# naman1618/Distributed-Inference-with-PyTorch-and-LiteLLM

Hardware: AMD Instinct MI355X
Metric: fine-tune tokens/sec (whole node) Llama-3.1-70B DDP at 1/2/4/8 MI355X (higher is better)
Workload: dtype bf16; 1 GPU; model=Llama-3.1-70B, global_batch=2, seq_len=2048, parallelism=dp1, finetune=lora r=16 alpha=32.0 on q,k,v,o,gate,up,down; frozen bf16 base, micro_batch=2, grad_accum=1, activation_checkpointing=False, optimizer=fused AdamW (HIP), grad clip 1.0, grad_reduce_dtype=bf16

## Files before the change

csrc/bindings.cpp:

```cpp
#include <torch/library.h>
#include <ATen/ATen.h>
#include <ATen/hip/impl/HIPStreamMasqueradingAsCUDA.h>
#include <ATen/hip/impl/HIPGuardImplMasqueradingAsCUDA.h>
#include <hip/hip_runtime.h>
#include "bindings.h"
#include <algorithm>
#include <cstring>
#include <limits>
#include <mutex>
#include <vector>

namespace {

inline hipStream_t cur_stream() { return c10::hip::getCurrentHIPStreamMasqueradingAsCUDA().stream(); }
using DevGuard = c10::hip::HIPGuardMasqueradingAsCUDA;

#define MX_CHECK(cond, ...) TORCH_CHECK(cond, "mxllm: ", __VA_ARGS__)
#define MX_OK(call)                                                                              \
  do {                                                                                           \
    int _rc = (call);                                                                            \
    TORCH_CHECK(_rc == 0, "mxllm kernel launch failed (" #call ") rc=", _rc, " ",                 \
                hipGetErrorString((hipError_t)(_rc > 0 ? _rc : 1)));                             \
  } while (0)

// ... 100 lines not shown
  return {dx, need_dw ? dw : at::Tensor()};
}

void copy2d_batched(const at::Tensor& desc, int64_t total_blocks) {
  MX_CHECK(desc.is_cuda() && desc.scalar_type() == at::kLong && desc.dim() == 2 && desc.size(1) == 9 &&
               desc.is_contiguous(), "desc must be int64 [n, 9] on the GPU");
  DevGuard g(desc.device());
  MX_OK(mx_copy2d_batched(desc.data_ptr<int64_t>(), (int)desc.size(0), total_blocks, cur_stream()));
}

at::Tensor transpose2d(const at::Tensor& in, const c10::optional<at::Tensor>& scale) {
  MX_CHECK(in.is_cuda() && in.dim() == 2 && in.element_size() == 2, "in must be a 2-D 16-bit GPU tensor");
  MX_CHECK(in.stride(1) == 1 && in.stride(0) >= in.size(1), "in must be a row-major (row-strided) view");
  const float* sc = nullptr;
  if (scale.has_value()) {
    MX_CHECK(in.scalar_type() == at::kBFloat16 && scale->scalar_type() == at::kFloat && scale->numel() == 1 &&
                 scale->device() == in.device(), "transpose2d scale: f32 scalar on the device, bf16 input");
    sc = scale->data_ptr<float>();
  }
  DevGuard g(in.device());
  const int64_t R = in.size(0), C = in.size(1);
  auto out = at::empty({C, R}, in.options());
  MX_OK(mx_transpose16(in.data_ptr(), out.data_ptr(), R, C, in.stride(0), R, sc, cur_stream()));
  return out;
}


inline const uint16_t* g8p(const mx::G8Mat& m) { return static_cast<const uint16_t*>(m.p); }
inline uint16_t* g8pm(const mx::G8Mat& m) { return static_cast<uint16_t*>(const_cast<void*>(m.p)); }

const float* f32_scalar(const char* what, const c10::optional<at::Tensor>& t, const at::Device& dev) {
  if (!t.has_value()) return nullptr;
  MX_CHECK(t->scalar_type() == at::kFloat && t->numel() == 1 && t->device() == dev, what,
           ": f32 scalar on the device");
  return t->data_ptr<float>();
}

bool g8_fill(const char* op, mx::G8Launch& L, const at::Tensor& a, bool a_kc, const at::Tensor& b, bool b_kc,
             const at::Tensor* out, bool f32_ok) {
  MX_CHECK(a.is_cuda() && b.is_cuda() && (!out || out->is_cuda()), op, ": GPU tensors");
  MX_CHECK(a.scalar_type() == at::kBFloat16 && b.scalar_type() == at::kBFloat16, op, ": bf16 operands");
  MX_CHECK(!out || out->scalar_type() == at::kBFloat16 || (f32_ok && out->scalar_type() == at::kFloat), op,
           f32_ok ? ": fp32 / bf16 output" : ": bf16 output");
  MX_CHECK(a.dim() == 2 && b.dim() == 2 && (!out || out->dim() == 2), op, ": 2-D operands");
  const int64_t M = a_kc ? a.size(0) : a.size(1), K = a_kc ? a.size(1) : a.size(0);
  const int64_t N = b_kc ? b.size(0) : b.size(1), Kb = b_kc ? b.size(1) : b.size(0);
  MX_CHECK(K == Kb && (!out || (out->size(0) == M && out->size(1) == N)), op, ": shape mismatch");
  if (a.stride(1) != 1 || b.stride(1) != 1 || (out && out->stride(1) != 1)) return false;
  if (M > INT32_MAX || N > INT32_MAX || K > INT32_MAX) return false;
  L.A = {a.data_ptr(), a.stride(0), a_kc ? 1 : 0};
  L.B = {b.data_ptr(), b.stride(0), b_kc ? 1 : 0};
  if (out) L.C = {out->data_ptr(), out->stride(0), 1};
  L.out_f32 = out && out->scalar_type() == at::kFloat ? 1 : 0;
  L.M = (int)M, L.N = (int)N, L.K = (int)K;
  return true;
}

bool g8_fill_rope(const char* op, mx::G8Launch& L, const at::Tensor& x, const at::Tensor& w, const at::Tensor& cos,
                  const at::Tensor& sin, int64_t B, int64_t S, int64_t Hq, int64_t Hkv, at::Tensor& q, at::Tensor& k,
                  at::Tensor& v) {
  MX_CHECK(x.dim() == 2 && w.dim() == 2 && x.size(0) == B * S, op, ": shapes");
  MX_CHECK(w.size(0) == (Hq + 2 * Hkv) * 128, op, ": head dim 128");
  MX_CHECK(cos.scalar_type() == at::kFloat && sin.scalar_type() == at::kFloat && cos.is_contiguous() &&
               sin.is_contiguous() && cos.size(-1) == 64 && cos.size(0) >= S && sin.sizes() == cos.sizes(),
           op, ": f32 [>= S, 64] tables");
  for (const at::Tensor* t : {&q, &k, &v})
    MX_CHECK(t->is_cuda() && t->scalar_type() == at::kBFloat16 && t->is_contiguous(), op, ": bf16 outputs");
  MX_CHECK(q.numel() == B * Hq * S * 128 && k.numel() == B * Hkv * S * 128 && v.numel() == k.numel(), op,
           ": output sizes");
  if (!g8_fill(op, L, x, true, w, true, nullptr, false)) return false;
  L.epi = mx::G8_EPI_ROPE;
  L.ep.q = bfm(q), L.ep.k = bfm(k), L.ep.v = bfm(v);
  L.ep.cosb = cos.data_ptr<float>(), L.ep.sinb = sin.data_ptr<float>();
  L.ep.S = (int)S, L.ep.Hq = (int)Hq, L.ep.Hkv = (int)Hkv;
  return true;
}

bool g8_launched(const char* op, int rc) {
  if (rc == -1) return false;
  TORCH_CHECK(rc == 0, "mxllm kernel launch failed (", op, ") rc=", rc, " ", hipGetErrorString((hipError_t)(rc > 0 ? rc : 1)));
  return true;
}

bool gemm8(const at::Tensor& a, bool a_kc, const at::Tensor& b, bool b_kc, at::Tensor& out, double beta,
           const c10::optional<at::Tensor>& alpha_t, double alpha_f, int64_t ph) {
  mx::G8Launch L{};
  if (!g8_fill("gemm8", L, a, a_kc, b, b_kc, &out, true)) return false;
  const float* sc = f32_scalar("gemm8 alpha_t", alpha_t, a.device());
  DevGuard g(a.device());
  return g8_launched("mx_gemm8", mx_gemm8(g8p(L.A), L.A.ld, L.A.kc, g8p(L.B), L.B.ld, L.B.kc, out.data_ptr(), L.C.ld,
                                          L.out_f32, L.M, L.N, L.K, (float)beta, sc, (float)alpha_f, (int)ph,
                                          cur_stream()));
}

bool gemm8_sq(const at::Tensor& a, bool a_kc, const at::Tensor& b, bool b_kc, at::Tensor& out, at::Tensor& sq,
              const c10::optional<at::Tensor>& alpha_t, double alpha_f) {
  MX_CHECK(sq.is_cuda() && sq.scalar_type() == at::kFloat, "gemm8_sq: f32 GPU partials");
  mx::G8Launch L{};
  if (!g8_fill("gemm8_sq", L, a, a_kc, b, b_kc, &out, false) || !sq.is_contiguous()) return false;
  if (L.M % 256 || L.N % 256) return false;
  MX_CHECK(sq.numel() >= (int64_t)(L.M / 256) * (L.N / 256), "gemm8_sq: partials buffer too small");
  const float* sc = f32_scalar("gemm8_sq alpha_t", alpha_t, a.device());
  DevGuard g(a.device());
  return g8_launched("mx_gemm8_sq", mx_gemm8_sq(g8p(L.A), L.A.ld, L.A.kc, g8p(L.B), L.B.ld, L.B.kc, g8pm(L.C), L.C.ld,
                                                L.M, L.N, L.K, sc, (float)alpha_f, sq.data_ptr<float>(),
                                                cur_stream()));
}

bool gemm8_tail(const at::Tensor& a, bool a_kc, const at::Tensor& b, bool b_kc, at::Tensor& out, int64_t at,
                bool rows, int64_t ph, const c10::optional<at::Tensor>& sq) {
  mx::G8Launch L{};
  if (!g8_fill("gemm8_tail", L, a, a_kc, b, b_kc, &out, false)) return false;
  const int64_t lim = rows ? L.M : L.N;
  if (at <= 0 || at >= lim) return false;
  float* sqp = nullptr;
  if (sq.has_value()) {
    MX_CHECK(sq->scalar_type() == at::kFloat && sq->is_contiguous() && sq->device() == a.device(),
             "gemm8_tail sq: contiguous f32 on the device");
    if (L.M % 256 || L.N % 256) return false;
    MX_CHECK(sq->numel() >= (int64_t)(L.M / 256) * (L.N / 256), "gemm8_tail sq: partials buffer too small");
    sqp = sq->data_ptr<float>();
  }
  DevGuard g(a.device());
  auto ws = at::empty({2 * (lim - at) * (rows ? L.N : L.M)}, a.options().dtype(at::kFloat));
  return g8_launched("mx_gemm8_tail",
                     mx_gemm8_tail(g8p(L.A), L.A.ld, L.A.kc, g8p(L.B), L.B.ld, L.B.kc, g8pm(L.C), L.C.ld, L.M, L.N, L.K,
                                   rows ? 1 : 0, (int)at, ws.data_ptr<float>(), (int)ph, cur_stream(), sqp));
}

bool gemm8_rope(const at::Tensor& x, const at::Tensor& w, const at::Tensor& cos, const at::Tensor& sin, int64_t B,
                int64_t S, int64_t Hq, int64_t Hkv, at::Tensor& q, at::Tensor& k, at::Tensor& v) {
  mx::G8Launch L{};
  if (!g8_fill_rope("gemm8_rope", L, x, w, cos, sin, B, S, Hq, Hkv, q, k, v)) return false;
  DevGuard g(x.device());
  return g8_launched("mx_gemm8_epi", mx_gemm8_epi(g8p(L.A), L.A.ld, g8p(L.B), L.B.ld, nullptr, 0, L.M, L.N, L.K,
                                                  mx::G8_EPI_ROPE, L.ep, cur_stream()));
}

bool gemm8_rope_tail(const at::Tensor& x, const at::Tensor& w, const at::Tensor& cos, const at::Tensor& sin, int64_t B,
                     int64_t S, int64_t Hq, int64_t Hkv, at::Tensor& q, at::Tensor& k, at::Tensor& v, int64_t at) {
  mx::G8Launch L{};
  if (!g8_fill_rope("gemm8_rope_tail", L, x, w, cos, sin, B, S, Hq, Hkv, q, k, v) || at <= 0 || at >= L.N) return false;
  DevGuard g(x.device());
  auto ws = at::empty({2 * (int64_t)L.M * (L.N - at)}, x.options().dtype(at::kFloat));
  return g8_launched("mx_gemm8_rope_tail", mx_gemm8_rope_tail(g8p(L.A), L.A.ld, g8p(L.B), L.B.ld, L.M, L.N, L.K, (int)at,
                                                              ws.data_ptr<float>(), L.ep, cur_stream()));
}

bool gemm8_swiglu(const at::Tensor& x, const at::Tensor& w, at::Tensor& gu, at::Tensor& m) {
  mx::G8Launch L{};
  const bool ok = g8_fill("gemm8_swiglu", L, x, true, w, true, &gu, false);
  MX_CHECK(m.scalar_type() == at::kBFloat16 && m.dim() == 2 && m.size(0) == x.size(0) && 2 * m.size(1) == w.size(0),
           "gemm8_swiglu: m [T, F] bf16");
  if (!ok || m.stride(1) != 1) return false;
  DevGuard g(x.device());
  L.ep.m = bfm(m);
  L.ep.ldm = m.stride(0);
  return g8_launched("mx_gemm8_epi", mx_gemm8_epi(g8p(L.A), L.A.ld, g8p(L.B), L.B.ld, g8pm(L.C), L.C.ld, L.M, L.N, L.K,
                                                  mx::G8_EPI_SWIGLU, L.ep, cur_stream()));
}

bool gemm8_swiglu_bwd(const at::Tensor& dy, const at::Tensor& w, const at::Tensor& gu, at::Tensor& dgu,
                      const c10::optional<at::Tensor>& m) {
  mx::G8Launch L{};
  const bool ok = g8_fill("gemm8_swiglu_bwd", L, dy, true, w, false, nullptr, false);
  MX_CHECK(gu.is_cuda() && gu.scalar_type() == at::kBFloat16 && dgu.scalar_type() == at::kBFloat16,
           "gemm8_swiglu_bwd: bf16 GPU tensors");
  MX_CHECK(gu.dim() == 2 && dgu.dim() == 2 && gu.size(0) == dy.size(0) && gu.size(1) == 2 * w.size(1) &&
               dgu.sizes() == gu.sizes(),
           "gemm8_swiglu_bwd: shapes");
  if (m) {
    MX_CHECK(m->scalar_type() == at::kBFloat16 && m->dim() == 2 && m->size(0) == dy.size(0) &&
                 m->size(1) == w.size(1),
             "gemm8_swiglu_bwd: m [T, F] bf16");
    if (m->stride(1) != 1) return false;
    L.ep.m = reinterpret_cast<uint16_t*>(m->data_ptr());
    L.ep.ldm = m->stride(0);
  }
  if (!ok || gu.stride(1) != 1 || dgu.stride(1) != 1) return false;
  DevGuard g(dy.device());
  L.ep.gu = bf(gu);
  L.ep.ldg = gu.stride(0);
  return g8_launched("mx_gemm8_epi", mx_gemm8_epi(g8p(L.A), L.A.ld, g8p(L.B), L.B.ld, bfm(dgu), dgu.stride(0), L.M, L.N,
                                                  L.K, mx::G8_EPI_SWIGLU_BWD, L.ep, cur_stream()));
}

at::Tensor gemm8_stamps() {
  auto out = at::empty({1024, 2, 80}, at::TensorOptions().dtype(at::kLong));
  MX_OK(mx_gemm8_stamps(reinterpret_cast<unsigned long long*>(out.data_ptr<int64_t>())));
  return out;
}

int64_t cu_masked_stream(int64_t device, std::vector<int64_t> mask) {
  MX_CHECK(!mask.empty(), "cu_masked_stream: empty mask");
  DevGuard g(c10::Device(c10::DeviceType::CUDA, (c10::DeviceIndex)device));
  std::vector<uint32_t> w(mask.size());
  for (size_t i = 0; i < mask.size(); ++i) w[i] = (uint32_t)(mask[i] & 0xffffffffLL);
  hipStream_t s = nullptr;
  hipError_t e = hipExtStreamCreateWithCUMask(&s, (uint32_t)(w.size() * 32), w.data());
  MX_CHECK(e == hipSuccess, "hipExtStreamCreateWithCUMask: ", hipGetErrorString(e));
  return (int64_t)reinterpret_cast<intptr_t>(s);
}

void prefetch(const at::Tensor& t, int64_t wgs) {
  MX_CHECK(t.is_cuda() && t.is_contiguous(), "prefetch: contiguous GPU tensor");
  DevGuard g(t.device());
  MX_OK(mx_prefetch(t.data_ptr(), t.numel() * t.element_size(), (int)wgs, cur_stream()));
}

at::Tensor segmented_mean(const at::Tensor& codes, const at::Tensor& offsets) {
  MX_CHECK(codes.is_cuda() && codes.scalar_type() == at::kInt, "codes must be int32 GPU");
  MX_CHECK(offsets.is_cuda() && offsets.scalar_type() == at::kLong, "offsets must be int64 GPU");
  DevGuard g(codes.device());
  const int64_t n = offsets.numel() - 1;
  auto out = at::empty({std::max<int64_t>(n, 0)}, codes.options().dtype(at::kFloat));
  if (n > 0)
    MX_OK(mx_segmented_mean_i32(codes.data_ptr<int32_t>(), offsets.data_ptr<int64_t>(),
                                out.data_ptr<float>(), (int)n, cur_stream()));
  return out;
}

at::Tensor sqnorm(const at::Tensor& x) {
  MX_CHECK(x.is_cuda() && x.is_contiguous(), "x must be a contiguous GPU tensor");
  MX_CHECK(x.scalar_type() == at::kFloat || x.scalar_type() == at::kBFloat16, "x must be float32 or bfloat16");
  DevGuard g(x.device());
  auto opts = x.options().dtype(at::kFloat);
  auto out = at::empty({1}, opts);
  auto work = at::empty({2048}, opts);
  MX_OK(mx_sqnorm(x.data_ptr(), x.scalar_type() == at::kBFloat16 ? 1 : 0, x.numel(), out.data_ptr<float>(),
                  work.data_ptr<float>(), cur_stream()));
  return out;
}

at::Tensor swiglu_fwd(const at::Tensor& gu, int64_t out_pad) {
  check_bf16(gu, "gu");
  DevGuard g(gu.device());
  const int64_t F2 = gu.size(-1);
  MX_CHECK(F2 % 16 == 0, "2F must be a multiple of 16");
  MX_CHECK(out_pad >= 0 && out_pad % 8 == 0, "out_pad must be a non-negative multiple of 8");
  const int64_t T = gu.numel() / F2;
  at::Tensor m;
  if (out_pad > 0) {
    m = empty_rows(T, F2 / 2, out_pad, gu.options());
  } else {
    auto sizes = gu.sizes().vec();
    sizes.back() = F2 / 2;
    m = at::empty(sizes, gu.options());
  }
  if (T > 0) MX_OK(mx_swiglu_fwd(bf(gu), bfm(m), T, (int)(F2 / 2), F2 / 2 + out_pad, cur_stream()));
  return m;
}

at::Tensor swiglu_bwd(const at::Tensor& dm, const at::Tensor& gu, int64_t out_pad) {
  check_bf16(dm, "dm");
  check_bf16(gu, "gu");
  DevGuard g(gu.device());
  const int64_t F2 = gu.size(-1);
  const int64_t T = gu.numel() / F2;
  MX_CHECK(dm.numel() == T * (F2 / 2), "dm shape mismatch");
  MX_CHECK(out_pad >= 0 && out_pad % 8 == 0, "out_pad must be a non-negative multiple of 8");
  at::Tensor dgu = out_pad > 0 ? empty_rows(T, F2, out_pad, gu.options()) : at::empty_like(gu);
  if (T > 0) MX_OK(mx_swiglu_bwd(bf(dm), bf(gu), bfm(dgu), T, (int)(F2 / 2), F2 + out_pad, cur_stream()));
  return dgu;
}

std::vector<at::Tensor> swiglu_bwd_m(const at::Tensor& dm, const at::Tensor& gu) {
  check_bf16(dm, "dm");
  check_bf16(gu, "gu");
  DevGuard g(gu.device());
  const int64_t F2 = gu.size(-1);
  const int64_t T = gu.numel() / F2;
  MX_CHECK(dm.numel() == T * (F2 / 2), "dm shape mismatch");
  MX_CHECK(dm.is_contiguous() && gu.is_contiguous(), "swiglu_bwd_m: dense dm / gu");
  at::Tensor dgu = at::empty_like(gu);
  at::Tensor m = at::empty({T, F2 / 2}, gu.options());
  if (T > 0) MX_OK(mx_swiglu_bwd(bf(dm), bf(gu), bfm(dgu), T, (int)(F2 / 2), F2, cur_stream(), bfm(m)));
  return {dgu, m};
}

at::Tensor swiglu_lora(const c10::optional<at::Tensor>& dm, const at::Tensor& gu, int64_t pad, const at::Tensor& v,
                       int64_t nrb, double alpha) {
  check_bf16(gu, "gu");
  const int64_t ldv = check_rows_bf16(v, "v");
  DevGuard g(gu.device());
  const bool bwd = dm.has_value();
  MX_CHECK(gu.dim() == 2 && gu.size(1) > 0 && gu.size(1) % 256 == 0,
           "swiglu_lora: gu [T, 2F] with F % 128 == 0 (gate | up halves of equal width)");
  const int64_t F2 = gu.size(1), F = F2 / 2, T = gu.size(0);
  MX_CHECK(T % 16 == 0, "swiglu_lora: [T, 2F] with T % 16 == 0");
  MX_CHECK(nrb >= 1 && nrb <= 4 && pad >= 16 * nrb && pad % 8 == 0, "swiglu_lora: 16 nrb <= pad");
  MX_CHECK(v.size(0) >= 16 * nrb && v.size(1) == (bwd ? F2 : F), "swiglu_lora: v shape");
  if (bwd) {
    check_bf16(*dm, "dm");
    MX_CHECK(dm->numel() == T * F, "swiglu_lora: dm shape");
  }
  const int64_t W = bwd ? F2 : F;
  at::Tensor out = at::empty({T, W + pad}, gu.options());
  const int64_t nws = mx_swiglu_lora_ws((int)T, (int)F, (int)nrb);
  auto ws = at::empty({nws > 0 ? nws : 1}, gu.options().dtype(at::kFloat));
  if (T > 0)
    MX_OK(mx_swiglu_lora(bwd ? 1 : 0, bf(gu), bwd ? bf(*dm) : nullptr, bfm(out), W + pad, bf(v), ldv, (int)nrb,
                         (int)pad, (float)alpha, ws.data_ptr<float>(), (int)T, (int)F, cur_stream()));
  return out.narrow(1, 0, W);
}

void adamw_step(const c10::optional<at::Tensor>& master, at::Tensor grad, at::Tensor m, at::Tensor v,
                const c10::optional<at::Tensor>& lowp, const c10::optional<at::Tensor>& lo, double lr, double b1,
                double b2, double eps, double wd, double bc1, double bc2, const c10::optional<at::Tensor>& scale_t,
                double scale_f, bool zero_grad) {
  MX_CHECK(master.has_value() != lo.has_value(), "give either the fp32 master or the split low half");
  check_f32(m, "m");
  check_f32(v, "v");
  MX_CHECK(grad.is_cuda() && grad.is_contiguous(), "grad must be contiguous GPU");
  MX_CHECK(grad.scalar_type() == at::kFloat || grad.scalar_type() == at::kBFloat16, "grad f32/bf16");
  const int64_t n = m.numel();
  MX_CHECK(grad.numel() == n && v.numel() == n, "adamw size mismatch");
  float* mp = nullptr;
  if (master.has_value()) {
    check_f32(*master, "master");
    MX_CHECK(master->numel() == n, "master size");
    mp = master->data_ptr<float>();
  }
  DevGuard g(m.device());
  uint16_t* lp = nullptr;
  if (lowp.has_value()) {
    check_bf16(*lowp, "lowp");
    MX_CHECK(lowp->numel() == n, "lowp size");
    lp = reinterpret_cast<uint16_t*>(lowp->data_ptr());
  }
  int16_t* lop = nullptr;
  if (lo.has_value()) {
    MX_CHECK(lo->is_cuda() && lo->is_contiguous() && lo->scalar_type() == at::kShort && lo->numel() == n,
             "lo must be a contiguous int16 GPU tensor of the master's size");
    MX_CHECK(lp != nullptr, "split master needs lowp (the high half)");
    lop = lo->data_ptr<int16_t>();
  }
  const float* st = nullptr;
  if (scale_t.has_value()) {
    check_f32(*scale_t, "scale_t");
    st = scale_t->data_ptr<float>();
  }
  MX_OK(mx_adamw(mp, grad.data_ptr(), grad.scalar_type() == at::kBFloat16 ? 1 : 0, m.data_ptr<float>(),
                 v.data_ptr<float>(), lp, lop, n, (float)lr, (float)b1, (float)b2, (float)eps, (float)wd, (float)bc1,
                 (float)bc2, st, (float)scale_f, zero_grad ? 1 : 0, cur_stream()));
}

void split_master(const at::Tensor& x, at::Tensor hi, at::Tensor lo) {
  check_f32(x, "x");
  check_bf16(hi, "hi");
  MX_CHECK(lo.is_cuda() && lo.is_contiguous() && lo.scalar_type() == at::kShort, "lo int16 contiguous GPU");
  MX_CHECK(hi.numel() == x.numel() && lo.numel() == x.numel(), "split_master size mismatch");
  DevGuard g(x.device());
  MX_OK(mx_split_master(x.data_ptr<float>(), reinterpret_cast<uint16_t*>(hi.data_ptr()), lo.data_ptr<int16_t>(),
                        x.numel(), cur_stream()));
}

void join_master(const at::Tensor& hi, const at::Tensor& lo, at::Tensor out) {
  check_bf16(hi, "hi");
  check_f32(out, "out");
  MX_CHECK(lo.is_cuda() && lo.is_contiguous() && lo.scalar_type() == at::kShort, "lo int16 contiguous GPU");
  MX_CHECK(hi.numel() == out.numel() && lo.numel() == out.numel(), "join_master size mismatch");
  DevGuard g(out.device());
  MX_OK(mx_join_master(reinterpret_cast<const uint16_t*>(hi.data_ptr()), lo.data_ptr<int16_t>(),
                       out.data_ptr<float>(), out.numel(), cur_stream()));
}

at::Tensor embedding_fwd(const at::Tensor& ids, const at::Tensor& w) {
  check_bf16(w, "weight");
  MX_CHECK(ids.is_cuda() && ids.scalar_type() == at::kLong, "ids must be int64 GPU");
  DevGuard g(w.device());
  auto idc = ids.contiguous();
  const int64_t T = idc.numel(), H = w.size(1), V = w.size(0);
  auto out = at::empty({T, H}, w.options());
  MX_OK(mx_embedding_fwd(idc.data_ptr<int64_t>(), bf(w), bfm(out), T, (int)H, V, cur_stream()));
  return out;
}

at::Tensor embedding_bwd(const at::Tensor& dy, const at::Tensor& ids, int64_t V) {
  check_bf16(dy, "dy");
  DevGuard g(dy.device());
  auto idc = ids.contiguous();
  const int64_t H = dy.size(-1), T = idc.numel();
  auto dw = at::zeros({V, H}, dy.options().dtype(at::kFloat));
  MX_OK(mx_embedding_bwd(idc.data_ptr<int64_t>(), bf(dy), dw.data_ptr<float>(), T, (int)H, V, cur_stream()));
  return dw;
}

void embedding_bwd_sorted(const at::Tensor& dy, const at::Tensor& sid, const at::Tensor& perm, at::Tensor out) {
  check_bf16(dy, "dy");
  MX_CHECK(sid.scalar_type() == at::kLong && perm.scalar_type() == at::kLong && sid.is_contiguous() &&
               perm.is_contiguous() && sid.numel() == perm.numel(), "sid / perm: int64, same length");
  MX_CHECK(out.is_contiguous() && (out.scalar_type() == at::kFloat || out.scalar_type() == at::kBFloat16) &&
               out.dim() == 2 && out.size(1) == dy.size(-1) && dy.is_contiguous() &&
               dy.numel() == sid.numel() * dy.size(-1) && out.device() == dy.device(),
           "embedding_bwd_sorted: out [V, H] f32/bf16 contiguous, dy [T, H] contiguous");
  DevGuard g(dy.device());
  const int64_t T = sid.numel(), nch = (T + 63) / 64;
  auto ws = at::empty({std::max<int64_t>(1, 2 * nch * out.size(1))}, dy.options().dtype(at::kFloat));
  MX_OK(mx_embedding_bwd_sorted(bf(dy), sid.data_ptr<int64_t>(), perm.data_ptr<int64_t>(), T, (int)out.size(1),
                                out.size(0), out.data_ptr(), out.scalar_type() == at::kFloat ? 1 : 0,
                                ws.data_ptr<float>(), cur_stream()));
}

std::tuple<at::Tensor, at::Tensor> ce_fwd_bwd(at::Tensor logits, const at::Tensor& labels, int64_t ignore) {
  check_bf16(logits, "logits");
  MX_CHECK(labels.is_cuda() && labels.scalar_type() == at::kLong, "labels must be int64 GPU");
  DevGuard g(logits.device());
  const int64_t V = logits.size(-1), T = logits.numel() / V;
  MX_CHECK(labels.numel() == T, "labels size mismatch");
  auto lab = labels.contiguous();
  auto losses = at::empty({T}, logits.options().dtype(at::kFloat));
  auto ws = at::empty({2}, logits.options().dtype(at::kFloat));
  auto loss = at::empty({}, logits.options().dtype(at::kFloat));
  MX_OK(mx_ce_fwd_bwd(bfm(logits), lab.data_ptr<int64_t>(), losses.data_ptr<float>(), ws.data_ptr<float>(),
                      loss.data_ptr<float>(), T, (int)V, ignore, cur_stream()));
  return {loss, losses};
}

at::Tensor ce_inv_count(const at::Tensor& labels, int64_t ignore, int64_t V) {
  MX_CHECK(labels.is_cuda() && labels.scalar_type() == at::kLong, "labels must be int64 GPU");
  DevGuard g(labels.device());
  auto lab = labels.contiguous();
  auto inv = at::empty({1}, labels.options().dtype(at::kFloat));
  MX_OK(mx_ce_inv_count(lab.data_ptr<int64_t>(), lab.numel(), (int)V, ignore, inv.data_ptr<float>(), cur_stream()));
  return inv;
}

at::Tensor ce_chunk(at::Tensor logits, const at::Tensor& labels, int64_t ignore, const at::Tensor& inv_n) {
  check_bf16(logits, "logits");
  MX_CHECK(logits.is_contiguous(), "ce_chunk: contiguous logits");
  MX_CHECK(labels.is_cuda() && labels.scalar_type() == at::kLong, "labels must be int64 GPU");
  MX_CHECK(inv_n.scalar_type() == at::kFloat && inv_n.numel() == 1 && inv_n.device() == logits.device(),
           "ce_chunk: inv_n f32 device scalar");
  DevGuard g(logits.device());
  const int64_t V = logits.size(-1), T = logits.numel() / V;
  MX_CHECK(labels.numel() == T, "labels size mismatch");
  auto lab = labels.contiguous();
  auto losses = at::empty({T}, logits.options().dtype(at::kFloat));
  MX_OK(mx_ce_chunk(bfm(logits), lab.data_ptr<int64_t>(), losses.data_ptr<float>(), inv_n.data_ptr<float>(), T,
                    (int)V, ignore, cur_stream()));
  return losses;
}

at::Tensor ce_chunk_f32(const at::Tensor& logits, at::Tensor dl, const at::Tensor& labels, int64_t ignore,
                        const at::Tensor& inv_n) {
  check_f32(logits, "logits");
  check_bf16(dl, "dl");
  MX_CHECK(logits.is_contiguous() && dl.is_contiguous() && dl.sizes() == logits.sizes(), "ce_chunk_f32: shapes");
  MX_CHECK(labels.is_cuda() && labels.scalar_type() == at::kLong, "labels must be int64 GPU");
  MX_CHECK(inv_n.scalar_type() == at::kFloat && inv_n.numel() == 1 && inv_n.device() == logits.device(),
           "ce_chunk_f32: inv_n f32 device scalar");
  DevGuard g(logits.device());
  const int64_t V = logits.size(-1), T = logits.numel() / V;
  MX_CHECK(labels.numel() == T, "labels size mismatch");
  auto lab = labels.contiguous();
  auto losses = at::empty({T}, logits.options());
  MX_OK(mx_ce_chunk_f32(logits.data_ptr<float>(), bfm(dl), lab.data_ptr<int64_t>(), losses.data_ptr<float>(),
                        inv_n.data_ptr<float>(), T, (int)V, ignore, cur_stream()));
  return losses;
}

std::tuple<at::Tensor, at::Tensor, at::Tensor> rope_split(const at::Tensor& qkv, const at::Tensor& cos,
                                                          const at::Tensor& sin, int64_t B, int64_t S, int64_t Hq,
                                                          int64_t Hkv, int64_t D,
                                                          const c10::optional<at::Tensor>& positions) {
  check_bf16(qkv, "qkv");
  check_f32(cos, "cos");
  check_f32(sin, "sin");
  MX_CHECK(qkv.numel() == B * S * (Hq + 2 * Hkv) * D, "qkv shape mismatch");
  MX_CHECK(cos.size(-1) == D / 2, "rope table width");
  DevGuard g(qkv.device());
  const int32_t* pos = nullptr;
  if (positions.has_value()) {
    MX_CHECK(positions->scalar_type() == at::kInt && positions->numel() == B * S, "positions int32 [B*S]");
    pos = positions->data_ptr<int32_t>();
  } else {
    MX_CHECK(cos.size(0) >= S, "rope table too short");
  }
  auto q = at::empty({B, Hq, S, D}, qkv.options());
  auto k = at::empty({B, Hkv, S, D}, qkv.options());
  auto v = at::empty({B, Hkv, S, D}, qkv.options());
  MX_OK(mx_rope_split(bf(qkv), cos.data_ptr<float>(), sin.data_ptr<float>(), pos, bfm(q), bfm(k), bfm(v), (int)B,
                      (int)S, (int)Hq, (int)Hkv, (int)D, cur_stream()));
  return {q, k, v};
}

at::Tensor rope_merge_bwd(const at::Tensor& dq, const at::Tensor& dkp, const at::Tensor& dvp, const at::Tensor& cos,
                          const at::Tensor& sin, int64_t B, int64_t S, int64_t Hq, int64_t Hkv, int64_t D,
                          int64_t out_pad) {
  check_f32(dq, "dq");
  check_f32(dkp, "dkp");
  check_f32(dvp, "dvp");
  DevGuard g(dq.device());
  const int64_t kvin = dkp.size(1);
  MX_CHECK(dkp.dim() == 4 && dkp.size(0) == B && dkp.size(2) == S && dkp.size(3) == D, "dk partial shape");
  MX_CHECK(out_pad >= 0 && out_pad % 8 == 0, "out_pad must be a non-negative multiple of 8");
  const int64_t NHD = (Hq + 2 * Hkv) * D;
  auto dqkv = empty_rows(B * S, NHD, out_pad, dq.options().dtype(at::kBFloat16));
  MX_OK(mx_rope_merge_bwd(dq.data_ptr<float>(), dkp.data_ptr<float>(), dvp.data_ptr<float>(), cos.data_ptr<float>(),
                          sin.data_ptr<float>(), bfm(dqkv), (int)B, (int)S, (int)Hq, (int)Hkv, (int)kvin, (int)D,
                          NHD + out_pad, cur_stream(), 0));
  return dqkv;
}

typedef c10::optional<at::Tensor> OptTensor;
static void attn_operand(const char* op, const char* name, const at::Tensor& t, at::Device dev, at::ScalarType dt) {
  MX_CHECK(t.is_cuda() && t.device() == dev && t.scalar_type() == dt && t.is_contiguous(), op, ": ", name,
           " must be a contiguous ", c10::toString(dt), " GPU tensor on q's device");
}
static void attn_launched(const char* op, int rc, const mx::AbLaunch& L) {
  MX_CHECK(rc != -1, op, ": the kernels do not take this call (mx::af_takes / mx::ab_takes, kernels/attn_args.h): B ",
           L.B, ", Hq ", L.Hq, ", Hkv ", L.Hkv, ", S ", L.S, ", Sk ", L.Sk, ", D ", L.D, ", causal ", L.causal,
           ", dq_mode ", L.dq_mode, ", row strides o ", L.ldo, ", dqkv ", L.ldq);
  TORCH_CHECK(rc == 0, "mxllm kernel launch failed (", op, ") rc=", rc, " ", hipGetErrorString((hipError_t)rc));
}
static mx::AbLaunch attn_fill(const char* op, const at::Tensor& q, const at::Tensor& k, const at::Tensor& v,
                              bool causal, int64_t dq_mode = 3, const at::Tensor* o = nullptr,
                              const at::Tensor* dout = nullptr, const at::Tensor* lse = nullptr,
                              const at::Tensor* cos = nullptr, const at::Tensor* sin = nullptr,
                              const OptTensor& dq_out = c10::nullopt, const OptTensor& dk_out = c10::nullopt,
                              const OptTensor& dv_out = c10::nullopt) {
  MX_CHECK(q.dim() == 4 && k.dim() == 4 && v.dim() == 4, op, ": q [B,Hq,S,D], k/v [B,Hkv,Sk,D]");
  const at::Device dev = q.device();
  for (auto [n, t] : {std::pair{"q", &q}, {"k", &k}, {"v", &v}}) attn_operand(op, n, *t, dev, at::kBFloat16);
  mx::AbLaunch L{};
  L.B = q.size(0), L.Hq = q.size(1), L.S = q.size(2), L.D = q.size(3), L.Hkv = k.size(1), L.Sk = k.size(2);
  MX_CHECK(k.size(0) == L.B && k.size(3) == L.D && v.sizes() == k.sizes(), op, ": k ", k.sizes(), " and v ", v.sizes(),
           " must be [B,Hkv,Sk,D] for q ", q.sizes());
  L.q = q.data_ptr(), L.k = k.data_ptr(), L.v = v.data_ptr(), L.q_bf16 = L.kv_bf16 = 1;
  L.causal = causal ? 1 : 0, L.dq_mode = (int)dq_mode, L.ldo = L.Hq * L.D, L.hpw = 1;
  if (!dout) return L;
  MX_CHECK(dq_mode >= 1 && dq_mode <= 3, op, ": dq_mode must be 1, 2 or 3");
  attn_operand(op, "dout", *dout, dev, at::kBFloat16);
  attn_operand(op, "lse", *lse, dev, at::kFloat);
  MX_CHECK(dout->numel() == q.numel() && o->numel() == dout->numel(), op, ": dout/o shape");
  MX_CHECK(lse->numel() == L.B * L.Hq * L.S, op, ": lse must be [B,Hq,S], got ", lse->sizes());
  if (o->is_contiguous()) {
    attn_operand(op, "o", *o, dev, at::kBFloat16);
  } else {
    MX_CHECK(o->is_cuda() && o->device() == dev && o->scalar_type() == at::kBFloat16 && o->dim() == 3 &&
                 o->stride(2) == 1 && o->size(2) == L.Hq * L.D && o->stride(0) == L.S * o->stride(1) &&
                 o->stride(1) % 8 == 0, op, ": o must be [B, S, Hq*D] with unit inner stride");
    L.ldo = o->stride(1);
  }
  L.o = o->data_ptr(), L.dout = dout->data_ptr(), L.lse = lse->data_ptr();
  L.o_bf16 = L.dout_bf16 = L.lse_f32 = L.out_f32 = 1;
  if (cos) {
    MX_CHECK(mx::ab_takes_rope(dq_mode, L.D, L.S, L.Sk), op, ": D = 128 self-attention in the split mode");
    for (auto [n, t] : {std::pair{"cos", cos}, {"sin", sin}}) attn_operand(op, n, *t, dev, at::kFloat);
    MX_CHECK(L.D >= 2 && cos->numel() >= L.S * (L.D / 2) && sin->numel() >= L.S * (L.D / 2), op,
             ": cos / sin: [>= S, D/2] contiguous f32");
    L.cos = cos->data_ptr(), L.sin = sin->data_ptr();
    L.cos_rows = std::min(cos->numel(), sin->numel()) / (L.D / 2);
  }
  const int64_t P = mx_attn_bwd_partial_heads(L);
  if (dq_out.has_value() || dk_out.has_value() || dv_out.has_value()) {
    MX_CHECK(dq_out.has_value() && dk_out.has_value() && dv_out.has_value() && dq_mode == 3, op,
             ": preallocated outputs need all three and the split mode");
    for (auto [n, t] : {std::pair{"dq_out", &*dq_out}, {"dk_out", &*dk_out}, {"dv_out", &*dv_out}})
      attn_operand(op, n, *t, dev, at::kFloat);
    MX_CHECK(dq_out->numel() == q.numel() && dk_out->numel() == L.B * P * L.Sk * L.D &&
                 dv_out->numel() == L.B * P * L.Sk * L.D, op, ": output sizes");
  }
  attn_launched(op, mx::ab_shape_takes(L) ? 0 : -1, L);
  return L;
}

std::tuple<at::Tensor, at::Tensor> attn_fwd(const at::Tensor& q, const at::Tensor& k, const at::Tensor& v,
                                            bool causal, double scale, int64_t out_pad) {
  mx::AbLaunch S = attn_fill("attn_fwd", q, k, v, causal);
  MX_CHECK(out_pad >= 0 && out_pad % 8 == 0, "out_pad must be a non-negative multiple of 8");
  S.ldo += out_pad;
  DevGuard g(q.device());
  auto o = at::empty({S.B, S.S, S.ldo}, q.options()).narrow(2, 0, S.Hq * S.D);
  auto lse = at::empty({S.B, S.Hq, S.S}, q.options().dtype(at::kFloat));
  mx::AfLaunch L{S.q, S.k, S.v, o.data_ptr(), lse.data_ptr(), 1, 1, 1, 1, S.B, S.Hq, S.Hkv, S.S, S.Sk, S.D, S.ldo};
  L.causal = S.causal;
  attn_launched("attn_fwd", mx_attn_fwd(L, (float)scale, cur_stream()), S);
  return {o, lse};
}

static std::tuple<at::Tensor, at::Tensor, at::Tensor> attn_bwd_impl(
    const char* op, const at::Tensor& dout, const at::Tensor& q, const at::Tensor& k, const at::Tensor& v,
    const at::Tensor& o, const at::Tensor& lse, bool causal, double scale, int64_t dq_mode, const OptTensor& dq_out,
    const OptTensor& dk_out, const OptTensor& dv_out, at::Tensor* dqkv = nullptr, int64_t dqkv_pad = 0,
    const at::Tensor* cos = nullptr, const at::Tensor* sin = nullptr) {
  mx::AbLaunch L = attn_fill(op, q, k, v, causal, dq_mode, &o, &dout, &lse, cos, sin, dq_out, dk_out, dv_out);
  DevGuard g(q.device());
  const auto f32 = q.options().dtype(at::kFloat);
  const bool outs = dq_out.has_value();
  const int64_t P = L.Hq / L.hpw, S_pad = mx::ab_s_pad(L.S);
  auto dkp = outs ? *dk_out : at::empty({L.B, P, L.Sk, L.D}, f32);
  auto dvp = outs ? *dv_out : at::empty({L.B, P, L.Sk, L.D}, f32);
  auto delta = at::empty({L.B, L.Hq, L.S}, f32);
  auto work = at::empty({mx::ab_work_bytes(L)}, q.options().dtype(at::kByte));
  auto dq = outs ? *dq_out
                 : (dq_mode == 1 ? at::zeros({L.B, L.Hq, S_pad, L.D}, f32)
                                 : at::empty({dqkv ? 0 : L.B, L.Hq, L.S, L.D}, f32));
  L.delta = delta.data_ptr(), L.dq = dq.data_ptr(), L.dkp = dkp.data_ptr(), L.dvp = dvp.data_ptr();
  if (dq_mode != 1) L.work = work.data_ptr();
  if (dqkv) *dqkv = empty_rows(L.B * L.S, (L.Hq + 2 * L.Hkv) * L.D, dqkv_pad, q.options());
  if (dqkv) L.dqkv = dqkv->data_ptr(), L.ldq = dqkv->stride(0), L.dqkv_bf16 = 1;
  attn_launched(op, mx_attn_bwd(L, (float)scale, cur_stream()), L);
  if (dq_mode == 1 && S_pad != L.S) dq = dq.narrow(2, 0, L.S).contiguous();
  return {dq, dkp, dvp};
}
// ... 433 lines not shown
at::Tensor spec_accept(const at::Tensor& drawn, const at::Tensor& tokens, const at::Tensor& nq) {
  MX_CHECK(drawn.is_cuda() && drawn.is_contiguous() && drawn.dim() == 2 && drawn.scalar_type() == at::kLong &&
               drawn.size(1) >= 1,
           "spec_accept: drawn must be a contiguous int64 [B, n] GPU tensor");
  MX_CHECK(tokens.device() == drawn.device() && tokens.is_contiguous() && tokens.scalar_type() == at::kLong &&
               tokens.sizes() == drawn.sizes(),
           "spec_accept: tokens must be a contiguous int64 [B, n] tensor on drawn's device");
  const int64_t B = drawn.size(0), n = drawn.size(1);
  MX_CHECK(B <= 0x7fffffff / (n + 1), "spec_accept: B * (n + 1) must fit 31 bits");
  MX_CHECK(nq.defined(), "spec_accept: nq");
  const int32_t* np = check_rows_i32(nq, drawn.device(), B, "spec_accept", "nq");
  DevGuard g(drawn.device());
  auto out = at::empty({B, n + 1}, drawn.options().dtype(at::kInt));
  MX_OK(mx_spec_accept(drawn.data_ptr<int64_t>(), tokens.data_ptr<int64_t>(), np, out.data_ptr<int32_t>(), (int)B,
                       (int)n, cur_stream()));
  return out;
}

at::Tensor logits_adjust_rows(const at::Tensor& logits, const c10::optional<at::Tensor>& state,
                              const at::Tensor& slots, const at::Tensor& presence, const at::Tensor& frequency,
                              const at::Tensor& repetition, const c10::optional<at::Tensor>& bias) {
  MX_CHECK(logits.is_cuda() && logits.is_contiguous() && logits.dim() == 2, "logits [B, V] contiguous GPU");
  MX_CHECK(logits.scalar_type() == at::kBFloat16 || logits.scalar_type() == at::kFloat, "logits bf16/f32");
  const int64_t B = logits.size(0), V = logits.size(1);
  auto chk = [&](const at::Tensor& t, at::ScalarType st, const char* name) {
    MX_CHECK(t.is_cuda() && t.is_contiguous() && t.scalar_type() == st && t.numel() == B, name);
  };
  chk(slots, at::kInt, "slots i32 [B]");
  chk(presence, at::kFloat, "presence f32 [B]");
  chk(frequency, at::kFloat, "frequency f32 [B]");
  chk(repetition, at::kFloat, "repetition f32 [B]");
  int64_t n_slots = -1;
  auto table = [&](const c10::optional<at::Tensor>& t, at::ScalarType st, const char* name) {
    if (!t.has_value()) return;
    MX_CHECK(t->is_cuda() && t->is_contiguous() && t->scalar_type() == st && t->dim() == 2 && t->size(1) == V &&
                 (n_slots < 0 || t->size(0) == n_slots), name);
    n_slots = t->size(0);
  };
  table(state, at::kInt, "state i32 [n_slots, V]");
  table(bias, at::kFloat, "bias f32 [n_slots, V]");
  DevGuard g(logits.device());
  auto out = at::empty({B, V}, logits.options().dtype(at::kFloat));
  MX_OK(mx_logits_adjust_rows(logits.data_ptr(), logits.scalar_type() == at::kBFloat16 ? 1 : 0,
                              out.data_ptr<float>(), (int)B, (int)V,
                              state.has_value() ? state->data_ptr<int32_t>() : nullptr, slots.data_ptr<int32_t>(),
                              (int)std::max<int64_t>(n_slots, 0), presence.data_ptr<float>(),
                              frequency.data_ptr<float>(), repetition.data_ptr<float>(),
                              bias.has_value() ? bias->data_ptr<float>() : nullptr, cur_stream()));
  return out;
}

void token_state_update(at::Tensor state, const at::Tensor& slots, const at::Tensor& ids) {
  MX_CHECK(state.is_cuda() && state.is_contiguous() && state.scalar_type() == at::kInt && state.dim() == 2,
           "state i32 [n_slots, V] contiguous GPU");
  const int64_t B = slots.numel();
  MX_CHECK(slots.is_cuda() && slots.is_contiguous() && slots.scalar_type() == at::kInt, "slots i32 [B]");
  MX_CHECK(ids.is_cuda() && ids.is_contiguous() && ids.scalar_type() == at::kLong && ids.numel() == B, "ids i64 [B]");
  DevGuard g(state.device());
  MX_OK(mx_token_state_update(state.data_ptr<int32_t>(), slots.data_ptr<int32_t>(), ids.data_ptr<int64_t>(), (int)B,
                              (int)state.size(1), (int)state.size(0), cur_stream()));
}

std::tuple<at::Tensor, at::Tensor, at::Tensor> logprob_rows(const at::Tensor& logits, const at::Tensor& ids,
                                                            const at::Tensor& n_top) {
  MX_CHECK(logits.is_cuda() && logits.is_contiguous() && logits.dim() == 2, "logits [B, V] contiguous GPU");
  MX_CHECK(logits.scalar_type() == at::kBFloat16 || logits.scalar_type() == at::kFloat, "logits bf16/f32");
  const int64_t B = logits.size(0);
  MX_CHECK(ids.is_cuda() && ids.is_contiguous() && ids.scalar_type() == at::kLong && ids.numel() == B, "ids i64 [B]");
  MX_CHECK(n_top.is_cuda() && n_top.is_contiguous() && n_top.scalar_type() == at::kInt && n_top.numel() == B,
           "n_top i32 [B]");
  DevGuard g(logits.device());
  auto chosen = at::empty({B}, logits.options().dtype(at::kFloat));
  auto top_ids = at::empty({B, 20}, logits.options().dtype(at::kInt));
  auto top_lp = at::empty({B, 20}, logits.options().dtype(at::kFloat));
  MX_CHECK(B <= 65535 && logits.size(1) <= 2048 * 400, "logprob_rows: at most 65535 rows of at most 819200 logits");
  auto ws = at::empty({std::max<int64_t>(1, (mx_logprob_ws_bytes((int)B, (int)logits.size(1)) + 7) / 8)},
                      logits.options().dtype(at::kLong));
  MX_OK(mx_logprob_rows(logits.data_ptr(), logits.scalar_type() == at::kBFloat16 ? 1 : 0, ids.data_ptr<int64_t>(),
                        n_top.data_ptr<int32_t>(), chosen.data_ptr<float>(), top_ids.data_ptr<int32_t>(),
                        top_lp.data_ptr<float>(), (int)B, (int)logits.size(1), ws.data_ptr(), cur_stream()));
  return {chosen, top_ids, top_lp};
}

}


static void sk_rows(const char* op, const char* name, const at::Tensor& t, const at::Device& dev) {
  MX_CHECK(t.is_cuda() && t.device() == dev && t.scalar_type() == at::kBFloat16 && t.dim() == 2 && t.stride(1) == 1, op,
           ": ", name, " must be bf16 [rows, cols] GPU rows with a unit inner stride, on one device with the others");
}
static bool sk_ints(int64_t M, int64_t N, int64_t K) {
  const int64_t lim = std::numeric_limits<int>::max();
  return M <= lim && N <= lim && K <= lim;
}
static mx::SkLaunch sk_fill(const char* op, mx::SkEntry entry, const at::Tensor* x, const at::Tensor& w,
                            const at::Device& dev, int64_t M, int64_t K) {
  if (x) sk_rows(op, "x", *x, dev);
  sk_rows(op, "w", w, dev);
  MX_CHECK(w.size(1) == K && (!x || M >= 1) && sk_ints(M, w.size(0), K), op, ": ", M, " rows of ", K, " against w ",
           w.sizes());
  mx::SkLaunch L{};
  L.entry = entry, L.W = {w.data_ptr(), w.stride(0)}, L.M = (int)M, L.N = (int)w.size(0), L.K = (int)K;
  if (x) L.X = {x->data_ptr(), x->stride(0)};
  return L;
}
static mx::SkLaunch sk_fill(const char* op, mx::SkEntry entry, const at::Tensor& x, const at::Tensor& w) {
  MX_CHECK(x.dim() == 2, op, ": x must be [M, K]");
  return sk_fill(op, entry, &x, w, x.device(), x.size(0), x.size(1));
}
static at::Tensor sk_norm(const char* op, mx::SkLaunch& L, const at::Tensor& h, const c10::optional<at::Tensor>& delta,
                          const at::Tensor& gamma, double eps) {
  MX_CHECK(gamma.device() == h.device() && gamma.scalar_type() == at::kBFloat16 && gamma.is_contiguous() &&
               gamma.numel() == L.K, op, ": gamma must be contiguous bf16 [K] on h's device");
  L.na.gamma = bf(gamma);
  L.na.eps = (float)eps;
  if (!delta.has_value() || !delta->defined()) return h;
  sk_rows(op, "delta", *delta, h.device());
  MX_CHECK(delta->size(0) == L.M && delta->size(1) == L.K, op, ": delta must have h's shape");
  at::Tensor h_out = at::empty({L.M, L.K}, h.options());
  L.na.delta = bf(*delta), L.na.ldd = delta->stride(0), L.na.h_out = bfm(h_out);
  return h_out;
}
static void sk_rope(const char* op, mx::SkLaunch& L, const at::Tensor& h, const at::Tensor& cosb, const at::Tensor& sinb,
                    const at::Tensor& pos, const c10::optional<at::Tensor>& slots, at::Tensor& k_cache,
                    at::Tensor& v_cache, int64_t Hq, int64_t Hkv, const c10::optional<at::Tensor>& block_table) {
  MX_CHECK(Hq > 0 && Hkv > 0 && sk_ints(Hq, Hkv, 0), op, ": Hq, Hkv");
  check_kv_pools(k_cache, v_cache, at::kBFloat16, 128, h.device(), Hkv, op);
  for (const at::Tensor* t : {&cosb, &sinb})
    MX_CHECK(t->device() == h.device() && t->scalar_type() == at::kFloat && t->is_contiguous() && t->dim() == 2 &&
                 t->size(1) == 64, op, ": cos / sin must be contiguous float32 [positions, 64] on h's device");
  MX_CHECK(pos.defined(), op, ": pos");
  const int32_t* pp = check_rows_i32(pos, h.device(), L.M, op, "pos");
  const int32_t* sl = check_rows_i32(slots, h.device(), L.M, op, "slots");
  const KvPages pg = kv_pages(block_table, k_cache);
  L.rp = {cosb.data_ptr<float>(), sinb.data_ptr<float>(), pp, sl, nullptr, bfm(k_cache), bfm(v_cache), (int)Hq,
          (int)Hkv, (int)k_cache.size(2), pg.bt, pg.maxb};
}
static void sk_launched(const char* op, int rc, const mx::SkLaunch& L) {
  MX_CHECK(rc != -1, op, ": the kernel does not take this call (mx::sk_takes, csrc/kernels/skinny_args.h): M ", L.M,
           ", N ", L.N, ", K ", L.K, ", row strides x ", L.X.ld, ", w ", L.W.ld, ", y ", L.Y.ld, ", delta ", L.na.ldd);
  TORCH_CHECK(rc == 0, "mxllm kernel launch failed (", op, ") rc=", rc, " ", hipGetErrorString((hipError_t)rc));
}
static at::Tensor sk_run(const char* op, mx::SkLaunch& L, const at::Tensor& t, int64_t cols) {
  auto y = at::empty({L.M, cols}, t.options());
  L.Y = {y.data_ptr(), cols};
  sk_launched(op, mx_skinny(L, cur_stream()), L);
  return y;
}

at::Tensor skinny_linear(const at::Tensor& x, const at::Tensor& w) {
  mx::SkLaunch L = sk_fill("skinny_linear", mx::SK_PLAIN, x, w);
  DevGuard g(x.device());
  return sk_run("skinny_linear", L, x, L.N);
}

at::Tensor skinny_linear_swiglu(const at::Tensor& x, const at::Tensor& w) {
  mx::SkLaunch L = sk_fill("skinny_linear_swiglu", mx::SK_SWIGLU, x, w);
  DevGuard g(x.device());
  return sk_run("skinny_linear_swiglu", L, x, L.N / 2);
}

std::tuple<at::Tensor, at::Tensor> skinny_norm_linear(const at::Tensor& h, const c10::optional<at::Tensor>& delta,
                                                      const at::Tensor& gamma, double eps, const at::Tensor& w,
                                                      bool swiglu) {
  mx::SkLaunch L = sk_fill("skinny_norm_linear", mx::SK_NORM, h, w);
  L.swiglu = swiglu ? 1 : 0;
  DevGuard g(h.device());
  at::Tensor h_out = sk_norm("skinny_norm_linear", L, h, delta, gamma, eps);
  return {sk_run("skinny_norm_linear", L, h, swiglu ? L.N / 2 : L.N), h_out};
}

std::tuple<at::Tensor, at::Tensor> skinny_qkv_rope(const at::Tensor& h, const c10::optional<at::Tensor>& delta,
                                                   const c10::optional<at::Tensor>& gamma, double eps,
                                                   const at::Tensor& w, const at::Tensor& cosb, const at::Tensor& sinb,
                                                   const at::Tensor& pos, const c10::optional<at::Tensor>& slots,
                                                   at::Tensor& k_cache, at::Tensor& v_cache, int64_t Hq, int64_t Hkv,
                                                   const c10::optional<at::Tensor>& block_table) {
  mx::SkLaunch L = sk_fill("skinny_qkv_rope", mx::SK_ROPE, h, w);
  sk_rope("skinny_qkv_rope", L, h, cosb, sinb, pos, slots, k_cache, v_cache, Hq, Hkv, block_table);
  L.norm = gamma.has_value() && gamma->defined();
  DevGuard g(h.device());
  at::Tensor h_out = L.norm ? sk_norm("skinny_qkv_rope", L, h, delta, *gamma, eps) : h;
  auto q = at::empty({L.M, Hq, 128}, h.options());
  L.rp.q = bfm(q);
  sk_launched("skinny_qkv_rope", mx_skinny(L, cur_stream()), L);
  return {q, h_out};
}

at::Tensor skinny_merge_linear(const at::Tensor& ml, const at::Tensor& po, const at::Tensor& w) {
  MX_CHECK(ml.is_cuda() && ml.scalar_type() == at::kFloat && ml.is_contiguous() && ml.dim() == 4 && ml.size(3) == 2,
           "skinny_merge_linear: part_ml f32 [M, Hq, nsplit, 2]");
  MX_CHECK(po.device() == ml.device() && po.scalar_type() == at::kFloat && po.is_contiguous() && po.dim() == 4 &&
               po.size(0) == ml.size(0) && po.size(1) == ml.size(1) && po.size(2) == ml.size(2) && po.size(3) == 128,
           "skinny_merge_linear: part_o f32 [M, Hq, nsplit, 128]");
  mx::SkLaunch L = sk_fill("skinny_merge_linear", mx::SK_MERGE, nullptr, w, ml.device(), ml.size(0), ml.size(1) * 128);
  MX_CHECK(sk_ints(ml.size(2), 0, 0), "skinny_merge_linear: nsplit");
  L.mg = {ml.data_ptr<float>(), po.data_ptr<float>(), (int)ml.size(2)};
  DevGuard g(w.device());
  return sk_run("skinny_merge_linear", L, w, L.N);
}

at::Tensor w8_linear(const at::Tensor& x, const at::Tensor& q, const at::Tensor& scale) {
  sk_rows("w8_linear", "x", x, x.device());
  MX_CHECK(q.is_cuda() && q.scalar_type() == at::kByte && q.dim() == 2 && q.is_contiguous(), "q: uint8 [N, K]");
  check_f32(scale, "scale");
  const int64_t M = x.size(0), K = x.size(1), N = q.size(0);
  MX_CHECK(q.size(1) == K && scale.numel() == N, "w8_linear shapes");
  DevGuard g(x.device());
  auto y = at::empty({M, N}, x.options());
  mx::SkLaunch L{};
  L.entry = mx::SK_W8, L.X = {x.data_ptr(), x.stride(0)}, L.W = {q.data_ptr(), K}, L.Y = {y.data_ptr(), N};
  L.M = (int)M, L.N = (int)N, L.K = (int)K, L.scale = scale.data_ptr<float>();
  if (M == 0 || (sk_ints(M, N, K) && mx::sk_takes(L))) {
    sk_launched("w8_linear", mx_w8a16_gemm(bf(x), x.stride(0), q.data_ptr<uint8_t>(), L.scale, bfm(y), N, L.M, L.N,
                                           L.K, cur_stream()), L);
    return y;
  }
  auto w = at::empty({N, K}, x.options());
  MX_OK(mx_w8_dequant(q.data_ptr<uint8_t>(), scale.data_ptr<float>(), bfm(w), N, (int)K, cur_stream()));
  return at::mm(x, w.t());
}

std::tuple<at::Tensor, at::Tensor> quant_rows_e4m3(const at::Tensor& x) {
  MX_CHECK(x.is_cuda() && x.scalar_type() == at::kBFloat16 && x.dim() == 2 && x.stride(1) == 1, "x: bf16 [M, K] rows");
  DevGuard g(x.device());
  const int64_t M = x.size(0), K = x.size(1);
  auto q = at::empty({M, K}, x.options().dtype(at::kByte));
  auto s = at::empty({M, 1}, x.options().dtype(at::kFloat));
  MX_OK(mx_quant_rows_e4m3(bf(x), x.stride(0), q.data_ptr<uint8_t>(), s.data_ptr<float>(), M, (int)K,
                           cur_stream()));
  return {q, s};
}

at::Tensor w8_dequant(const at::Tensor& q, const at::Tensor& scale) {
  MX_CHECK(q.is_cuda() && q.scalar_type() == at::kByte && q.dim() == 2 && q.is_contiguous(), "q: uint8 [N, K]");
  check_f32(scale, "scale");
  DevGuard g(q.device());
  auto w = at::empty({q.size(0), q.size(1)}, q.options().dtype(at::kBFloat16));
  MX_OK(mx_w8_dequant(q.data_ptr<uint8_t>(), scale.data_ptr<float>(), bfm(w), q.size(0), (int)q.size(1),
                      cur_stream()));
  return w;
}

static void w4_weights(const char* op, const at::Tensor& codes, const at::Tensor& scales, const at::Device& dev) {
  MX_CHECK(codes.is_cuda() && codes.device() == dev && codes.scalar_type() == at::kByte && codes.dim() == 2 &&
               codes.is_contiguous(), op, ": codes must be contiguous uint8 [N, K/2] on the GPU");
  MX_CHECK(scales.device() == dev && scales.scalar_type() == at::kByte && scales.dim() == 2 && scales.is_contiguous() &&
               scales.size(0) == codes.size(0) && codes.size(1) % 16 == 0 && scales.size(1) == codes.size(1) / 16,
           op, ": scales must be contiguous uint8 [N, K/32] beside codes [N, K/2], K % 32 == 0");
}

at::Tensor w4_dequant(const at::Tensor& codes, const at::Tensor& scales) {
  w4_weights("w4_dequant", codes, scales, codes.device());
  DevGuard g(codes.device());
  const int64_t N = codes.size(0), K = 2 * codes.size(1);
  auto w = at::empty({N, K}, codes.options().dtype(at::kBFloat16));
  MX_OK(mx_w4_dequant(codes.data_ptr<uint8_t>(), scales.data_ptr<uint8_t>(), bfm(w), N, K, cur_stream()));
  return w;
}

at::Tensor w4_linear(const at::Tensor& x, const at::Tensor& codes, const at::Tensor& scales, int64_t stream_m) {
  sk_rows("w4_linear", "x", x, x.device());
  w4_weights("w4_linear", codes, scales, x.device());
  const int64_t M = x.size(0), K = x.size(1), N = codes.size(0);
  MX_CHECK(2 * codes.size(1) == K, "w4_linear: x has ", K, " columns, the codes ", 2 * codes.size(1));
  DevGuard g(x.device());
  auto y = at::empty({M, N}, x.options());
  if (M == 0 || N == 0) return y;
  const int64_t ldx = M <= 1 ? K : x.stride(0);
  mx::W4Launch L{};
  L.x = x.data_ptr(), L.ldx = ldx, L.codes = codes.data_ptr(), L.scales = scales.data_ptr();
  L.y = y.data_ptr(), L.ldy = N;
  L.M = std::min<int64_t>(M, mx::W4_MAX_M), L.N = N, L.K = K;
  if (M <= std::max<int64_t>(stream_m, mx::W4_MAX_M) && mx::w4_takes(L)) {
    for (int64_t m0 = 0; m0 < M; m0 += mx::W4_MAX_M) {
      L.x = bf(x) + m0 * ldx, L.y = bfm(y) + m0 * N, L.M = std::min<int64_t>(M - m0, mx::W4_MAX_M);
      const int rc = mx_w4a16_gemm(L, cur_stream());
      MX_CHECK(rc != -1, "w4_linear: the kernel does not take this call (mx::w4_takes, csrc/kernels/w4_args.h): M ", L.M,
               ", N ", N, ", K ", K, ", row stride x ", ldx);
      TORCH_CHECK(rc == 0, "mxllm kernel launch failed (w4_linear) rc=", rc, " ", hipGetErrorString((hipError_t)rc));
    }
    return y;
  }
  auto w = at::empty({N, K}, x.options());
  MX_OK(mx_w4_dequant(codes.data_ptr<uint8_t>(), scales.data_ptr<uint8_t>(), bfm(w), N, K, cur_stream()));
  return at::mm(x, w.t());
}

void lora_xwt(const at::Tensor& x, const at::Tensor& v, at::Tensor& out, double alpha, int64_t rows) {
  const int64_t ldx = check_rows_bf16(x, "x"), ldv = check_rows_bf16(v, "v"), ldo = check_rows_bf16(out, "out");
  const int64_t M = x.size(0), K = x.size(1), Vr = v.size(0);
  MX_CHECK(v.size(1) == K && out.size(0) == M && out.size(1) >= Vr, "lora_xwt shapes");
  MX_CHECK(rows >= 0 && rows <= Vr, "lora_xwt: rows <= rows(v)");
  MX_CHECK(M % 16 == 0 && K % 64 == 0 && Vr % 64 == 0 && ldo % 4 == 0,
           "lora_xwt: M % 16, K % 64, rows(v) % 64");
  DevGuard g(x.device());
  const int64_t nws = mx_lora_xwt_ws((int)M, (int)K, (int)rows);
  auto ws = at::empty({nws > 0 ? nws : 1}, x.options().dtype(at::kFloat));
  MX_OK(mx_lora_xwt(bf(x), ldx, bf(v), ldv, (int)Vr, bfm(out), ldo, ws.data_ptr<float>(), (int)M, (int)K, (float)alpha,
                    (int)rows, cur_stream()));
}

void lora_grads(const at::Tensor& x, const at::Tensor& dy, const at::Tensor& g, const at::Tensor& st, at::Tensor& ga,
                at::Tensor& gb, at::IntArrayRef splits, int64_t r, bool accumulate) {
  const int64_t ldx = check_rows_bf16(x, "x"), ldd = check_rows_bf16(dy, "dy");
  const int64_t ldg = check_rows_bf16(g, "g"), lds = check_rows_bf16(st, "st");
  check_bf16(ga, "ga");
  check_bf16(gb, "gb");
  const int64_t T = x.size(0), K = x.size(1), N = dy.size(1), n = (int64_t)splits.size(), R = n * r;
  MX_CHECK(dy.size(0) == T && g.size(0) == T && st.size(0) == T, "lora_grads: token counts differ");
  MX_CHECK(ga.size(0) == R && ga.size(1) == K && gb.size(0) == N && gb.size(1) == R, "lora_grads: grad shapes");
  MX_CHECK(T % 64 == 0 && K % 64 == 0 && r % 16 == 0 && r <= 64, "lora_grads: T, K multiples of 64, r of 16");
  std::vector<int64_t> desc;
  auto add = [&](const uint16_t* X, int64_t lx, const uint16_t* G, int64_t lg, int64_t gw, uint16_t* out, int64_t os_n,
                 int64_t os_j, int64_t Nx, int64_t jb0, int64_t JB) {
    MX_CHECK(16 * (jb0 + JB) <= gw, "lora_grads: operand tail too narrow");
    MX_CHECK(Nx % 64 == 0, "lora_grads: split sizes must be multiples of 64");
    if (JB > 1 && 16 * jb0 + 64 > gw) {
      for (int64_t j = 0; j < JB; ++j)
        desc.insert(desc.end(), {(int64_t)X, (int64_t)G, (int64_t)(out + 16 * j * os_j), lx, lg, os_n, os_j, Nx,
                                 jb0 + j, (int64_t)1});
      return;
    }
    desc.insert(desc.end(), {(int64_t)X, (int64_t)G, (int64_t)out, lx, lg, os_n, os_j, Nx, jb0, JB});
  };
  for (int64_t j0 = 0; j0 < R; j0 += 64) {
    const int64_t jb = std::min<int64_t>(4, (R - j0) / 16);
    add(bf(x), ldx, bf(g), ldg, g.size(1), bfm(ga) + j0 * K, 1, K, K, j0 / 16, jb);
  }
  int64_t off = 0;
  for (int64_t i = 0; i < n; ++i) {
    const int64_t ni = splits[i];
    add(bf(dy) + off, ldd, bf(st), lds, st.size(1), bfm(gb) + off * R + i * r, R, 1, ni, i * r / 16, r / 16);
    off += ni;
  }
  MX_CHECK(off == N, "lora_grads: splits do not sum to dy's width");
  const int np = (int)(desc.size() / 10);
  MX_CHECK(np <= 8, "lora_grads: too many problems");
  int64_t ntiles = 0;
  for (int i = 0; i < np; ++i) ntiles += desc[i * 10 + 7] / 64;
  DevGuard gd(x.device());
  const int64_t nws = mx_lora_xtg_ws((int)ntiles, (int)T);
  auto ws = at::empty({nws > 0 ? nws : 1}, x.options().dtype(at::kFloat));
  MX_OK(mx_lora_xtg(desc.data(), np, (int)T, 1.0f, accumulate ? 1 : 0, ws.data_ptr<float>(), cur_stream()));
}

struct LoraServeCall {
  int64_t M, W, ld, n_adapters, KS, R;
  const int32_t* ids;
};
static LoraServeCall check_lora_serve(const char* op, const at::Tensor& rows, const char* rows_name,
                                      const at::Tensor& ids, const at::Tensor& tab, int64_t tab_w_dim,
                                      const at::Tensor& partials, int64_t K) {
  MX_CHECK(rows.is_cuda() && rows.scalar_type() == at::kBFloat16 && rows.dim() == 2 && rows.size(0) >= 1, op, ": ",
           rows_name, " must be a bfloat16 [M, ", tab_w_dim == 2 ? "K" : "N", "] GPU tensor with M >= 1");
  MX_CHECK(rows.stride(1) == 1 && rows.stride(0) >= rows.size(1) && rows.stride(0) % 8 == 0 &&
               reinterpret_cast<uintptr_t>(rows.data_ptr()) % 16 == 0,
           op, ": ", rows_name, " must be a 16-byte aligned row-major view with a row stride that is a multiple of 8");
  LoraServeCall c{rows.size(0), rows.size(1), rows.stride(0), 0, 0, 0, nullptr};
  MX_CHECK(c.W >= 8 && c.W % 8 == 0, op, ": ", rows_name, " has ", c.W, " columns, not a positive multiple of 8");
  MX_CHECK(c.M < (int64_t(1) << 31) && c.ld < (int64_t(1) << 31), op, ": ", rows_name, " is too large");
  c.ids = check_rows_i32(ids, rows.device(), c.M, op, "ids");
  MX_CHECK(c.ids != nullptr, op, ": ids");
  MX_CHECK(tab.device() == rows.device() && tab.scalar_type() == at::kBFloat16 && tab.is_contiguous() &&
               tab.dim() == 3 && tab.size(0) >= 1 && tab.size(tab_w_dim) == c.W,
           op, ": the table must be a contiguous bfloat16 ", tab_w_dim == 2 ? "[n_adapters, R, K]" : "[n_adapters, N, r_max]",
           " tensor on ", rows_name, "'s device whose ", tab_w_dim == 2 ? "K" : "N", " is ", c.W);
  c.n_adapters = tab.size(0);
  c.KS = mx_lora_serve_ksplits((int)(tab_w_dim == 2 ? c.W : K));
  MX_CHECK(partials.device() == rows.device() && partials.scalar_type() == at::kFloat && partials.is_contiguous() &&
               partials.dim() == 3 && partials.size(0) == c.KS && partials.size(1) == c.M,
           op, ": partials must be a contiguous float32 [", c.KS, ", ", c.M, ", R] tensor on ", rows_name, "'s device");
  c.R = partials.size(2);
  return c;
}

void lora_gather_shrink(const at::Tensor& x, const at::Tensor& ids, const at::Tensor& a_tab, at::Tensor partials) {
  const LoraServeCall c = check_lora_serve("lora_gather_shrink", x, "x", ids, a_tab, 2, partials, 0);
  MX_CHECK(a_tab.size(1) == c.R && c.R % 8 == 0 && c.R >= 8 && c.R <= 192, "lora_gather_shrink: A_tab holds ",
           a_tab.size(1), " rows per adapter and partials ", c.R, "; both must be n_splits * r_max <= 192");
  DevGuard g(x.device());
  MX_OK(mx_lora_gather_shrink(bf(x), c.ld, c.ids, bf(a_tab), partials.data_ptr<float>(), (int)c.M, (int)c.W, (int)c.R,
                              (int)c.n_adapters, cur_stream()));
}

void lora_gather_expand_add_(at::Tensor y, const at::Tensor& partials, const at::Tensor& ids, const at::Tensor& b_tab,
                             const at::Tensor& s_tab, at::IntArrayRef splits, int64_t K) {
  const char* op = "lora_gather_expand_add_";
  MX_CHECK(K >= 8 && K % 8 == 0 && K < (int64_t(1) << 31), op, ": K must be a positive multiple of 8");
  const LoraServeCall c = check_lora_serve(op, y, "y", ids, b_tab, 1, partials, K);
  const int64_t r_max = b_tab.size(2), ns = (int64_t)splits.size();
  MX_CHECK(r_max == 8 || r_max == 16 || r_max == 32 || r_max == 64, op, ": r_max must be 8, 16, 32 or 64, got ", r_max);
  MX_CHECK(ns >= 1 && ns <= 3, op, ": 1 to 3 splits, got ", ns);
  int sp[3] = {0, 0, 0};
  int64_t sum = 0;
  for (int64_t i = 0; i < ns; ++i) {
    MX_CHECK(splits[i] >= 8 && splits[i] % 8 == 0, op, ": every split must be a positive multiple of 8, got ", splits[i]);
    sp[i] = (int)splits[i];
    sum += splits[i];
  }
  MX_CHECK(sum == c.W, op, ": the splits sum to ", sum, ", y has ", c.W, " columns");
  MX_CHECK(c.R == ns * r_max, op, ": partials hold ", c.R, " columns, expected n_splits * r_max = ", ns * r_max);
  MX_CHECK(s_tab.device() == y.device() && s_tab.scalar_type() == at::kFloat && s_tab.is_contiguous() &&
               s_tab.dim() == 1 && s_tab.size(0) == c.n_adapters,
           op, ": s_tab must be a contiguous float32 [n_adapters] tensor on y's device");
  DevGuard g(y.device());
  MX_OK(mx_lora_gather_expand_add(bfm(y), c.ld, partials.data_ptr<float>(), c.ids, bf(b_tab), s_tab.data_ptr<float>(),
                                  (int)c.M, (int)c.W, (int)c.KS, (int)r_max, sp, (int)ns, (int)c.n_adapters,
                                  cur_stream()));
}

TORCH_LIBRARY(mxllm, m) {
  m.def("rmsnorm_fwd(Tensor x, Tensor? res, Tensor w, float eps, int out_pad=0) -> (Tensor, Tensor, Tensor)");
  m.def("rmsnorm_bwd(Tensor dy, Tensor x, Tensor w, Tensor rstd, Tensor? dres, bool need_dw, int out_pad=0) -> (Tensor, Tensor)");
  m.def("segmented_mean(Tensor codes, Tensor offsets) -> Tensor");
  m.def("copy2d_batched(Tensor desc, int total_blocks) -> ()");
  m.def("transpose2d(Tensor x, Tensor? scale=None) -> Tensor");
  m.def("gemm8(Tensor a, bool a_kc, Tensor b, bool b_kc, Tensor(a!) out, float beta, Tensor? alpha_t=None, float alpha=1.0, int ph=8) -> bool");
  m.def("prefetch(Tensor t, int wgs) -> ()");
  m.def("cu_masked_stream(int device, int[] mask) -> int", &cu_masked_stream);
  m.def("gemm8_stamps() -> Tensor", &gemm8_stamps);
  m.def("gemm8_tail(Tensor a, bool a_kc, Tensor b, bool b_kc, Tensor(a!) out, int at, bool rows=False, int ph=4, Tensor(b!)? sq=None) -> bool");
  m.def("gemm8_rope(Tensor x, Tensor w, Tensor cos, Tensor sin, int B, int S, int Hq, int Hkv, Tensor(a!) q, Tensor(b!) k, Tensor(c!) v) -> bool");
  m.def("gemm8_rope_tail(Tensor x, Tensor w, Tensor cos, Tensor sin, int B, int S, int Hq, int Hkv, Tensor(a!) q, Tensor(b!) k, Tensor(c!) v, int at) -> bool");
  m.def("gemm8_swiglu(Tensor x, Tensor w, Tensor(a!) gu, Tensor(b!) m) -> bool");
  m.def("gemm8_sq(Tensor a, bool a_kc, Tensor b, bool b_kc, Tensor(a!) out, Tensor(b!) sq, Tensor? alpha_t=None, float alpha=1.0) -> bool");
  m.def("gemm8_swiglu_bwd(Tensor dy, Tensor w, Tensor gu, Tensor(a!) dgu, Tensor(b!)? m=None) -> bool");
  m.def("sqnorm(Tensor x) -> Tensor");
  m.def("swiglu_fwd(Tensor gu, int out_pad=0) -> Tensor");
  m.def("swiglu_bwd(Tensor dm, Tensor gu, int out_pad=0) -> Tensor");
  m.def("swiglu_bwd_m(Tensor dm, Tensor gu) -> Tensor[]");
  m.def("adamw_step(Tensor(a!)? master, Tensor(e!) grad, Tensor(b!) m, Tensor(c!) v, Tensor(d!)? lowp, Tensor(f!)? lo, float lr, float b1, float b2, float eps, float wd, float bc1, float bc2, Tensor? scale_t, float scale_f, bool zero_grad=False) -> ()");
  m.def("split_master(Tensor x, Tensor(a!) hi, Tensor(b!) lo) -> ()");
  m.def("join_master(Tensor hi, Tensor lo, Tensor(a!) out) -> ()");
  m.def("embedding_fwd(Tensor ids, Tensor w) -> Tensor");
  m.def("embedding_bwd(Tensor dy, Tensor ids, int V) -> Tensor");
  m.def("embedding_bwd_sorted(Tensor dy, Tensor sid, Tensor perm, Tensor(a!) out) -> ()");
  m.def("ce_fwd_bwd(Tensor(a!) logits, Tensor labels, int ignore_index) -> (Tensor, Tensor)");
  m.def("ce_inv_count(Tensor labels, int ignore_index, int vocab) -> Tensor");
  m.def("ce_chunk(Tensor(a!) logits, Tensor labels, int ignore_index, Tensor inv_n) -> Tensor");
  m.def("ce_chunk_f32(Tensor logits, Tensor(a!) dl, Tensor labels, int ignore_index, Tensor inv_n) -> Tensor");
  m.def("rope_split(Tensor qkv, Tensor cos, Tensor sin, int B, int S, int Hq, int Hkv, int D, Tensor? positions=None) -> (Tensor, Tensor, Tensor)");
  m.def("rope_merge_bwd(Tensor dq, Tensor dkp, Tensor dvp, Tensor cos, Tensor sin, int B, int S, int Hq, int Hkv, int D, int out_pad=0) -> Tensor");
  m.def("attn_fwd(Tensor q, Tensor k, Tensor v, bool causal, float scale, int out_pad=0) -> (Tensor, Tensor)");
  m.def("rope_append(Tensor qkv, Tensor cos, Tensor sin, Tensor pos, Tensor? slots, Tensor(a!) k_cache, Tensor(b!) v_cache, int Hq, int Hkv, int D, Tensor? block_table=None) -> Tensor");
  m.def("decode_attn(Tensor q, Tensor k_cache, Tensor v_cache, Tensor lens, Tensor? slots, int max_len, float scale, int len_off=0, Tensor? block_table=None, Tensor? counters=None) -> Tensor");
  m.def("decode_attn_partials(Tensor q, Tensor k_cache, Tensor v_cache, Tensor lens, Tensor? slots, int max_len, float scale, int len_off=0, Tensor? block_table=None) -> (Tensor, Tensor)");
  m.def("prefill_attn_paged(Tensor q, Tensor k_cache, Tensor v_cache, Tensor block_table, Tensor segs, float scale, Tensor? out=None) -> Tensor");
  m.def("kv8_quant_rows(Tensor x) -> (Tensor, Tensor)");
  m.def("rope_append_kv8(Tensor qkv, Tensor cos, Tensor sin, Tensor pos, Tensor? slots, Tensor(a!) k_codes, Tensor(b!) k_scale, Tensor(c!) v_codes, Tensor(d!) v_scale, int Hq, int Hkv, Tensor? block_table=None) -> Tensor");
  m.def("decode_attn_kv8(Tensor q, Tensor k_codes, Tensor k_scale, Tensor v_codes, Tensor v_scale, Tensor lens, Tensor? slots, int max_len, float scale, int len_off=0, Tensor? block_table=None) -> Tensor");
  m.def("verify_attn(Tensor q, Tensor k_cache, Tensor v_cache, Tensor lens, Tensor nq, Tensor? slots, int n, int max_len, float scale, Tensor? block_table=None, Tensor? out=None) -> Tensor");
  m.def("verify_attn_kv8(Tensor q, Tensor k_codes, Tensor k_scale, Tensor v_codes, Tensor v_scale, Tensor lens, Tensor nq, Tensor? slots, int n, int max_len, float scale, Tensor? block_table=None, Tensor? out=None) -> Tensor");
  m.def("spec_accept(Tensor drawn, Tensor tokens, Tensor nq) -> Tensor");
  m.def("skinny_merge_linear(Tensor ml, Tensor po, Tensor w) -> Tensor");
  m.def("sample(Tensor logits, float temperature, int seed, int step) -> Tensor");
  m.def("sample_rows(Tensor logits, Tensor temps, Tensor top_p, Tensor top_k, Tensor seeds, Tensor steps) -> Tensor");
  m.def("sample_temp_rows(Tensor logits, Tensor temps, Tensor seeds, Tensor steps) -> Tensor");
  m.def("logits_adjust_rows(Tensor logits, Tensor? state, Tensor slots, Tensor presence, Tensor frequency, "
        "Tensor repetition, Tensor? bias) -> Tensor");
  m.def("token_state_update(Tensor(a!) state, Tensor slots, Tensor ids) -> ()");
  m.def("logprob_rows(Tensor logits, Tensor ids, Tensor n_top) -> (Tensor, Tensor, Tensor)");
  m.def("w8_linear(Tensor x, Tensor q, Tensor scale) -> Tensor");
  m.def("skinny_linear(Tensor x, Tensor w) -> Tensor");
  m.def("skinny_linear_swiglu(Tensor x, Tensor w) -> Tensor");
  m.def("skinny_qkv_rope(Tensor h, Tensor? delta, Tensor? gamma, float eps, Tensor w, Tensor cos, Tensor sin, Tensor pos, Tensor? slots, Tensor(a!) k_cache, Tensor(b!) v_cache, int Hq, int Hkv, Tensor? block_table=None) -> (Tensor, Tensor)");
  m.def("skinny_norm_linear(Tensor h, Tensor? delta, Tensor gamma, float eps, Tensor w, bool swiglu) -> (Tensor, Tensor)");
  m.def("w8_dequant(Tensor q, Tensor scale) -> Tensor");
  m.def("w4_linear(Tensor x, Tensor codes, Tensor scales, int stream_m) -> Tensor");
  m.def("w4_dequant(Tensor codes, Tensor scales) -> Tensor");
  m.def("quant_rows_e4m3(Tensor x) -> (Tensor, Tensor)");
  m.def("lora_xwt(Tensor x, Tensor v, Tensor(a!) out, float alpha, int rows=0) -> ()");
  m.def("swiglu_lora(Tensor? dm, Tensor gu, int pad, Tensor v, int nrb, float alpha) -> Tensor");
  m.def("lora_grads(Tensor x, Tensor dy, Tensor g, Tensor st, Tensor(a!) ga, Tensor(b!) gb, int[] splits, int r, bool accumulate) -> ()");
  m.def("lora_gather_shrink(Tensor x, Tensor ids, Tensor a_tab, Tensor(a!) partials) -> ()");
  m.def("lora_gather_expand_add_(Tensor(a!) y, Tensor partials, Tensor ids, Tensor b_tab, Tensor s_tab, int[] splits, int K) -> ()");
  m.def("attn_bwd(Tensor dout, Tensor q, Tensor k, Tensor v, Tensor o, Tensor lse, bool causal, float scale, int dq_mode=3, Tensor? dq_out=None, Tensor? dk_out=None, Tensor? dv_out=None) -> (Tensor, Tensor, Tensor)");
  m.def("attn_bwd_rope(Tensor dout, Tensor q, Tensor k, Tensor v, Tensor o, Tensor lse, bool causal, float scale, Tensor cos, Tensor sin, int out_pad=0) -> Tensor");
}

TORCH_LIBRARY_IMPL(mxllm, CUDA, m) {
  m.impl("rmsnorm_fwd", &rmsnorm_fwd);
  m.impl("rmsnorm_bwd", &rmsnorm_bwd);
  m.impl("segmented_mean", &segmented_mean);
  m.impl("copy2d_batched", &copy2d_batched);
  m.impl("transpose2d", &transpose2d);
  m.impl("gemm8", &gemm8);
  m.impl("gemm8_tail", &gemm8_tail);
  m.impl("gemm8_rope", &gemm8_rope);
  m.impl("gemm8_rope_tail", &gemm8_rope_tail);
  m.impl("gemm8_swiglu", &gemm8_swiglu);
  m.impl("gemm8_sq", &gemm8_sq);
  m.impl("gemm8_swiglu_bwd", &gemm8_swiglu_bwd);
  m.impl("ce_inv_count", &ce_inv_count);
  m.impl("ce_chunk", &ce_chunk);
  m.impl("ce_chunk_f32", &ce_chunk_f32);
  m.impl("prefetch", &prefetch);
  m.impl("sqnorm", &sqnorm);
  m.impl("swiglu_fwd", &swiglu_fwd);
  m.impl("swiglu_bwd", &swiglu_bwd);
  m.impl("swiglu_bwd_m", &swiglu_bwd_m);
  m.impl("adamw_step", &adamw_step);
  m.impl("split_master", &split_master);
  m.impl("join_master", &join_master);
  m.impl("embedding_fwd", &embedding_fwd);
  m.impl("embedding_bwd", &embedding_bwd);
  m.impl("embedding_bwd_sorted", &embedding_bwd_sorted);
  m.impl("ce_fwd_bwd", &ce_fwd_bwd);
  m.impl("rope_split", &rope_split);
  m.impl("rope_merge_bwd", &rope_merge_bwd);
  m.impl("attn_fwd", &attn_fwd);
  m.impl("attn_bwd", &attn_bwd);
  m.impl("attn_bwd_rope", &attn_bwd_rope);
  m.impl("rope_append", &rope_append);
  m.impl("decode_attn_partials", &decode_attn_partials);
  m.impl("skinny_merge_linear", &skinny_merge_linear);
  m.impl("decode_attn", &decode_attn);
  m.impl("prefill_attn_paged", &prefill_attn_paged);
  m.impl("kv8_quant_rows", &kv8_quant_rows);
  m.impl("rope_append_kv8", &rope_append_kv8);
  m.impl("decode_attn_kv8", &decode_attn_kv8);
  m.impl("spec_accept", &spec_accept);
  m.impl("verify_attn", &verify_attn);
  m.impl("verify_attn_kv8", &verify_attn_kv8);
  m.impl("sample", &sample);
  m.impl("sample_rows", &sample_rows);
  m.impl("sample_temp_rows", &sample_temp_rows);
  m.impl("logits_adjust_rows", &logits_adjust_rows);
  m.impl("token_state_update", &token_state_update);
  m.impl("logprob_rows", &logprob_rows);
  m.impl("w8_linear", &w8_linear);
  m.impl("skinny_linear", &skinny_linear);
  m.impl("skinny_linear_swiglu", &skinny_linear_swiglu);
  m.impl("skinny_qkv_rope", &skinny_qkv_rope);
  m.impl("skinny_norm_linear", &skinny_norm_linear);
  m.impl("w8_dequant", &w8_dequant);
  m.impl("w4_linear", &w4_linear);
  m.impl("w4_dequant", &w4_dequant);
  m.impl("quant_rows_e4m3", &quant_rows_e4m3);
  m.impl("lora_xwt", &lora_xwt);
  m.impl("swiglu_lora", &swiglu_lora);
  m.impl("lora_grads", &lora_grads);
  m.impl("lora_gather_shrink", &lora_gather_shrink);
  m.impl("lora_gather_expand_add_", &lora_gather_expand_add_);
}
```

csrc/bindings.h:

```cpp
#pragma once
#include <hip/hip_runtime.h>
#include <stddef.h>
#include <stdint.h>

#include "kernels/attn_args.h"
#include "kernels/gemm8_args.h"
#include "kernels/prefill_paged_args.h"
#include "kernels/skinny_args.h"
#include "kernels/verify_args.h"
#include "kernels/w4_args.h"

extern "C" {
int mx_attn_bwd_partial_heads(mx::AbLaunch& L);
int mx_attn_bwd(const mx::AbLaunch& L, float scale, hipStream_t stream);

int mx_attn_fwd(const mx::AfLaunch& L, float scale, hipStream_t stream);

int mx_ce_fwd_bwd(uint16_t* logits, const int64_t* labels, float* losses, float* inv_n, float* loss_out, int64_t T,
                  int V, int64_t ignore, hipStream_t stream);
int mx_ce_inv_count(const int64_t* labels, int64_t T, int V, int64_t ignore, float* inv_n, hipStream_t stream);
int mx_ce_chunk(uint16_t* logits, const int64_t* labels, float* losses, const float* inv_n, int64_t T, int V,
                int64_t ignore, hipStream_t stream);
int mx_ce_chunk_f32(const float* logits, uint16_t* dl, const int64_t* labels, float* losses, const float* inv_n,
                    int64_t T, int V, int64_t ignore, hipStream_t stream);

int mx_rope_append(const uint16_t* qkv, const float* cosb, const float* sinb, const int32_t* pos, const int32_t* slots,
                   uint16_t* q, uint16_t* kc, uint16_t* vc, int B, int Hq, int Hkv, int D, int max_seq,
                   const int32_t* bt, int maxb, hipStream_t stream);
int mx_decode_attn(const uint16_t* q, const uint16_t* kc, const uint16_t* vc, const int32_t* lens, int len_off,
                   const int32_t* slots, float* part_ml, float* part_o, uint16_t* out, int B, int Hq, int Hkv, int D,
                   int max_seq, int nsplit, float scale, const int32_t* bt, int maxb, unsigned int* cnt,
                   hipStream_t stream);
int mx_kv8_quant_rows(const uint16_t* x, int64_t ldx, uint8_t* q, float* s, int64_t R, hipStream_t stream);
int mx_rope_append_kv8(const uint16_t* qkv, const float* cosb, const float* sinb, const int32_t* pos,
                       const int32_t* slots, uint16_t* q, uint8_t* kq, float* ks, uint8_t* vq, float* vs, int B, int Hq,
                       int Hkv, int max_seq, const int32_t* bt, int maxb, hipStream_t stream);
int mx_decode_attn_kv8(const uint16_t* q, const uint8_t* kq, const float* ks, const uint8_t* vq, const float* vs,
                       const int32_t* lens, int len_off, const int32_t* slots, float* part_ml, float* part_o,
                       uint16_t* out, int B, int Hq, int Hkv, int max_seq, int nsplit, float scale, const int32_t* bt,
                       int maxb, hipStream_t stream);
int mx_verify_attn(const mx::VfLaunch& L, float scale, hipStream_t stream);
int64_t mx_sample_ws_floats(int B);
int mx_sample(const void* logits, int is_bf16, int64_t* out, int B, int V, float temperature, uint32_t seed,
              uint32_t step, float* ws, hipStream_t stream);
int mx_sample_temp_rows(const void* logits, int is_bf16, int64_t* out, int B, int V, const float* temps,
                        const int64_t* seeds, const int32_t* steps, float* ws, hipStream_t stream);

int mx_swiglu_fwd(const uint16_t* gu, uint16_t* m, int64_t T, int F, int64_t ldm, hipStream_t stream);
int mx_swiglu_bwd(const uint16_t* dm, const uint16_t* gu, uint16_t* dgu, int64_t T, int F, int64_t ldg,
                  hipStream_t stream, uint16_t* m = nullptr);
int mx_adamw(float* p, void* g, int grad_bf16, float* m, float* v, uint16_t* lowp, int16_t* lo, int64_t n,
             float lr, float b1, float b2, float eps, float wd, float bc1, float bc2, const float* scale_t,
             float scale_f, int zero_grad, hipStream_t stream);
int mx_split_master(const float* x, uint16_t* hi, int16_t* lo, int64_t n, hipStream_t stream);
int mx_join_master(const uint16_t* hi, const int16_t* lo, float* x, int64_t n, hipStream_t stream);
int mx_embedding_fwd(const int64_t* ids, const uint16_t* w, uint16_t* out, int64_t T, int H, int64_t V,
                     hipStream_t stream);
int mx_embedding_bwd_sorted(const uint16_t* dy, const int64_t* sid, const int64_t* perm, int64_t T, int H,
                            int64_t V, void* out, int out_f32, float* ws, hipStream_t stream);
int mx_embedding_bwd(const int64_t* ids, const uint16_t* dy, float* dw, int64_t T, int H, int64_t V,
                     hipStream_t stream);

int mx_w8a16_gemm(const uint16_t* x, int64_t ldx, const uint8_t* q, const float* scale, uint16_t* y, int64_t ldy,
                  int M, int N, int K, hipStream_t stream);
int mx_quant_rows_e4m3(const uint16_t* x, int64_t ldx, uint8_t* q, float* s, int64_t M, int K, hipStream_t stream);
int mx_w8_dequant(const uint8_t* q, const float* scale, uint16_t* w, int64_t N, int K, hipStream_t stream);

int mx_w4a16_gemm(const mx::W4Launch& L, hipStream_t stream);
int mx_w4_dequant(const uint8_t* codes, const uint8_t* scales, uint16_t* w, int64_t N, int64_t K, hipStream_t stream);

int mx_gemm8(const uint16_t* A, int64_t lda, int a_kc, const uint16_t* B, int64_t ldb, int b_kc, void* C,
             int64_t ldc, int out_f32, int M, int N, int K, float beta, const float* alpha_t, float alpha_f,
             int ph, hipStream_t stream);
int mx_gemm8_epi(const uint16_t* A, int64_t lda, const uint16_t* B, int64_t ldb, uint16_t* C, int64_t ldc, int M,
                 int N, int K, mx::G8EpiMode mode, mx::G8Epi ep, hipStream_t stream);
int mx_gemm8_sq(const uint16_t* A, int64_t lda, int a_kc, const uint16_t* B, int64_t ldb, int b_kc, uint16_t* C,
                int64_t ldc, int M, int N, int K, const float* alpha_t, float alpha_f, float* sq, hipStream_t stream);
int mx_gemm8_tail(const uint16_t* A, int64_t lda, int a_kc, const uint16_t* B, int64_t ldb, int b_kc, uint16_t* C,
                  int64_t ldc, int M, int N, int K, int rows, int at, float* ws, int ph, hipStream_t stream,
                  float* sq = nullptr);
int mx_gemm8_rope_tail(const uint16_t* A, int64_t lda, const uint16_t* B, int64_t ldb, int M, int N, int K, int at,
                       float* ws, mx::G8Epi ep, hipStream_t stream);
int mx_gemm8_stamps(unsigned long long* host);

int mx_logits_adjust_rows(const void* logits, int is_bf16, float* out, int B, int V, const int32_t* state,
                          const int32_t* slots, int n_slots, const float* presence, const float* frequency,
                          const float* repetition, const float* bias, hipStream_t stream);
int mx_token_state_update(int32_t* state, const int32_t* slots, const int64_t* ids, int B, int V, int n_slots,
                          hipStream_t stream);
int64_t mx_logprob_ws_bytes(int B, int V);
int mx_logprob_rows(const void* logits, int is_bf16, const int64_t* ids, const int32_t* n_top, float* chosen_lp,
                    int32_t* top_ids, float* top_lp, int B, int V, void* ws, hipStream_t stream);

int64_t mx_swiglu_lora_ws(int T, int F, int nrb);
int mx_swiglu_lora(int bwd, const uint16_t* gu, const uint16_t* dm, uint16_t* out, int64_t ldo, const uint16_t* V,
                   int64_t ldv, int nrb, int pad, float alpha, float* ws, int T, int F, hipStream_t stream);
int64_t mx_lora_xwt_ws(int M, int K, int rows);
int64_t mx_lora_xtg_ws(int ntiles, int T);
int mx_lora_xwt(const uint16_t* X, int64_t ldx, const uint16_t* V, int64_t ldv, int Vrows, uint16_t* out, int64_t ldo,
                float* ws, int M, int K, float alpha, int rows, hipStream_t stream);
int mx_lora_xtg(const int64_t* desc, int np, int T, float alpha, int accumulate, float* ws, hipStream_t stream);

int mx_lora_serve_ksplits(int K);
int mx_lora_gather_shrink(const uint16_t* x, int64_t ldx, const int32_t* ids, const uint16_t* a_tab, float* part,
                          int M, int K, int R, int n_adapters, hipStream_t stream);
int mx_lora_gather_expand_add(uint16_t* y, int64_t ldy, const float* part, const int32_t* ids, const uint16_t* b_tab,
                              const float* s_tab, int M, int N, int KS, int r_max, const int* splits, int n_splits,
                              int n_adapters, hipStream_t stream);

int mx_copy2d_batched(const int64_t* desc, int n, int64_t total_blocks, hipStream_t stream);
int mx_segmented_mean_i32(const int32_t* codes, const int64_t* offs, float* out, int nseg,
                          hipStream_t stream);
int mx_sqnorm(const void* x, int bf16, int64_t n, float* out, float* work, hipStream_t stream);
int mx_transpose16(const void* in, void* out, int64_t R, int64_t C, int64_t ld_in, int64_t ld_out,
                   const float* scale, hipStream_t stream);
int mx_prefetch(const void* p, int64_t bytes, int wgs, hipStream_t stream);

size_t mx_peer_staging_bytes(int world, int wgs, int slot_bytes);
size_t mx_peer_staging_bytes2(int world, int wgs, int slot_bytes, int64_t light_cap);
int mx_peer_collective_light(int mode, int dtype, int wire, char* const* lbases, const void* in, void* out,
                             int64_t n, int64_t m, int rank, int world, int wgs, int64_t light_cap,
                             uint32_t* epoch, int* err, long long timeout_ticks, hipStream_t stream);
int mx_peer_collective(int mode, int dtype, char* const* bases, const void* in, void* out, int64_t n,
                       int64_t m, int rank, int world, int wgs, int slot_bytes, uint32_t* epochs, int* err,
                       long long timeout_ticks, hipStream_t stream);

int mx_prefill_attn_paged(const mx::PpLaunch& L, float scale, hipStream_t stream);

int mx_rmsnorm_fwd(const uint16_t* x, const uint16_t* res, const uint16_t* w, uint16_t* y,
                   uint16_t* h_out, float* rstd, int T, int H, int ldy, float eps, hipStream_t stream);
int mx_rmsnorm_bwd(const uint16_t* dy, const uint16_t* x, const uint16_t* w, const float* rstd,
                   const uint16_t* dres, uint16_t* dx, float* dwp, int T, int H, int ldr, int ldx, int rpb,
                   hipStream_t stream);
int mx_colsum_f32(const float* p, float* out, int nblk, int H, hipStream_t stream);

int mx_rope_split(const uint16_t* qkv, const float* cosb, const float* sinb, const int32_t* positions, uint16_t* q,
                  uint16_t* k, uint16_t* v, int B, int S, int Hq, int Hkv, int D, hipStream_t stream);
int mx_rope_merge_bwd(const float* dq, const float* dkp, const float* dvp, const float* cosb, const float* sinb,
                      uint16_t* dqkv, int B, int S, int Hq, int Hkv, int kv_heads_in, int D, int64_t ldq,
                      hipStream_t stream, int head0);

int mx_sample_rows(const void* logits, int is_bf16, int64_t* out, int B, int V, const float* temps,
                   const float* top_ps, const int32_t* top_ks, const int64_t* seeds, const int32_t* steps,
                   hipStream_t stream);

int mx_spec_accept(const int64_t* drawn, const int64_t* tokens, const int32_t* nq, int32_t* out, int B, int n,
                   hipStream_t stream);

int mx_skinny(const mx::SkLaunch& L, hipStream_t stream);

int mx_xgmi_allreduce(uint32_t* const* flags, float* const* data, const float* in, float* out, int n,
                      int rank, int world, uint32_t epoch, int max_elems, int op, int* err,
                      long long timeout_ticks, hipStream_t stream);
int mx_xgmi_allreduce_bf16(uint32_t* const* flags, uint16_t* const* data, const uint16_t* in,
                           uint16_t* out, int n, int rank, int world, int max_elems, uint32_t* epochs,
                           int* err, long long timeout_ticks, hipStream_t stream);
}
```

csrc/kernels/lora.hip:

```cpp
#include "bindings.h"
#include "common.h"
#include <stdlib.h>
#include <string.h>

namespace mx {

namespace {

typedef __bf16 lbf16x8_t __attribute__((ext_vector_type(8)));
typedef __attribute__((address_space(1))) const void* lgptr_t;
typedef __attribute__((address_space(3))) void* llptr_t;

__device__ __forceinline__ f32x4 lmfma(const u16x8& a, const u16x8& b, const f32x4& c) {
  return __builtin_amdgcn_mfma_f32_16x16x32_bf16(__builtin_bit_cast(lbf16x8_t, a), __builtin_bit_cast(lbf16x8_t, b),
                                                 c, 0, 0, 0);
}

constexpr int kRS = 68;
constexpr int kMaxTiles = 16384;

__device__ unsigned int g_xwt_cnt[kMaxTiles];
__device__ unsigned int g_xtg_cnt[kMaxTiles];

__device__ __forceinline__ bool arrive_last(unsigned int* cnt, int S, int* s_flag) {
// ... 453 lines not shown
      for (int ks = 0; ks < 2; ++ks) {
        const u16x8 bf = u16x8{gr[ks][0][0], gr[ks][0][1], gr[ks][0][2], gr[ks][0][3],
                               gr[ks][1][0], gr[ks][1][1], gr[ks][1][2], gr[ks][1][3]};
#pragma unroll
        for (int i = 0; i < 4; ++i) {
          const u16x8 af = u16x8{xr[ks][0][i][0], xr[ks][0][i][1], xr[ks][0][i][2], xr[ks][0][i][3],
                                 xr[ks][1][i][0], xr[ks][1][i][1], xr[ks][1][i][2], xr[ks][1][i][3]};
          acc[i][0] = lmfma(af, bf, acc[i][0]);
        }
      }
    };
    if (b0 < b1) issue3(b0, 0);
    if (b0 + 1 < b1) issue3(b0 + 1, 1);
    if (b0 + 2 < b1) issue3(b0 + 2, 2);
    for (int b = b0; b < b1; b += 3) {
      block3(std::integral_constant<int, 0>{}, b);
      if (b + 1 < b1) block3(std::integral_constant<int, 1>{}, b + 1);
      if (b + 2 < b1) block3(std::integral_constant<int, 2>{}, b + 2);
    }
  }
  float* rw = reinterpret_cast<float*>(wreg);
#pragma unroll
  for (int i = 0; i < 4; ++i)
#pragma unroll
    for (int j = 0; j < 4; ++j) {
      if (j >= JB) continue;
#pragma unroll
      for (int e = 0; e < 4; ++e) rw[(16 * i + 4 * g + e) * kRS + 16 * j + c] = acc[i][j][e];
    }
  if (a.wt) {
    asm volatile("s_waitcnt lgkmcnt(0)" ::: "memory");
    __builtin_amdgcn_wave_barrier();
    const int J = 16 * JB, nel = 64 * J;
    const bool jfast = P.os_j == 1;
    for (int e = lane; e < nel; e += 64) {
      const int n = jfast ? e / J : (e & 63), j = jfast ? e % J : (e >> 6);
      uint16_t* o = P.out + (int64_t)(n0 + n) * P.os_n + (int64_t)j * P.os_j;
      const float r = a.alpha * rw[n * kRS + j] + (a.accumulate ? bf2f(*o) : 0.f);
      *o = f2bf(r);
    }
    return;
  }
  __syncthreads();
  const int J = 16 * JB, nel = 64 * J;
  const bool jfast = P.os_j == 1;
  float v[16];
#pragma unroll
  for (int q = 0; q < 16; ++q) {
    const int e = tid + 256 * q;
    v[q] = 0.f;
    if (e < nel) {
      const int n = jfast ? e / J : (e & 63), j = jfast ? e % J : (e >> 6);
      float s = 0.f;
#pragma unroll
      for (int ww = 0; ww < 4; ++ww) s += reinterpret_cast<const float*>(smem + ww * WREG)[n * kRS + j];
      v[q] = s;
    }
  }
  if (a.S > 1) {
    float* wp = ws + ((int64_t)split * a.ntiles + tile) * 4096;
    if (!a.fused_red) {
#pragma unroll
      for (int q = 0; q < 16; ++q)
        if (tid + 256 * q < nel) wp[tid + 256 * q] = v[q];
      return;
    }
#pragma unroll
    for (int q = 0; q < 16; ++q)
      if (tid + 256 * q < nel) __hip_atomic_store(wp + tid + 256 * q, v[q], __ATOMIC_RELAXED, __HIP_MEMORY_SCOPE_AGENT);
    if (!arrive_last_sc1(&g_xtg_cnt[tile], a.S, &s_last)) return;
#pragma unroll
    for (int q = 0; q < 16; ++q) {
      const int e = tid + 256 * q;
      if (e < nel) {
        float s = __hip_atomic_load(ws + (int64_t)tile * 4096 + e, __ATOMIC_RELAXED, __HIP_MEMORY_SCOPE_AGENT);
        for (int sp = 1; sp < a.S; ++sp)
          s += __hip_atomic_load(ws + ((int64_t)sp * a.ntiles + tile) * 4096 + e, __ATOMIC_RELAXED,
                                 __HIP_MEMORY_SCOPE_AGENT);
        v[q] = s;
      }
    }
  }
#pragma unroll
  for (int q = 0; q < 16; ++q) {
    const int e = tid + 256 * q;
    if (e < nel) {
      const int n = jfast ? e / J : (e & 63), j = jfast ? e % J : (e >> 6);
      uint16_t* o = P.out + (int64_t)(n0 + n) * P.os_n + (int64_t)j * P.os_j;
      const float r = a.alpha * v[q] + (a.accumulate ? bf2f(*o) : 0.f);
      *o = f2bf(r);
    }
  }
}

__global__ void __launch_bounds__(256) lora_xtg_reduce_kernel(const XtgArgs a, const float* __restrict__ ws) {
  const int tile = blockIdx.x, tid = threadIdx.x;
  XtgProb P = a.p[0];
#pragma unroll
  for (int i = 1; i < kMaxProb; ++i)
    if (i < a.np && tile >= a.p[i].tile0) P = a.p[i];
  const int n0 = (tile - P.tile0) * 64, J = 16 * P.JB, nel = 64 * J;
  const bool jfast = P.os_j == 1;
  for (int e = tid; e < nel; e += 256) {
    float s = ws[(int64_t)tile * 4096 + e];
    for (int sp = 1; sp < a.S; ++sp) s += ws[((int64_t)sp * a.ntiles + tile) * 4096 + e];
    const int n = jfast ? e / J : (e & 63), j = jfast ? e % J : (e >> 6);
    uint16_t* o = P.out + (int64_t)(n0 + n) * P.os_n + (int64_t)j * P.os_j;
    *o = f2bf(a.alpha * s + (a.accumulate ? bf2f(*o) : 0.f));
  }
}

constexpr int kSlRow = 136;

__device__ __forceinline__ float sl_sigmoid(float x) { return __builtin_amdgcn_rcpf(1.f + __expf(-x)); }

template <bool BWD, int NRB, int RBW>
__global__ void __launch_bounds__(256) swiglu_lora_kernel(const uint16_t* __restrict__ gu,
                                                          const uint16_t* __restrict__ dm, uint16_t* __restrict__ out,
                                                          int64_t ldo, const uint16_t* __restrict__ V, int64_t ldv,
                                                          float* __restrict__ ws, int F, int CS) {
  constexpr int NP = BWD ? 2 : 1;
  constexpr int NC = 16 * NRB;
  __shared__ __attribute__((aligned(16))) uint16_t img[2][NP][RBW][16 * kSlRow];
  __shared__ __attribute__((aligned(16))) float red[4][16][NC + 4];
  const int rg = blockIdx.x, split = blockIdx.y, tid = threadIdx.x;
  const int lane = tid & 63, w = tid >> 6, r = lane & 15, gq = lane >> 4;
  const int row = tid >> 4, ch = tid & 15;
  const int tiles = F >> 7;
  const int t0 = (int)((int64_t)split * tiles / CS), t1 = (int)((int64_t)(split + 1) * tiles / CS);
  const int64_t tok = (int64_t)rg * 16 * RBW + row;
  const uint16_t* grow = gu + tok * (2 * (int64_t)F) + 8 * ch;
  const uint16_t* drow = dm + tok * (int64_t)F + 8 * ch;
  uint16_t* orow = out + tok * ldo + 8 * ch;
  const int64_t gstep = 16 * (2 * (int64_t)F), dstep = 16 * (int64_t)F, ostep = 16 * ldo;
  const uint16_t* vrow = V + (int64_t)r * ldv + 32 * w + 8 * gq;
  const int wofs = row * kSlRow + 8 * ch, rofs = r * kSlRow + 32 * w + 8 * gq;

  f32x4 acc[RBW][NRB];
#pragma unroll
  for (int i = 0; i < RBW; ++i)
#pragma unroll
    for (int b = 0; b < NRB; ++b) acc[i][b] = f32x4{0.f, 0.f, 0.f, 0.f};

  u16x8 g[RBW], u[RBW], d[RBW], vf[NP][NRB];
  auto vload = [&](int t) {
#pragma unroll
    for (int p = 0; p < NP; ++p)
#pragma unroll
      for (int b = 0; b < NRB; ++b)
        vf[p][b] = *reinterpret_cast<const u16x8*>(vrow + (int64_t)(16 * b) * ldv + p * F + (t << 7));
  };
  auto load = [&](int t, u16x8(&g_)[RBW], u16x8(&u_)[RBW], u16x8(&d_)[RBW]) {
    const int c = t << 7;
#pragma unroll
    for (int i = 0; i < RBW; ++i) {
      g_[i] = *reinterpret_cast<const u16x8*>(grow + i * gstep + c);
      u_[i] = *reinterpret_cast<const u16x8*>(grow + i * gstep + F + c);
      if (BWD) d_[i] = *reinterpret_cast<const u16x8*>(drow + i * dstep + c);
    }
  };
  if (t0 < t1) {
    load(t0, g, u, d);
    vload(t0);
  }
  for (int t = t0; t < t1; ++t) {
    const int c = t << 7, buf = (t - t0) & 1;
    u16x8 gn[RBW], un[RBW], dn[RBW];
    load(t + 1 < t1 ? t + 1 : t, gn, un, dn);
#pragma unroll
    for (int i = 0; i < RBW; ++i) {
      u16x8 o0, o1;
      if (!BWD) {
#pragma unroll
        for (int j = 0; j < 8; ++j) {
          const float gf = bf2f(g[i][j]);
          o0[j] = f2bf(gf * sl_sigmoid(gf) * bf2f(u[i][j]));
        }
        *reinterpret_cast<u16x8*>(orow + i * ostep + c) = o0;
        *reinterpret_cast<u16x8*>(&img[buf][0][i][wofs]) = o0;
      } else {
#pragma unroll
        for (int j = 0; j < 8; ++j) {
          const float gf = bf2f(g[i][j]), uf = bf2f(u[i][j]), df = bf2f(d[i][j]);
          float dg, du;
          swiglu_grad(df, gf, uf, dg, du);
          o0[j] = f2bf(dg);
          o1[j] = f2bf(du);
        }
        *reinterpret_cast<u16x8*>(orow + i * ostep + c) = o0;
        *reinterpret_cast<u16x8*>(orow + i * ostep + F + c) = o1;
        *reinterpret_cast<u16x8*>(&img[buf][0][i][wofs]) = o0;
        *reinterpret_cast<u16x8*>(&img[buf][NP - 1][i][wofs]) = o1;
      }
    }
    __syncthreads();
#pragma unroll
    for (int i = 0; i < RBW; ++i)
#pragma unroll
      for (int p = 0; p < NP; ++p) {
        const u16x8 a = *reinterpret_cast<const u16x8*>(&img[buf][p][i][rofs]);
#pragma unroll
        for (int b = 0; b < NRB; ++b) acc[i][b] = lmfma(a, vf[p][b], acc[i][b]);
      }
    vload(t + 1 < t1 ? t + 1 : t);
#pragma unroll
    for (int i = 0; i < RBW; ++i) {
      g[i] = gn[i], u[i] = un[i];
      if (BWD) d[i] = dn[i];
    }
  }
#pragma unroll
  for (int i = 0; i < RBW; ++i) {
    __syncthreads();
#pragma unroll
    for (int b = 0; b < NRB; ++b)
#pragma unroll
      for (int e = 0; e < 4; ++e) red[w][4 * gq + e][16 * b + r] = acc[i][b][e];
    __syncthreads();
    float* wp = ws + ((int64_t)split * (gridDim.x * RBW) + rg * RBW + i) * (16 * NC);
    for (int k = tid; k < 16 * NC; k += 256) {
      const int rr = k / NC, cc = k % NC;
      wp[k] = ((red[0][rr][cc] + red[1][rr][cc]) + red[2][rr][cc]) + red[3][rr][cc];
    }
  }
}

__global__ void __launch_bounds__(256) swiglu_lora_reduce_kernel(const float* __restrict__ ws, int CS, int NC, int pad,
                                                                 uint16_t* __restrict__ tail, int64_t ldo, float alpha) {
  const int rb = blockIdx.x, nrb = gridDim.x;
  for (int i = threadIdx.x; i < 16 * pad; i += 256) {
    const int rr = i / pad, cc = i % pad;
    float v = 0.f;
    if (cc < NC)
      for (int sp = 0; sp < CS; ++sp) v += ws[(((int64_t)sp * nrb + rb) * 16 + rr) * NC + cc];
    tail[((int64_t)rb * 16 + rr) * ldo + cc] = f2bf(alpha * v);
  }
}

template <int NRB, int RBW>
__global__ void __launch_bounds__(256) lora_xwt_tile_kernel(const uint16_t* __restrict__ X, int64_t ldx,
                                                            const uint16_t* __restrict__ V, int64_t ldv,
                                                            float* __restrict__ ws, int K, int CS) {
  constexpr int NC = 16 * NRB;
  __shared__ __attribute__((aligned(16))) uint16_t img[2][RBW][16 * kSlRow];
  __shared__ __attribute__((aligned(16))) float red[4][16][NC + 4];
  const int rg = blockIdx.x, split = blockIdx.y, tid = threadIdx.x;
  const int lane = tid & 63, w = tid >> 6, r = lane & 15, gq = lane >> 4;
  const int row = tid >> 4, ch = tid & 15;
  const int tiles = K >> 7;
  const int t0 = (int)((int64_t)split * tiles / CS), t1 = (int)((int64_t)(split + 1) * tiles / CS);
  const uint16_t* xrow = X + ((int64_t)rg * 16 * RBW + row) * ldx + 8 * ch;
  const int64_t xstep = 16 * ldx;
  const uint16_t* vrow = V + (int64_t)r * ldv + 32 * w + 8 * gq;
  const int wofs = row * kSlRow + 8 * ch, rofs = r * kSlRow + 32 * w + 8 * gq;

  f32x4 acc[RBW][NRB];
#pragma unroll
  for (int i = 0; i < RBW; ++i)
#pragma unroll
    for (int b = 0; b < NRB; ++b) acc[i][b] = f32x4{0.f, 0.f, 0.f, 0.f};
  u16x8 x[RBW], vf[NRB];
  auto xload = [&](int t, u16x8(&dst)[RBW]) {
#pragma unroll
    for (int i = 0; i < RBW; ++i) dst[i] = *reinterpret_cast<const u16x8*>(xrow + i * xstep + (t << 7));
  };
  auto vload = [&](int t) {
#pragma unroll
    for (int b = 0; b < NRB; ++b) vf[b] = *reinterpret_cast<const u16x8*>(vrow + (int64_t)(16 * b) * ldv + (t << 7));
  };
  if (t0 < t1) {
    xload(t0, x);
    vload(t0);
  }
  for (int t = t0; t < t1; ++t) {
    const int buf = (t - t0) & 1;
    u16x8 xn[RBW];
    xload(t + 1 < t1 ? t + 1 : t, xn);
#pragma unroll
    for (int i = 0; i < RBW; ++i) *reinterpret_cast<u16x8*>(&img[buf][i][wofs]) = x[i];
    __syncthreads();
#pragma unroll
    for (int i = 0; i < RBW; ++i) {
      const u16x8 a = *reinterpret_cast<const u16x8*>(&img[buf][i][rofs]);
#pragma unroll
      for (int b = 0; b < NRB; ++b) acc[i][b] = lmfma(a, vf[b], acc[i][b]);
    }
    vload(t + 1 < t1 ? t + 1 : t);
#pragma unroll
    for (int i = 0; i < RBW; ++i) x[i] = xn[i];
  }
#pragma unroll
  for (int i = 0; i < RBW; ++i) {
    __syncthreads();
#pragma unroll
    for (int b = 0; b < NRB; ++b)
#pragma unroll
      for (int e = 0; e < 4; ++e) red[w][4 * gq + e][16 * b + r] = acc[i][b][e];
    __syncthreads();
    float* wp = ws + ((int64_t)split * (gridDim.x * RBW) + rg * RBW + i) * (16 * NC);
    for (int k = tid; k < 16 * NC; k += 256) {
      const int rr = k / NC, cc = k % NC;
      wp[k] = ((red[0][rr][cc] + red[1][rr][cc]) + red[2][rr][cc]) + red[3][rr][cc];
    }
  }
}

}

using namespace mx;

static int lora_env(const char* name, int dflt);

static int swiglu_lora_rbw(int T) {
  int rbw = lora_env("MXLLM_SWIGLU_LORA_RBW", 2);
  rbw = rbw >= 4 ? 4 : (rbw >= 2 ? 2 : 1);
  while (rbw > 1 && (T / 16) % rbw) rbw >>= 1;
  return rbw;
}

static int swiglu_lora_splits(int T, int F) {
  const int tiles = F / 128, rbs = T / (16 * swiglu_lora_rbw(T));
  int cs = lora_env("MXLLM_SWIGLU_LORA_CS", 0);
  if (cs <= 0) cs = (512 + rbs - 1) / rbs;
  cs = cs < 1 ? 1 : cs;
  cs = cs > tiles ? tiles : cs;
  return cs > 32 ? 32 : cs;
}

extern "C" int64_t mx_swiglu_lora_ws(int T, int F, int nrb) {
  if (T <= 0 || F < 128) return 0;
  return (int64_t)swiglu_lora_splits(T, F) * T * 16 * nrb;
}

extern "C" int mx_swiglu_lora(int bwd, const uint16_t* gu, const uint16_t* dm, uint16_t* out, int64_t ldo,
                              const uint16_t* V, int64_t ldv, int nrb, int pad, float alpha, float* ws, int T, int F,
                              hipStream_t stream) {
  if (T <= 0) return 0;
  if (T % 16 || F % 128 || nrb < 1 || nrb > 4 || pad < 16 * nrb || pad % 8 || ldo % 8 || ldv % 8 ||
      ldo < (bwd ? 2 * (int64_t)F : F) + pad || ((uintptr_t)gu | (uintptr_t)out | (uintptr_t)V) % 16 ||
      (bwd && (!dm || (uintptr_t)dm % 16)))
    return (int)hipErrorInvalidValue;
  const int CS = swiglu_lora_splits(T, F), RBW = swiglu_lora_rbw(T);
  const dim3 grid(T / (16 * RBW), CS);
#define MX_SL_R(B, N, R) swiglu_lora_kernel<B, N, R><<<grid, 256, 0, stream>>>(gu, dm, out, ldo, V, ldv, ws, F, CS)
#define MX_SL(B, N)                                 \
  do {                                              \
    if (RBW == 4) MX_SL_R(B, N, 4);                 \
    else if (RBW == 2) MX_SL_R(B, N, 2);            \
    else MX_SL_R(B, N, 1);                          \
  } while (0)
  if (bwd) {
    switch (nrb) { case 1: MX_SL(true, 1); break; case 2: MX_SL(true, 2); break;
                   case 3: MX_SL(true, 3); break; default: MX_SL(true, 4); break; }
  } else {
    switch (nrb) { case 1: MX_SL(false, 1); break; case 2: MX_SL(false, 2); break;
                   case 3: MX_SL(false, 3); break; default: MX_SL(false, 4); break; }
  }
#undef MX_SL
#undef MX_SL_R
  swiglu_lora_reduce_kernel<<<T / 16, 256, 0, stream>>>(ws, CS, 16 * nrb, pad, out + (bwd ? 2 * (int64_t)F : F), ldo,
                                                        alpha);
  return (int)hipGetLastError();
}

static int lora_env(const char* name, int dflt) {
  const char* v = getenv(name);
  return v && *v ? atoi(v) : dflt;
}
static int lora_splits(int tiles, int blocks, int smax) {
  if (tiles <= 0) return 1;
  const int target = lora_env("MXLLM_LORA_WGS", 256);
  int S = (target + tiles - 1) / tiles;
  S = S < 1 ? 1 : (S > smax ? smax : S);
  while (S > 1 && blocks / (4 * S) < 2) --S;
  return S;
}

static bool xtg_wave_tiles(int ntiles) {
  return lora_env("MXLLM_LORA_XTG_WT", 1) == 1 && ntiles >= lora_env("MXLLM_LORA_XTG_WT_MIN", 1024);
}

static int xwt_mode() {
  const char* kv = getenv("MXLLM_LORA_XWT");
  if (kv && !strcmp(kv, "reg")) return 2;
  if (kv && !strcmp(kv, "tile")) return 0;
  return 1;
}
static bool xwt_tile_ok(const void* X, int64_t ldx, const void* V, int64_t ldv, int M, int K, int rows) {
  return xwt_mode() == 0 && M % 16 == 0 && K % 128 == 0 && rows > 0 && rows <= 64 && ldx % 8 == 0 &&
         ldv % 8 == 0 && (uintptr_t)X % 16 == 0 && (uintptr_t)V % 16 == 0;
}
static int xwt_rbw(int M) { return M % 64 == 0 ? 4 : (M % 32 == 0 ? 2 : 1); }
static int xwt_tile_splits(int M, int K) {
  const int groups = M / (16 * xwt_rbw(M)), tiles = K / 128;
  int cs = lora_env("MXLLM_LORA_XWT_CS", 0);
  if (cs <= 0) cs = (512 + groups - 1) / groups;
  cs = cs < 1 ? 1 : cs;
  return cs > tiles ? tiles : cs;
}

extern "C" int64_t mx_lora_xwt_ws(int M, int K, int rows) {
  const int S = M >= 64 && K >= 64 ? lora_splits(M / 64, K / 64, 16) : 1;
  const int64_t dma = S > 1 ? (int64_t)S * (M / 64) * 4096 : 0;
  if (rows > 0 && rows <= 64 && M % 16 == 0 && K % 128 == 0 && xwt_mode() == 0) {
    const int64_t tile = (int64_t)xwt_tile_splits(M, K) * M * 16 * ((rows + 15) / 16);
    return tile > dma ? tile : dma;
  }
  return dma;
}
extern "C" int64_t mx_lora_xtg_ws(int ntiles, int T) {
  if (xtg_wave_tiles(ntiles)) return 0;
  const int S = lora_splits(ntiles, T / 64, 8);
  return S > 1 ? (int64_t)S * ntiles * 4096 : 0;
}

extern "C" int mx_lora_xwt(const uint16_t* X, int64_t ldx, const uint16_t* V, int64_t ldv, int Vrows, uint16_t* out,
                           int64_t ldo, float* ws, int M, int K, float alpha, int rows, hipStream_t stream) {
  if (M <= 0) return 0;
  if (xwt_tile_ok(X, ldx, V, ldv, M, K, rows) && rows <= Vrows && ldo % 4 == 0) {
    const int nrb = (rows + 15) / 16, rbw = xwt_rbw(M), CS = xwt_tile_splits(M, K);
    const dim3 grid(M / (16 * rbw), CS);
#define MX_XT(N, R) lora_xwt_tile_kernel<N, R><<<grid, 256, 0, stream>>>(X, ldx, V, ldv, ws, K, CS)
#define MX_XT_N(R)                                  \
  switch (nrb) {                                    \
    case 1: MX_XT(1, R); break;                     \
    case 2: MX_XT(2, R); break;                     \
    case 3: MX_XT(3, R); break;                     \
    default: MX_XT(4, R); break;                    \
  }
    if (rbw == 4) { MX_XT_N(4) } else if (rbw == 2) { MX_XT_N(2) } else { MX_XT_N(1) }
#undef MX_XT_N
#undef MX_XT
    swiglu_lora_reduce_kernel<<<M / 16, 256, 0, stream>>>(ws, CS, 16 * nrb, Vrows, out, ldo, alpha);
    return (int)hipGetLastError();
  }
  if (M % 64 || K % 64 || Vrows % 64 || M / 64 > kMaxTiles) return (int)hipErrorInvalidValue;
  const int mtiles = M / 64, S = lora_splits(mtiles, K / 64, 16);
  const int fused = lora_env("MXLLM_LORA_FUSED_RED", 0);
  const bool lds = xwt_mode() != 2 && ((uintptr_t)X % 16 == 0) && ((uintptr_t)V % 16 == 0) && ldx % 8 == 0 &&
                   ldv % 8 == 0;
  for (int c0 = 0; c0 < Vrows; c0 += 64) {
    if (lds)
      lora_xwt_lds_kernel<<<dim3(mtiles, S), 256, 0, stream>>>(X, ldx, V + (int64_t)c0 * ldv, ldv, out + c0, ldo, ws,
                                                               M, K, S, alpha, fused);
    else
      lora_xwt_kernel<<<dim3(mtiles, S), 256, 0, stream>>>(X, ldx, V + (int64_t)c0 * ldv, ldv, out + c0, ldo, ws, M,
                                                           K, S, alpha, fused);
    if (S > 1 && !fused) {
      const int qpw = lora_env("MXLLM_LORA_XWT_RED_ROWS", 16) >= 64 ? 4 : 1;
      lora_xwt_reduce_kernel<<<(4 / qpw) * mtiles, 256, 0, stream>>>(ws, S, mtiles, out + c0, ldo, alpha, qpw);
    }
  }
  return (int)hipGetLastError();
}

extern "C" int mx_lora_xtg(const int64_t* desc, int np, int T, float alpha, int accumulate, float* ws,
                           hipStream_t stream) {
  if (np <= 0 || np > kMaxProb || T % 64) return (int)hipErrorInvalidValue;
  if (T == 0) return 0;
  XtgArgs a{};
  int ntiles = 0;
  for (int i = 0; i < np; ++i) {
    const int64_t* d = desc + i * 10;
    XtgProb& p = a.p[i];
    p.X = reinterpret_cast<const uint16_t*>(d[0]);
    p.G = reinterpret_cast<const uint16_t*>(d[1]);
    p.out = reinterpret_cast<uint16_t*>(d[2]);
    p.ldx = d[3], p.ldg = d[4], p.os_n = d[5], p.os_j = d[6];
    p.Nx = (int)d[7], p.jb0 = (int)d[8], p.JB = (int)d[9];
    if (p.Nx <= 0 || p.Nx % 64 || p.JB < 1 || p.JB > 4) return (int)hipErrorInvalidValue;
    p.tile0 = ntiles;
    ntiles += p.Nx / 64;
  }
  if (ntiles > kMaxTiles) return (int)hipErrorInvalidValue;
  a.np = np, a.T = T, a.ntiles = ntiles, a.alpha = alpha;
  a.wt = xtg_wave_tiles(ntiles);
  a.S = a.wt ? 1 : lora_splits(ntiles, T / 64, 8);
  a.accumulate = accumulate;
  a.fused_red = a.wt ? 0 : lora_env("MXLLM_LORA_FUSED_RED", 0);
  a.narrow3 = lora_env("MXLLM_LORA_XTG_STAGES", 3) == 3;
  lora_xtg_kernel<<<dim3(a.wt ? (ntiles + 3) / 4 : ntiles, a.S), 256, 0, stream>>>(a, ws);
  if (a.S > 1 && !a.fused_red) lora_xtg_reduce_kernel<<<ntiles, 256, 0, stream>>>(a, ws);
  return (int)hipGetLastError();
}
```

mxllm/models/llama.py:

```python
from __future__ import annotations

import math
import os

import torch
import torch.nn as nn
import torch.utils.checkpoint as ckpt

from .. import ops
from ..ops import fused
from ..ops import reference as ref
from .config import LlamaConfig


class FusedLinear(nn.Module):

    def __init__(self, in_features: int, splits: list[int], *, dtype, device, lora_r: int = 0,
                 lora_alpha: float = 16.0, train_base: bool = True, dx_image: bool = False,
                 transposed: bool = False):
        super().__init__()
        self.in_features = in_features
        self.splits = list(splits)
        N = sum(splits)
        self.lora_r = lora_r
        self.pad = 0
        self.transposed = False
        if lora_r > 0:
            n = len(splits)
            self.scaling = lora_alpha / lora_r
            self.pad = (n * lora_r + 63) // 64 * 64
            self.transposed = transposed and not train_base
            shape = (in_features + self.pad, N + self.pad) if self.transposed else (N + self.pad, in_features + self.pad)
            self.register_buffer("wbuf", torch.zeros(*shape, dtype=dtype, device=device), persistent=False)
            self.register_buffer("wbt", torch.zeros(self.pad, N, dtype=dtype, device=device), persistent=False)
            if self.transposed:
                self.register_buffer("wa", torch.zeros(self.pad, in_features, dtype=dtype, device=device),
                                     persistent=False)
            if dx_image and not train_base and not self.transposed:
                self.register_buffer("wxt", torch.zeros(in_features, N + self.pad, dtype=dtype, device=device),
                                     persistent=False)
            w = self.wbuf[:in_features, :N].t() if self.transposed else self.wbuf[:N, :in_features]
            self.weight = nn.Parameter(w, requires_grad=train_base)
            self.lora_a = nn.Parameter(torch.empty(n * lora_r, in_features, dtype=dtype, device=device))
            self.lora_b = nn.Parameter(torch.zeros(N, n * lora_r, dtype=dtype, device=device))
        else:
            self.weight = nn.Parameter(torch.empty(N, in_features, dtype=dtype, device=device),
                                       requires_grad=train_base)

    def lora_b_blocks(self):
        out, off = [], 0
        for i, n_i in enumerate(self.splits):
            out.append(self.lora_b[off:off + n_i, i * self.lora_r:(i + 1) * self.lora_r])
            off += n_i
        return out

    def augmented(self) -> bool:
        return (self.lora_r > 0 and hasattr(self, "wbuf")
                and self.weight.data_ptr() == self.wbuf.data_ptr() and self.weight.dtype == self.wbuf.dtype)

    def adapter_copies(self):
        N, K, R = sum(self.splits), self.in_features, self.lora_a.shape[0]
        if self.transposed:
            return [(self.lora_a.data, self.wbuf[:K, N:N + R].t()), (self.lora_b.data, self.wbuf[K:K + R, :N].t()),
                    (self.lora_b.data, self.wbt[:R, :N].t()), (self.lora_a.data, self.wa[:R, :K])]
        out = [(self.lora_a.data, self.wbuf[N:N + R, :K]), (self.lora_b.data, self.wbuf[:N, K:K + R]),
               (self.lora_b.data, self.wbt[:R, :N].t())]
        if getattr(self, "wxt", None) is not None:
            out.append((self.lora_a.data, self.wxt[:, N:N + R].t()))
        return out

    @torch.no_grad()
    def refresh_images_(self):
        if getattr(self, "wxt", None) is not None and self.augmented():
            K = self.in_features
            self.wxt.copy_(ops.transpose2d(self.wbuf[:, :K]))

    @torch.no_grad()
    def sync_adapter_(self):
        for src, dst in self.adapter_copies():
            dst.copy_(src)

    @torch.no_grad()
    def reset_parameters(self, std: float, gen: torch.Generator | None):
        self.weight.normal_(0.0, std, generator=gen)
        if self.lora_r > 0:
            bound = 1.0 / math.sqrt(self.in_features)
            self.lora_a.uniform_(-bound, bound, generator=gen)
            self.lora_b.zero_()
            if self.augmented():
                self.sync_adapter_()
                self.refresh_images_()

    def tail_operands(self):
        R = self.lora_a.shape[0]
        amat = self.wa if self.transposed else self.wbuf[sum(self.splits):, :self.in_features]
        return (amat, R, self.scaling), (self.wbt, R, self.scaling)

    def forward(self, x: torch.Tensor, x_tail: bool = False, dy_tail: bool = False) -> torch.Tensor:
        if self.lora_r > 0:
            if self.augmented():
                return ops.lora_linear_aug(x, self.lora_a, self.lora_b, self.wbuf, self.splits, self.scaling,
                                           self.pad, self.wbt, getattr(self, "wxt", None),
                                           getattr(self, "wa", None) if self.transposed else None,
                                           x_tail=x_tail, dy_tail=dy_tail)
            return ops.lora_linear(x, self.weight, self.lora_a, self.lora_b, self.splits, self.scaling)
        return ops.linear(x, self.weight)


DX_IMAGE = tuple(x for x in os.environ.get("MXLLM_DX_IMAGE", "qkv,d").split(",") if x)
LORA_T = tuple(x for x in os.environ.get("MXLLM_LORA_T", "").split(",") if x)
RECOMPUTE_SWIGLU = os.environ.get("MXLLM_RECOMPUTE_SWIGLU", "auto")
RECOMPUTE_NORM = os.environ.get("MXLLM_RECOMPUTE_NORM", "auto")
REC_FUSED = os.environ.get("MXLLM_REC_FUSED", "1") != "0"


class LlamaLayer(nn.Module):
    def __init__(self, cfg: LlamaConfig, *, dtype, device, lora_r: int, lora_alpha: float, train_base: bool):
        super().__init__()
        kw = dict(dtype=dtype, device=device, lora_r=lora_r, lora_alpha=lora_alpha, train_base=train_base)
        h = cfg.hidden
        self.attn_norm = nn.Parameter(torch.ones(h, dtype=dtype, device=device), requires_grad=train_base)
        self.mlp_norm = nn.Parameter(torch.ones(h, dtype=dtype, device=device), requires_grad=train_base)
        self.wqkv = FusedLinear(h, [cfg.q_dim, cfg.kv_dim, cfg.kv_dim], dx_image="qkv" in DX_IMAGE,
                                transposed="qkv" in LORA_T, **kw)
        self.wo = FusedLinear(cfg.q_dim, [h], dx_image="o" in DX_IMAGE, transposed="o" in LORA_T, **kw)
        self.wgu = FusedLinear(h, [cfg.ffn, cfg.ffn], dx_image="gu" in DX_IMAGE, transposed="gu" in LORA_T, **kw)
        self.wd = FusedLinear(cfg.ffn, [h], dx_image="d" in DX_IMAGE, transposed="d" in LORA_T, **kw)


def ckpt_layer(setting: bool | int | None, i: int) -> bool:
    if isinstance(setting, bool) or setting is None:
        return bool(setting)
    return i < int(setting)


class Llama(nn.Module):
    def __init__(self, cfg: LlamaConfig, *, device=None, dtype=torch.bfloat16, lora_r: int = 0,
                 lora_alpha: float = 16.0, seed: int = 0, init: bool = True,
                 activation_checkpointing: bool | int = False):
        super().__init__()
        device = torch.device(device) if device is not None else torch.device("cpu")
        self.cfg = cfg
        self.lora = lora_r > 0
        train_base = not self.lora
        self.activation_checkpointing = activation_checkpointing
        self.mlp_recompute_ckpt = None
        self.seq_parallel = None
        self.param_wait = None
        self.tok_emb = nn.Parameter(torch.empty(cfg.vocab_size, cfg.hidden, dtype=dtype, device=device),
                                    requires_grad=train_base)
        self.layers = nn.ModuleList([
            LlamaLayer(cfg, dtype=dtype, device=device, lora_r=lora_r, lora_alpha=lora_alpha, train_base=train_base)
            for _ in range(cfg.n_layers)])
        self.final_norm = nn.Parameter(torch.ones(cfg.hidden, dtype=dtype, device=device), requires_grad=train_base)
        if cfg.tie_embeddings:
            self.lm_head = None
            self.tok_emb._mx_no_direct = True
        else:
            self.lm_head = nn.Parameter(torch.empty(cfg.vocab_size, cfg.hidden, dtype=dtype, device=device),
                                        requires_grad=train_base)
        cos, sin = ref.rope_tables(min(cfg.max_seq_len, 131072), cfg.head_dim, cfg.rope_theta, cfg.rope_scaling)
        self.register_buffer("rope_cos", cos.to(device), persistent=False)
        self.register_buffer("rope_sin", sin.to(device), persistent=False)
        if init:
            self.reset_parameters(seed)

    @torch.no_grad()
    def reset_parameters(self, seed: int = 0):
        dev = self.tok_emb.device
        gen = torch.Generator(device=dev)
        gen.manual_seed(seed)
        std = 0.02
        self.tok_emb.normal_(0.0, std, generator=gen)
        for layer in self.layers:
            for lin in (layer.wqkv, layer.wo, layer.wgu, layer.wd):
                lin.reset_parameters(std, gen)
        if self.lm_head is not None:
            self.lm_head.normal_(0.0, std, generator=gen)

    @property
    def head_weight(self) -> torch.Tensor:
        return self.tok_emb if self.lm_head is None else self.lm_head

    @staticmethod
    def _pad(lin) -> int:
        return lin.pad if lin.augmented() else 0

    def _layer(self, i: int, x: torch.Tensor, h: torch.Tensor, B: int, S: int):
        cfg = self.cfg
        layer = self.layers[i]
        rec = self._recompute_m(layer, i)
        rec_x = rec and RECOMPUTE_NORM != "0"
        lora_at = (ops.lora_qkv_attention_at(x, layer.wqkv, B, S, cfg.n_heads, cfg.n_kv_heads, cfg.head_dim)
                   if self.seq_parallel is None and layer.wqkv.lora_r and not rec_x else 0)
        if (self.seq_parallel is None and not layer.wqkv.lora_r
                and fused.qkv_attention_ok(x, layer.wqkv.weight, B, S, cfg.n_heads, cfg.n_kv_heads, cfg.head_dim)):
            o = fused.qkv_attention(x, layer.wqkv.weight, self.rope_cos, self.rope_sin, B, S, cfg.n_heads,
                                    cfg.n_kv_heads, cfg.head_dim, causal=True, out_pad=self._pad(layer.wo),
                                    norm=(h, layer.attn_norm, cfg.norm_eps) if rec_x else None)
            qkv = None
        elif lora_at:
            o = ops.lora_qkv_attention(x, layer.wqkv, self.rope_cos, self.rope_sin, B, S, cfg.n_heads,
                                       cfg.n_kv_heads, cfg.head_dim, lora_at, causal=True, out_pad=self._pad(layer.wo))
            qkv = None
        else:
            qkv = (ops.normed_linear(x, h, layer.attn_norm, cfg.norm_eps, layer.wqkv.weight) if rec_x
                   else layer.wqkv(x))
        if qkv is None:
            pass
        elif self.seq_parallel is not None:
            o = self.seq_parallel(qkv, self.rope_cos, self.rope_sin, B, S, cfg.n_heads, cfg.n_kv_heads,
                                  cfg.head_dim, causal=True)
        else:
            o = ops.attention_block(qkv, self.rope_cos, self.rope_sin, B, S, cfg.n_heads, cfg.n_kv_heads,
                                    cfg.head_dim, causal=True, out_pad=self._pad(layer.wo),
                                    grad_pad=self._pad(layer.wqkv))
        a = layer.wo(o)
        x, h = ops.add_rms_norm(a, h, layer.mlp_norm, cfg.norm_eps, out_pad=self._pad(layer.wgu),
                                grad_pad=self._pad(layer.wo))
        if rec and REC_FUSED and fused.gate_up_swiglu_down_ok(x, layer.wgu.weight, layer.wd.weight):
            d = fused.gate_up_swiglu_down(x, layer.wgu.weight, layer.wd.weight,
                                          norm=(h, layer.mlp_norm, cfg.norm_eps) if rec_x else None, recompute_m=True)
        elif rec:
            gu = ops.normed_linear(x, h, layer.mlp_norm, cfg.norm_eps, layer.wgu.weight) if rec_x else layer.wgu(x)
            d = ops.swiglu_linear(gu, layer.wd.weight)
        elif (not layer.wgu.lora_r and not layer.wd.lora_r
              and fused.gate_up_swiglu_down_ok(x, layer.wgu.weight, layer.wd.weight)):
            d = fused.gate_up_swiglu_down(x, layer.wgu.weight, layer.wd.weight)
        elif not layer.wgu.lora_r and fused.gate_up_swiglu_ok(x, layer.wgu.weight):
            m = fused.gate_up_swiglu(x, layer.wgu.weight, out_pad=self._pad(layer.wd))
            d = layer.wd(m)
        else:
            tf, tb = self._swiglu_tails(layer, x)
            m = ops.swiglu(layer.wgu(x, dy_tail=tb is not None), out_pad=self._pad(layer.wd),
                           grad_pad=self._pad(layer.wgu), tail_fwd=tf, tail_bwd=tb)
            d = layer.wd(m, x_tail=tf is not None)
        last = i + 1 == len(self.layers)
        nxt = self.final_norm if last else self.layers[i + 1].attn_norm
        x, h = ops.add_rms_norm(d, h, nxt, cfg.norm_eps, out_pad=0 if last else self._pad(self.layers[i + 1].wqkv),
                                grad_pad=self._pad(layer.wd))
        return x, h

    def _recompute_m(self, layer, i: int) -> bool:
        if (RECOMPUTE_SWIGLU == "0" or any(lin.lora_r > 0 for lin in (layer.wqkv, layer.wgu, layer.wd))
                or not self.training or not torch.is_grad_enabled()):
            return False
        if RECOMPUTE_SWIGLU == "1":
            return True
        ck = self.mlp_recompute_ckpt if self.mlp_recompute_ckpt is not None else self.activation_checkpointing
        return not isinstance(ck, bool) and ck is not None and not ckpt_layer(ck, i)

    def _swiglu_tails(self, layer, x: torch.Tensor):
        if x.dim() != 2:
            return None, None
        T, F2 = x.shape[0], 2 * self.cfg.ffn
        tf = tb = None
        if layer.wd.augmented() and ops.lora_tail_ok(x, T, F2, layer.wd.pad, layer.wd.lora_a.shape[0]):
            tf = layer.wd.tail_operands()[0]
        if layer.wgu.augmented() and ops.lora_tail_ok(x, T, F2, layer.wgu.pad, layer.wgu.lora_a.shape[0]):
            tb = layer.wgu.tail_operands()[1]
        return tf, tb

    def _wait_groups(self):
        if getattr(self, "_wgroups", None) is None:
            L = len(self.layers)
            g = [[self.tok_emb] + ([self.layers[0].attn_norm] if L else [])]
            for i, layer in enumerate(self.layers):
                nxt = self.final_norm if i + 1 == L else self.layers[i + 1].attn_norm
                g.append(list(layer.parameters()) + [nxt])
            g.append([self.final_norm] + ([self.lm_head] if self.lm_head is not None else []))
            self._wgroups = g
        return self._wgroups

    def hidden_states(self, ids: torch.Tensor) -> torch.Tensor:
        B, S = ids.shape
        wait = self.param_wait
        groups = self._wait_groups() if wait is not None else None
        if wait is not None:
            wait(groups[0])
        h = ops.embedding(ids.reshape(-1), self.tok_emb)
        x = (ops.rms_norm(h, self.layers[0].attn_norm, self.cfg.norm_eps, out_pad=self._pad(self.layers[0].wqkv))
             if len(self.layers) else h)
        for i in range(len(self.layers)):
            if wait is not None:
                wait(groups[i + 1])
            if ckpt_layer(self.activation_checkpointing, i) and self.training and torch.is_grad_enabled():
                x, h = ckpt.checkpoint(self._layer, i, x, h, B, S, use_reentrant=False)
            else:
                x, h = self._layer(i, x, h, B, S)
        if not len(self.layers):
            x = ops.rms_norm(h, self.final_norm, self.cfg.norm_eps)
        if wait is not None:
            wait(groups[-1])
        return x

    def forward(self, ids: torch.Tensor, labels: torch.Tensor | None = None, ignore_index: int = -100):
        B, S = ids.shape
        x = self.hidden_states(ids)
        if labels is not None:
            return ops.linear_cross_entropy(x, self.head_weight, labels.reshape(-1), ignore_index)
        return torch.matmul(x, self.head_weight.t()).view(B, S, -1)

    @torch.no_grad()
    def sync_adapters_(self) -> None:
        lins = [m for m in self.modules() if isinstance(m, FusedLinear) and m.augmented()]
        if not lins:
            return
        pairs = [p for m in lins for p in m.adapter_copies()]
        if not pairs[0][0].is_cuda or not ops.native_available():
            for src, dst in pairs:
                dst.copy_(src)
            return
        key = tuple((s.data_ptr(), d.data_ptr()) for s, d in pairs)
        if getattr(self, "_adapter_desc_key", None) != key:
            from ..ops.linear import copy2d_plan

            rows, total = copy2d_plan(pairs)
            self._adapter_desc = torch.tensor(rows, dtype=torch.int64, device=pairs[0][0].device)
            self._adapter_blocks = total
            self._adapter_desc_key = key
        ops.native().copy2d_batched(self._adapter_desc, self._adapter_blocks)

    @torch.no_grad()
    def refresh_images_(self) -> None:
        for m in self.modules():
            if isinstance(m, FusedLinear):
                m.refresh_images_()

    def set_sequence_parallel(self, group) -> None:
        if group is None:
            self.seq_parallel = None
            return
        from ..parallel.sequence import UlyssesAttention

        self.seq_parallel = UlyssesAttention(group)

    def set_context_parallel(self, group) -> None:
        if group is None:
            self.seq_parallel = None
            return
        from ..parallel.context import RingAttention

        self.seq_parallel = RingAttention(group)

    def trainable_parameters(self):
        return [p for p in self.parameters() if p.requires_grad]

    def named_trainable_parameters(self):
        return [(n, p) for n, p in self.named_parameters() if p.requires_grad]

    def num_params(self, trainable_only: bool = False) -> int:
        return sum(p.numel() for p in (self.trainable_parameters() if trainable_only else self.parameters()))
```

mxllm/ops/__init__.py:

```python
from ._ext import available as native_available, native, use_native
from .norm import rms_norm, add_rms_norm
from .attention import attention_block
from .activation import lora_tail_ok, swiglu
from .loss import linear_cross_entropy, cross_entropy
from .optim import SplitMaster, adamw_step_, sq_norm
from .embedding import embedding
from .linear import linear, lora_linear, lora_linear_aug, lora_qkv_attention, lora_qkv_attention_at, linear_swiglu, merge_linear_ok, norm_linear, normed_linear, qkv_rope_linear, qkv_rope_ok, swiglu_linear, transpose2d
from .lora_serve import AdapterTables, lora_delta_rows_
from . import reference
```

mxllm/ops/activation.py:

```python
from __future__ import annotations

import os

import torch

from . import reference as ref
from ._ext import native, use_native


class _SwiGLUFn(torch.autograd.Function):
    @staticmethod
    def forward(ctx, gu, out_pad, grad_pad, tail_fwd, tail_bwd):
        ctx.save_for_backward(gu)
        ctx.grad_pad = grad_pad
        ctx.tail_bwd = tail_bwd
        if tail_fwd is not None:
            v, nrb, s = tail_fwd
            return native().swiglu_lora(None, gu, out_pad, v, nrb, s)
        return native().swiglu_fwd(gu, out_pad)

    @staticmethod
    def backward(ctx, dm):
        (gu,) = ctx.saved_tensors
        if ctx.tail_bwd is not None:
            v, nrb, s = ctx.tail_bwd
            dgu = native().swiglu_lora(dm.contiguous(), gu, ctx.grad_pad, v, nrb, s)
        else:
            dgu = native().swiglu_bwd(dm.contiguous(), gu, ctx.grad_pad)
        return dgu, None, None, None, None


def lora_tail_ok(x: torch.Tensor, T: int, F2: int, pad: int, R: int) -> bool:
    return (_FUSE_TAIL and use_native(x) and x.dtype == torch.bfloat16 and T % 16 == 0 and F2 % 256 == 0
            and R % 16 == 0 and 16 <= R <= 64 and R <= pad and pad % 8 == 0)


_FUSE_TAIL = os.environ.get("MXLLM_SWIGLU_LORA", "1") != "0"


def swiglu(gate_up: torch.Tensor, out_pad: int = 0, grad_pad: int = 0, tail_fwd=None, tail_bwd=None) -> torch.Tensor:
    if use_native(gate_up):
        if gate_up.dim() != 2:
            out_pad = grad_pad = 0
            tail_fwd = tail_bwd = None
        tf = (tail_fwd[0], tail_fwd[1] // 16, float(tail_fwd[2])) if tail_fwd is not None else None
        tb = (tail_bwd[0], tail_bwd[1] // 16, float(tail_bwd[2])) if tail_bwd is not None else None
        return _SwiGLUFn.apply(gate_up.contiguous(), out_pad, grad_pad, tf, tb)
    return ref.swiglu(gate_up)
```

mxllm/ops/linear.py:

```python
from __future__ import annotations

import math
import os
from typing import Sequence

import torch
import torch.nn.functional as F

from ..parallel.grad_ready import direct_grad, direct_grad32, mark_ready
from . import gemm
from ._ext import native, use_native


class _LoRALinearFn(torch.autograd.Function):
    @staticmethod
    def forward(ctx, x, w, a, b, scaling, splits, r):
        x2 = x.reshape(-1, x.shape[-1])
        t = torch.matmul(x2, a.t())
        y = torch.empty(x2.shape[0], w.shape[0], dtype=x.dtype, device=x.device)
        y.addmm_(t, b.t(), beta=0.0, alpha=scaling)
        y.addmm_(x2, w.t())
        ctx.save_for_backward(x2, w, a, b, t)
        ctx.scaling, ctx.splits, ctx.r, ctx.xshape = scaling, tuple(splits), r, x.shape
        return y.view(*x.shape[:-1], w.shape[0])

    @staticmethod
    def backward(ctx, dy):
        x2, w, a, b, t = ctx.saved_tensors
        s, r = ctx.scaling, ctx.r
        dy2 = dy.reshape(-1, dy.shape[-1])
        g = torch.empty(dy2.shape[0], a.shape[0], dtype=dy2.dtype, device=dy2.device)
        g.addmm_(dy2, b, beta=0.0, alpha=s)
        ga, gb = direct_grad(a) if ctx.needs_input_grad[2] else None, direct_grad(b) if ctx.needs_input_grad[3] else None
        da = db = None
        if ctx.needs_input_grad[2]:
            if ga is not None:
                ga.addmm_(g.t(), x2)
                mark_ready(a)
            else:
                da = torch.matmul(g.t(), x2)
        if ctx.needs_input_grad[3]:
            tgt = gb if gb is not None else torch.zeros_like(b)
            off = 0
            for i, n_i in enumerate(ctx.splits):
                tgt[off:off + n_i, i * r:(i + 1) * r].addmm_(dy2[:, off:off + n_i].t(), t[:, i * r:(i + 1) * r],
                                                            beta=1.0 if gb is not None else 0.0, alpha=s)
                off += n_i
            if gb is not None:
                mark_ready(b)
            else:
                db = tgt
        dx = torch.matmul(g, a)
        dx.addmm_(dy2, w)
        return dx.view(ctx.xshape), None, da, db, None, None, None


def _padded_rows(t: torch.Tensor, pad: int) -> torch.Tensor | None:
    if t.dim() != 2 or t.stride(1) != 1 or t.stride(0) != t.shape[1] + pad:
        return None
    st = t.untyped_storage()
    need = (t.storage_offset() + t.shape[0] * t.stride(0)) * t.element_size()
    if st.nbytes() < need:
        return None
    full = torch.empty(0, dtype=t.dtype, device=t.device)
    full.set_(st, t.storage_offset(), (t.shape[0], t.shape[1] + pad), (t.stride(0), 1))
    return full


def _augment(t: torch.Tensor, pad: int) -> torch.Tensor:
    full = _padded_rows(t, pad)
    if full is None:
        full = torch.empty(t.shape[0], t.shape[1] + pad, dtype=t.dtype, device=t.device)
        full[:, :t.shape[1]].copy_(t)
    return full


_LORA_KERNELS = os.environ.get("MXLLM_LORA_KERNELS", "1") != "0"


def _lora_native(x2: torch.Tensor, N: int, K: int, splits, r: int, wbt) -> bool:
    return (_LORA_KERNELS and wbt is not None and use_native(x2) and x2.shape[0] % 64 == 0 and K % 64 == 0 and r % 16 == 0
            and r <= 64 and all(n % 64 == 0 for n in splits) and x2.dtype == torch.bfloat16)


def _lora_aug_backward(ctx, xa, wbuf, dy, dy_tail: bool, need_a: bool, need_b: bool):
    N, K, s, splits, r, pad, xshape, nat, tr = ctx.dims
    R = r * len(splits)
    dy2 = dy.reshape(-1, N)
    dya = _padded_rows(dy2, pad) if dy_tail else None
    if dya is None:
        dya = _augment(dy2, pad)
        if nat:
            native().lora_xwt(dy2, ctx.wbt, dya[:, N:], s, len(splits) * r)
        else:
            bmat = wbuf[K:, :N].t() if tr else wbuf[:N, K:]
            dya[:, N:].addmm_(dy2, bmat, beta=0.0, alpha=s)
    g = dya[:, N:N + R]
    x2, st = xa[:, :K], xa[:, K:K + R]
    da = db = None
    ga = direct_grad(ctx.lora_a) if need_a else None
    gb = direct_grad(ctx.lora_b) if need_b else None
    if nat and need_a and need_b:
        acc = ga is not None and gb is not None
        tga = ga if acc else torch.empty(R, K, dtype=dy2.dtype, device=dy2.device)
        tgb = gb if acc else torch.zeros(N, R, dtype=dy2.dtype, device=dy2.device)
        native().lora_grads(x2, dy2, dya[:, N:], xa[:, K:], tga, tgb, list(splits), r, acc)
        if acc:
            mark_ready(ctx.lora_a)
            mark_ready(ctx.lora_b)
        else:
            da, db = tga, tgb
    else:
        if need_a:
            if ga is not None:
                ga.addmm_(g.t(), x2)
                mark_ready(ctx.lora_a)
            else:
                da = torch.mm(g.t(), x2)
        if need_b:
            tgt = gb if gb is not None else torch.zeros(N, R, dtype=dy2.dtype, device=dy2.device)
            off = 0
            for i, n_i in enumerate(splits):
                tgt[off:off + n_i, i * r:(i + 1) * r].addmm_(dy2[:, off:off + n_i].t(), st[:, i * r:(i + 1) * r],
                                                            beta=1.0 if gb is not None else 0.0)
                off += n_i
            if gb is not None:
                mark_ready(ctx.lora_b)
            else:
                db = tgt
    if tr:
        dx = gemm.mm("tn", dya, wbuf[:K, :])
    elif ctx.wxt is not None:
        dx = gemm.mm("tn", dya, ctx.wxt)
    else:
        dx = gemm.mm("nn", dya, wbuf[:, :K])
    return dx.view(xshape), da, db


class _LoRAAugFn(torch.autograd.Function):

    @staticmethod
    def forward(ctx, x, a, b, wbuf, scaling, splits, r, pad, wbt, wxt=None, wa=None, x_tail=False, dy_tail=False):
        tr = wa is not None
        if tr:
            K, N = wbuf.shape[0] - pad, wbuf.shape[1] - pad
        else:
            N, K = wbuf.shape[0] - pad, wbuf.shape[1] - pad
        x2 = x.reshape(-1, K)
        nat = _lora_native(x2, N, K, splits, r, wbt)
        xa = _padded_rows(x2, pad) if x_tail else None
        if xa is None:
            xa = _augment(x2, pad)
            amat = wa if tr else wbuf[N:, :K]
            if nat:
                native().lora_xwt(x2, amat, xa[:, K:], scaling, a.shape[0])
            else:
                xa[:, K:].addmm_(x2, amat.t(), beta=0.0, alpha=scaling)
        y = gemm.mm("nn", xa, wbuf[:, :N]) if tr else gemm.mm("tn", xa, wbuf[:N, :])
        ctx.save_for_backward(xa, wbuf)
        ctx.lora_a, ctx.lora_b, ctx.wbt, ctx.wxt = a, b, wbt, wxt
        ctx.dims = (N, K, scaling, tuple(splits), r, pad, x.shape, nat, tr)
        ctx.dy_tail = dy_tail
        return y.view(*x.shape[:-1], N)

    @staticmethod
    def backward(ctx, dy):
        xa, wbuf = ctx.saved_tensors
        dx, da, db = _lora_aug_backward(ctx, xa, wbuf, dy, ctx.dy_tail, ctx.needs_input_grad[1],
                                        ctx.needs_input_grad[2])
        return dx, da, db, None, None, None, None, None, None, None, None, None, None


def lora_linear_aug(x: torch.Tensor, a: torch.Tensor, b: torch.Tensor, wbuf: torch.Tensor, splits: Sequence[int],
                    scaling: float, pad: int, wbt: torch.Tensor | None = None,
                    wxt: torch.Tensor | None = None, wa: torch.Tensor | None = None,
                    x_tail: bool = False, dy_tail: bool = False) -> torch.Tensor:
    r = a.shape[0] // len(splits)
    return _LoRAAugFn.apply(x, a, b, wbuf, scaling, tuple(splits), r, pad, wbt, wxt, wa, bool(x_tail), bool(dy_tail))


_LORA_QKV_ROPE = os.environ.get("MXLLM_LORA_QKV_ROPE", "1") != "0"


def lora_qkv_attention_at(x: torch.Tensor, lin, B: int, S: int, Hq: int, Hkv: int, D: int) -> int:
    if not (_LORA_QKV_ROPE and lin.lora_r > 0 and lin.augmented() and not lin.transposed and D == 128
            and S % 256 == 0 and use_native(x) and x.dtype == torch.bfloat16 and not gemm.deterministic()):
        return 0
    N, K, pad = sum(lin.splits), lin.in_features, lin.pad
    x2 = x.reshape(-1, x.shape[-1])
    if N != (Hq + 2 * Hkv) * D or x2.shape[0] != B * S or x2.shape[1] != K:
        return 0
    xa = _padded_rows(x2, pad)
    if xa is None or not gemm.schedule("tn", B * S, N, K + pad, torch.bfloat16):
        return 0
    at = gemm.tail_at("tn", B * S, N, K + pad, torch.bfloat16)
    return at if at > 0 and gemm.g8_rope_takes(xa, lin.wbuf[:N, :], S, Hq, Hkv, at) else 0


def _lora_aug_input(x2, a, wbuf, amat, scaling, N, K, pad, nat):
    xa = _augment(x2, pad)
    if nat:
        native().lora_xwt(x2, amat, xa[:, K:], scaling, a.shape[0])
    else:
        xa[:, K:].addmm_(x2, amat.t(), beta=0.0, alpha=scaling)
    return xa


class _LoRAQKVAttnFn(torch.autograd.Function):

    @staticmethod
    def forward(ctx, x, a, b, wbuf, scaling, splits, r, pad, wbt, wxt, cos, sin, B, S, Hq, Hkv, D, causal, out_pad,
                at):
        N, K = wbuf.shape[0] - pad, wbuf.shape[1] - pad
        x2 = x.reshape(-1, K)
        nat = _lora_native(x2, N, K, splits, r, wbt)
        xa = _lora_aug_input(x2, a, wbuf, wbuf[N:, :K], scaling, N, K, pad, nat)
        ops = native()
        q = torch.empty(B, Hq, S, D, dtype=x.dtype, device=x.device)
        k = torch.empty(B, Hkv, S, D, dtype=x.dtype, device=x.device)
        v = torch.empty_like(k)
        if not ops.gemm8_rope_tail(xa, wbuf[:N, :], cos, sin, B, S, Hq, Hkv, q, k, v, at):
            q, k, v = ops.rope_split(gemm.mm("tn", xa, wbuf[:N, :]), cos, sin, B, S, Hq, Hkv, D)
        o, lse = ops.attn_fwd(q, k, v, causal, 1.0 / math.sqrt(D), out_pad)
        ctx.save_for_backward(xa, wbuf, q, k, v, o, lse, cos, sin)
        ctx.lora_a, ctx.lora_b, ctx.wbt, ctx.wxt = a, b, wbt, wxt
        ctx.dims = (N, K, scaling, tuple(splits), r, pad, x.shape, nat, False)
        ctx.causal = causal
        return o.view(B * S, Hq * D)

    @staticmethod
    def backward(ctx, do):
        from .attention import backward_dqkv

        xa, wbuf, q, k, v, o, lse, cos, sin = ctx.saved_tensors
        pad = ctx.dims[5]
        dqkv = backward_dqkv(do, q, k, v, o, lse, cos, sin, ctx.causal, pad)
        del q, k, v, o, lse
        dx, da, db = _lora_aug_backward(ctx, xa, wbuf, dqkv, False, ctx.needs_input_grad[1], ctx.needs_input_grad[2])
        return (dx, da, db) + (None,) * 17


def lora_qkv_attention(x: torch.Tensor, lin, cos: torch.Tensor, sin: torch.Tensor, B: int, S: int, Hq: int,
                       Hkv: int, D: int, at: int, causal: bool = True, out_pad: int = 0) -> torch.Tensor:
    r = lin.lora_a.shape[0] // len(lin.splits)
    return _LoRAQKVAttnFn.apply(x, lin.lora_a, lin.lora_b, lin.wbuf, lin.scaling, tuple(lin.splits), r, lin.pad,
                                lin.wbt, getattr(lin, "wxt", None), cos, sin, B, S, Hq, Hkv, D, causal, out_pad, at)


def transpose2d(t: torch.Tensor, scale: torch.Tensor | None = None) -> torch.Tensor:
    if use_native(t):
        if t.stride(-1) != 1:
            t = t.contiguous()
        return native().transpose2d(t, scale)
    out = t.t().contiguous()
    return out if scale is None else (out * scale.to(out.dtype))


def copy2d_plan(pairs) -> tuple[list[list[int]], int]:
    rows, total = [], 0
    for s, d in pairs:
        assert s.shape == d.shape and s.dim() == 2 and s.element_size() == 2 and d.element_size() == 2
        r, c = s.shape
        rows.append([s.data_ptr(), d.data_ptr(), r, c, s.stride(0), d.stride(0), total, s.stride(1), d.stride(1)])
        if s.stride(1) == 1 and d.stride(0) == 1 and d.stride(1) != 1:
            total += ((r + 63) // 64) * ((c + 63) // 64)
        else:
            total += (r * c + 4095) // 4096
    return rows, total


_DW_TN = os.environ.get("MXLLM_DW_TN", "1") != "0"


def weight_grad_(out: torch.Tensor | None, dy: torch.Tensor, x: torch.Tensor, beta: float = 1.0,
                 dy_scale: torch.Tensor | None = None) -> torch.Tensor:
    f32 = out is not None and out.dtype == torch.float32 and dy.dtype != torch.float32
    if use_native(dy) and dy.dtype == torch.bfloat16 and x.dtype == torch.bfloat16:
        odt = out.dtype if out is not None else dy.dtype
        if gemm.want("tt", dy.shape[1], x.shape[1], dy.shape[0], odt):
            sc = None if dy_scale is None else dy_scale.reshape(1).float()
            return gemm.mm("tt", dy, x, out=out, beta=beta if out is not None else 0.0, alpha_t=sc,
                           out_dtype=odt)
    if _DW_TN and use_native(dy) and dy.dtype == torch.bfloat16 and x.dtype == torch.bfloat16:
        xt = transpose2d(x)
        dyt = transpose2d(dy, None if dy_scale is None else dy_scale.reshape(1).float())
        if out is None:
            return torch.mm(dyt, xt.t())
        if f32:
            return torch.ops.aten.addmm.dtype_out(out, dyt, xt.t(), torch.float32, beta=beta, out=out)
        return out.addmm_(dyt, xt.t(), beta=beta)
    if dy_scale is not None:
        dy = dy * dy_scale.to(dy.dtype)
    if out is None:
        return torch.mm(dy.t(), x)
    if f32:
        if dy.is_cuda:
            return torch.ops.aten.addmm.dtype_out(out, dy.t(), x, torch.float32, beta=beta, out=out)
        return out.addmm_(dy.t().float(), x.float(), beta=beta)
    return out.addmm_(dy.t(), x, beta=beta)


def param_weight_grad(wp: torch.Tensor | None, dy: torch.Tensor, x: torch.Tensor,
                      dy_scale: torch.Tensor | None = None) -> torch.Tensor | None:
    g = direct_grad(wp) if wp is not None else None
    if g is None and wp is not None:
        g = direct_grad32(wp)
    if g is None:
        return weight_grad_(None, dy, x, dy_scale=dy_scale)
    fresh = getattr(wp, "_mx_grad_fresh", False)
    armed = getattr(wp, "_mx_sq_done", None)
    sq = getattr(wp, "_mx_sq", None) if fresh and armed is False else None
    if sq is not None and g.dtype == dy.dtype == x.dtype == torch.bfloat16 and gemm.mm_sq(
            "tt", dy, x, g, sq, None if dy_scale is None else dy_scale.reshape(1).float()):
        wp._mx_sq_done = True
    else:
        if armed is True:
            wp._mx_sq_done = "dirty"
        weight_grad_(g, dy, x, beta=0.0 if fresh else 1.0, dy_scale=dy_scale)
    if fresh:
        wp._mx_grad_fresh = False
    mark_ready(wp)
    return None


class _LinearFn(torch.autograd.Function):

    @staticmethod
    def forward(ctx, x, w):
        x2 = x.reshape(-1, x.shape[-1])
        ctx.save_for_backward(x2, w)
        ctx.wp = w if w.is_leaf else None
        ctx.xshape = x.shape
        return gemm.mm("tn", x2, w).view(*x.shape[:-1], w.shape[0])

    @staticmethod
    def backward(ctx, dy):
        x2, w = ctx.saved_tensors
        dy2 = dy.reshape(-1, w.shape[0])
        dx = gemm.mm("nn", dy2, w).view(ctx.xshape) if ctx.needs_input_grad[0] else None
        dw = param_weight_grad(ctx.wp, dy2, x2) if ctx.needs_input_grad[1] else None
        return dx, dw


def _swiglu_nograd(gu: torch.Tensor) -> torch.Tensor:
    if use_native(gu):
        return native().swiglu_fwd(gu.contiguous(), 0)
    from . import reference as ref

    return ref.swiglu(gu)


class _SwiGLULinearFn(torch.autograd.Function):

    @staticmethod
    def forward(ctx, gu, w):
        g2 = gu.reshape(-1, gu.shape[-1])
        m = _swiglu_nograd(g2)
        ctx.save_for_backward(g2, w)
        ctx.wp = w if w.is_leaf else None
        ctx.gshape = gu.shape
        return gemm.mm("tn", m, w).view(*gu.shape[:-1], w.shape[0])

    @staticmethod
    def backward(ctx, dy):
        g2, w = ctx.saved_tensors
        dy2 = dy.reshape(-1, w.shape[0])
        dgu = dw = None
        if use_native(g2):
            from .fused import swiglu_bwd_gemm

            dgu, m = swiglu_bwd_gemm(dy2, w, g2, want_m=True)
            if ctx.needs_input_grad[1]:
                dw = param_weight_grad(ctx.wp, dy2, m)
            del m
        else:
            from . import reference as ref

            with torch.enable_grad():
                gr = g2.detach().requires_grad_(True)
                m = ref.swiglu(gr)
            if ctx.needs_input_grad[1]:
                dw = param_weight_grad(ctx.wp, dy2, m.detach())
            if ctx.needs_input_grad[0]:
                (dgu,) = torch.autograd.grad(m, gr, gemm.mm("nn", dy2, w))
        if dgu is not None and ctx.needs_input_grad[0]:
            dgu = dgu.view(ctx.gshape)
        else:
            dgu = None
        return dgu, dw


def swiglu_linear(gu: torch.Tensor, w: torch.Tensor) -> torch.Tensor:
    return _SwiGLULinearFn.apply(gu, w)


class _NormedLinearFn(torch.autograd.Function):

    @staticmethod
    def forward(ctx, x, h, nw, eps, w):
        x2 = x.reshape(-1, x.shape[-1])
        ctx.save_for_backward(h, nw, w)
        ctx.wp = w if w.is_leaf else None
        ctx.eps, ctx.xshape = eps, x.shape
        return gemm.mm("tn", x2, w).view(*x.shape[:-1], w.shape[0])

    @staticmethod
    def backward(ctx, dy):
        h, nw, w = ctx.saved_tensors
        dy2 = dy.reshape(-1, w.shape[0])
        dx = gemm.mm("nn", dy2, w).view(ctx.xshape) if ctx.needs_input_grad[0] else None
        dw = None
        if ctx.needs_input_grad[4]:
            h2 = h.reshape(-1, h.shape[-1])
            if use_native(h2):
                x2 = native().rmsnorm_fwd(h2.contiguous(), None, nw, ctx.eps, 0)[0]
            else:
                from . import reference as ref

                x2 = ref.rms_norm(h2, nw, ctx.eps)
            dw = param_weight_grad(ctx.wp, dy2, x2)
            del x2
        return dx, None, None, None, dw


def normed_linear(x: torch.Tensor, h: torch.Tensor, nw: torch.Tensor, eps: float, w: torch.Tensor) -> torch.Tensor:
    return _NormedLinearFn.apply(x, h, nw, eps, w)


def sk_takes(entry: str, M: int, N: int, K: int, ldx: int = 0, ldw: int = 0, ldy: int = 0, *, x=1, w=1, y=1,
             swiglu: bool = False, norm: bool = False, delta=0, ldd: int = 0, gamma=1, h_out=1, rope=None,
             merge=None, scale=1) -> bool:
    is_rope, is_merge, w8 = entry == "rope", entry == "merge", entry == "w8"
    norm = entry == "norm" or (is_rope and bool(norm))
    swiglu = entry == "swiglu" or (entry == "norm" and bool(swiglu))
    if entry not in ("plain", "swiglu", "norm", "rope", "merge", "w8"):
        return False
    if not w or (not is_merge and not x) or (not is_rope and not y):
        return False
    if K % 512 or M > (4 if norm or is_merge else 16 if is_rope else 32) or ((norm or is_merge) and M * K > 32768):
        return False
    if not is_merge and (ldx % 8 or ldx < K):
        return False
    if not w8 and (ldw % 8 or ldw < K):
        return False
    if not is_rope and (N % 16 or ldy % 4 or ldy < (N // 2 if swiglu else N)):
        return False
    if (entry == "norm" or is_rope) and ldd % 8:
        return False
    if norm and (not gamma or (delta and (ldd < K or not h_out))):
        return False
    if is_rope:
        r = rope.get
        if r("Hq", 0) <= 0 or r("Hkv", 0) <= 0 or r("max_seq", 0) <= 0 or N != (r("Hq") + 2 * r("Hkv")) * 128:
            return False
        if not all(r(p, 1) for p in ("cosb", "sinb", "pos", "q", "kc", "vc")) or (r("bt", 0) and r("maxb", 0) <= 0):
            return False
    if is_merge and (not merge.get("ml", 1) or not merge.get("po", 1) or merge["nsplit"] < 1):
        return False
    return not w8 or bool(scale)


SKINNY_M = int(os.environ.get("MXLLM_SKINNY_M", "8"))
_SKINNY_SMALL_W = 128 << 20
NORM_M = int(os.environ.get("MXLLM_NORM_FUSED_M", "2"))


def _skinny_takes(entry: str, x2: torch.Tensor, w: torch.Tensor, *, swiglu: bool = False, norm: bool = False,
                  gamma=None, delta=None, rope=None) -> bool:
    M, N = (x2.shape[0] if x2.dim() == 2 else 0), w.shape[0]
    if not 0 < M <= (min(NORM_M, SKINNY_M) if norm else SKINNY_M) or (w.requires_grad and torch.is_grad_enabled()):
        return False
    if M > 1 and N * w.shape[1] > _SKINNY_SMALL_W:
        return False
    rows = (x2, w) if delta is None else (x2, w, delta)
    if not (x2.is_cuda and use_native(x2) and x2.shape[1] == w.shape[1]
            and all(t.dtype == torch.bfloat16 and t.stride(1) == 1 for t in rows)):
        return False
    if gamma is not None and (gamma.dtype != torch.bfloat16 or not gamma.is_contiguous()):
        return False
    if delta is not None and (not norm or delta.shape != x2.shape):
        return False
# ... 62 lines not shown
```

mxllm/ops/reference.py:

```python
from __future__ import annotations

import math

import torch
import torch.nn.functional as F


def rms_norm(x: torch.Tensor, w: torch.Tensor, eps: float) -> torch.Tensor:
    xf = x.float()
    y = xf * torch.rsqrt(xf.pow(2).mean(-1, keepdim=True) + eps) * w.float()
    return y.to(x.dtype)


def llama3_inv_freq(head_dim: int, theta: float, scaling: dict | None) -> torch.Tensor:
    inv = 1.0 / (theta ** (torch.arange(0, head_dim, 2, dtype=torch.float64) / head_dim))
    if not scaling:
        return inv
    factor = scaling.get("factor", 8.0)
    lf = scaling.get("low_freq_factor", 1.0)
    hf = scaling.get("high_freq_factor", 4.0)
    old = scaling.get("original_max_position_embeddings", 8192)
    low_wl, high_wl = old / lf, old / hf
    wl = 2 * math.pi / inv
    out = torch.where(wl > low_wl, inv / factor, inv)
    smooth = (old / wl - lf) / (hf - lf)
    mid = (1 - smooth) * out / factor + smooth * out
    is_mid = (wl >= high_wl) & (wl <= low_wl)
    return torch.where(is_mid, mid, out)


def rope_tables(seq_len: int, head_dim: int, theta: float, scaling: dict | None, device=None):
    inv = llama3_inv_freq(head_dim, theta, scaling)
    t = torch.arange(seq_len, dtype=torch.float64)
    ang = torch.outer(t, inv)
    return ang.cos().float().to(device), ang.sin().float().to(device)


def apply_rope(x: torch.Tensor, cos: torch.Tensor, sin: torch.Tensor) -> torch.Tensor:
    S, D = x.shape[1], x.shape[-1]
    c = cos[:S].view(1, S, 1, D // 2).float()
    s = sin[:S].view(1, S, 1, D // 2).float()
    xf = x.float()
    x1, x2 = xf[..., : D // 2], xf[..., D // 2:]
    return torch.cat([x1 * c - x2 * s, x2 * c + x1 * s], dim=-1).to(x.dtype)


def attention(q: torch.Tensor, k: torch.Tensor, v: torch.Tensor, causal: bool = True,
              scale: float | None = None) -> torch.Tensor:
    B, S, Hq, D = q.shape
    Sk, Hkv = k.shape[1], k.shape[2]
    rep = Hq // Hkv
    scale = scale if scale is not None else 1.0 / math.sqrt(D)
    qf = q.float().transpose(1, 2)
    kf = k.float().transpose(1, 2).repeat_interleave(rep, dim=1)
    vf = v.float().transpose(1, 2).repeat_interleave(rep, dim=1)
    s = torch.matmul(qf, kf.transpose(-1, -2)) * scale
    if causal:
        i = torch.arange(S, device=q.device).view(S, 1)
        j = torch.arange(Sk, device=q.device).view(1, Sk)
        s = s.masked_fill(j > i + (Sk - S), float("-inf"))
    p = torch.softmax(s, dim=-1)
    o = torch.matmul(p, vf)
    return o.transpose(1, 2).to(q.dtype)


def swiglu(gate_up: torch.Tensor) -> torch.Tensor:
    F_ = gate_up.shape[-1] // 2
    g, u = gate_up[..., :F_].float(), gate_up[..., F_:].float()
    return (F.silu(g) * u).to(gate_up.dtype)


def cross_entropy(logits: torch.Tensor, labels: torch.Tensor, ignore_index: int = -100) -> torch.Tensor:
    return F.cross_entropy(logits.float(), labels, ignore_index=ignore_index, reduction="mean")


def adamw_(p: torch.Tensor, g: torch.Tensor, m: torch.Tensor, v: torch.Tensor, *, lr: float, beta1: float,
           beta2: float, eps: float, weight_decay: float, step: int, grad_scale: float = 1.0,
           p_lowp: torch.Tensor | None = None) -> None:
    gf = g.float() * grad_scale
    m.mul_(beta1).add_(gf, alpha=1 - beta1)
    v.mul_(beta2).addcmul_(gf, gf, value=1 - beta2)
    bc1 = 1 - beta1 ** step
    bc2 = 1 - beta2 ** step
    p.mul_(1 - lr * weight_decay)
    denom = (v / bc2).sqrt_().add_(eps)
    p.addcdiv_(m, denom, value=-lr / bc1)
    if p_lowp is not None:
        p_lowp.copy_(p)
```

Baseline: 4719 tokens/s.

## Fuse LoRA MLP weight gradients into SwiGLU backward column kernel

Adds a new HIP kernel that computes the SwiGLU backward, the LoRA tail projection, the gate/up LoRA B gradient and the down LoRA A gradient in a single pass over the activation tiles. A link object passes the needed operands between the down and gate_up LoRA linears and the SwiGLU autograd function, so lora_grads can skip the halves already produced. The aim is to avoid re-reading the large [T, 2F] dgu and SwiGLU output tensors in separate grad GEMMs. In exchange the backward bookkeeping becomes more complex and stateful, and the kernel accepts only a narrow set of shapes.

```diff
diff --git a/csrc/bindings.cpp b/csrc/bindings.cpp
--- a/csrc/bindings.cpp
+++ b/csrc/bindings.cpp
@@ -426,6 +426,56 @@
     MX_OK(mx_swiglu_lora(bwd ? 1 : 0, bf(gu), bwd ? bf(*dm) : nullptr, bfm(out), W + pad, bf(v), ldv, (int)nrb,
                          (int)pad, (float)alpha, ws.data_ptr<float>(), (int)T, (int)F, cur_stream()));
   return out.narrow(1, 0, W);
+}
+
+at::Tensor swiglu_lora_bwd_grads(const at::Tensor& dm, const at::Tensor& gu, int64_t pad, const at::Tensor& v,
+                                 int64_t nrb, double alpha, const at::Tensor& st, const at::Tensor& gd, int64_t nd,
+                                 at::Tensor& gb, at::Tensor& ga) {
+  check_bf16(gu, "gu");
+  check_bf16(dm, "dm");
+  const int64_t ldv = check_rows_bf16(v, "v"), ldst = check_rows_bf16(st, "st"), ldgd = check_rows_bf16(gd, "gd");
+  for (const at::Tensor* t : {&gb, &ga}) {
+    MX_CHECK(t->is_cuda() && t->scalar_type() == at::kBFloat16 && t->dim() == 2 && t->stride(1) == 1 &&
+                 t->stride(0) >= t->size(1),
+             "swiglu_lora_bwd_grads: gb / ga must be 2-D bf16 GPU views with unit column stride");
+  }
+  for (const at::Tensor* t : {&dm, &v, &st, &gd, (const at::Tensor*)&gb, (const at::Tensor*)&ga})
+    MX_CHECK(t->device() == gu.device(), "swiglu_lora_bwd_grads: operands on different devices");
+  MX_CHECK(gu.dim() == 2 && gu.size(1) > 0 && gu.size(1) % 256 == 0,
+           "swiglu_lora_bwd_grads: gu [T, 2F] with F % 128 == 0 (gate | up halves of equal width)");
+  const int64_t F2 = gu.size(1), F = F2 / 2, T = gu.size(0);
+  MX_CHECK(T % 64 == 0, "swiglu_lora_bwd_grads: [T, 2F] with T % 64 == 0");
+  MX_CHECK(nrb == 2 || nrb == 4, "swiglu_lora_bwd_grads: nrb 2 or 4 (r = 16 or 32 per gate / up adapter)");
+  MX_CHECK(nd == 1 || nd == 2, "swiglu_lora_bwd_grads: nd 1 or 2 (16 or 32 down-adapter rows)");
+  MX_CHECK(pad >= 16 * nrb && pad % 8 == 0, "swiglu_lora_bwd_grads: 16 nrb <= pad, pad % 8 == 0");
+  MX_CHECK(dm.dim() == 2 && dm.size(0) == T && dm.size(1) == F, "swiglu_lora_bwd_grads: dm shape");
+  MX_CHECK(v.size(0) >= 16 * nrb && v.size(1) == F2, "swiglu_lora_bwd_grads: v shape");
+  MX_CHECK(st.size(0) == T && st.size(1) >= 16 * nrb, "swiglu_lora_bwd_grads: st [T, >= 16 nrb]");
+  MX_CHECK(gd.size(0) == T && gd.size(1) >= 16 * nd, "swiglu_lora_bwd_grads: gd [T, >= 16 nd]");
+  MX_CHECK(gb.size(0) == F2 && gb.size(1) >= 16 * nrb, "swiglu_lora_bwd_grads: gb [2F, >= 16 nrb]");
+  MX_CHECK(ga.size(0) >= 16 * nd && ga.size(1) == F, "swiglu_lora_bwd_grads: ga [>= 16 nd, F]");
+  DevGuard g(gu.device());
+  mx::SwigluColsLaunch L{};
+  L.gu = gu.data_ptr(), L.dm = dm.data_ptr(), L.v = v.data_ptr(), L.ldv = ldv;
+  L.st = st.data_ptr(), L.ldst = ldst, L.gd = gd.data_ptr(), L.ldgd = ldgd;
+  L.gb = gb.data_ptr(), L.ldgb = gb.stride(0), L.ga = ga.data_ptr(), L.ldga = ga.stride(0);
+  L.T = T, L.F = F, L.nrb = nrb, L.nd = nd, L.pad = pad, L.ldo = F2 + pad;
+  L.splits = mx_swiglu_cols_splits_req();
+  alignas(16) static char standin[16];
+  L.out = standin, L.ws = reinterpret_cast<float*>(standin);
+  MX_CHECK(T == 0 || mx::swiglu_cols_takes(L),
+           "swiglu_lora_bwd_grads: the kernel does not take this call (mx::swiglu_cols_takes, "
+           "csrc/kernels/swiglu_cols_args.h): T ", T, ", F ", F, ", row strides v ", ldv, ", st ", ldst, ", gd ", ldgd,
+           ", gb ", L.ldgb, ", ga ", L.ldga, " or an operand that is not 16-B aligned");
+  at::Tensor out = at::empty({T, F2 + pad}, gu.options());
+  if (T == 0) return out.narrow(1, 0, F2);
+  auto ws = at::empty({mx::swiglu_cols_ws(T, F, nrb, nd, L.splits)}, gu.options().dtype(at::kFloat));
+  L.out = out.data_ptr(), L.ws = ws.data_ptr<float>();
+  const int rc = mx_swiglu_cols(L, (float)alpha, cur_stream());
+  MX_CHECK(rc != -1, "swiglu_lora_bwd_grads: launch refused (mx::swiglu_cols_takes)");
+  TORCH_CHECK(rc == 0, "mxllm kernel launch failed (swiglu_lora_bwd_grads) rc=", rc, " ",
+              hipGetErrorString((hipError_t)rc));
+  return out.narrow(1, 0, F2);
 }
 
 void adamw_step(const c10::optional<at::Tensor>& master, at::Tensor grad, at::Tensor m, at::Tensor v,
@@ -1465,7 +1515,7 @@
 }
 
 void lora_grads(const at::Tensor& x, const at::Tensor& dy, const at::Tensor& g, const at::Tensor& st, at::Tensor& ga,
-                at::Tensor& gb, at::IntArrayRef splits, int64_t r, bool accumulate) {
+                at::Tensor& gb, at::IntArrayRef splits, int64_t r, bool accumulate, bool want_a, bool want_b) {
   const int64_t ldx = check_rows_bf16(x, "x"), ldd = check_rows_bf16(dy, "dy");
   const int64_t ldg = check_rows_bf16(g, "g"), lds = check_rows_bf16(st, "st");
   check_bf16(ga, "ga");
@@ -1487,19 +1537,21 @@
     }
     desc.insert(desc.end(), {(int64_t)X, (int64_t)G, (int64_t)out, lx, lg, os_n, os_j, Nx, jb0, JB});
   };
-  for (int64_t j0 = 0; j0 < R; j0 += 64) {
+  for (int64_t j0 = 0; want_a && j0 < R; j0 += 64) {
     const int64_t jb = std::min<int64_t>(4, (R - j0) / 16);
     add(bf(x), ldx, bf(g), ldg, g.size(1), bfm(ga) + j0 * K, 1, K, K, j0 / 16, jb);
   }
   int64_t off = 0;
   for (int64_t i = 0; i < n; ++i) {
     const int64_t ni = splits[i];
-    add(bf(dy) + off, ldd, bf(st), lds, st.size(1), bfm(gb) + off * R + i * r, R, 1, ni, i * r / 16, r / 16);
+    if (want_b) add(bf(dy) + off, ldd, bf(st), lds, st.size(1), bfm(gb) + off * R + i * r, R, 1, ni, i * r / 16, r / 16);
+    else MX_CHECK(ni % 64 == 0, "lora_grads: split sizes must be multiples of 64");
     off += ni;
   }
   MX_CHECK(off == N, "lora_grads: splits do not sum to dy's width");
   const int np = (int)(desc.size() / 10);
   MX_CHECK(np <= 8, "lora_grads: too many problems");
+  if (np == 0) return;
   int64_t ntiles = 0;
   for (int i = 0; i < np; ++i) ntiles += desc[i * 10 + 7] / 64;
   DevGuard gd(x.device());
@@ -1635,7 +1687,8 @@
   m.def("quant_rows_e4m3(Tensor x) -> (Tensor, Tensor)");
   m.def("lora_xwt(Tensor x, Tensor v, Tensor(a!) out, float alpha, int rows=0) -> ()");
   m.def("swiglu_lora(Tensor? dm, Tensor gu, int pad, Tensor v, int nrb, float alpha) -> Tensor");
-  m.def("lora_grads(Tensor x, Tensor dy, Tensor g, Tensor st, Tensor(a!) ga, Tensor(b!) gb, int[] splits, int r, bool accumulate) -> ()");
+  m.def("lora_grads(Tensor x, Tensor dy, Tensor g, Tensor st, Tensor(a!) ga, Tensor(b!) gb, int[] splits, int r, bool accumulate, bool want_a=True, bool want_b=True) -> ()");
+  m.def("swiglu_lora_bwd_grads(Tensor dm, Tensor gu, int pad, Tensor v, int nrb, float alpha, Tensor st, Tensor gd, int nd, Tensor(a!) gb, Tensor(b!) ga) -> Tensor");
   m.def("lora_gather_shrink(Tensor x, Tensor ids, Tensor a_tab, Tensor(a!) partials) -> ()");
   m.def("lora_gather_expand_add_(Tensor(a!) y, Tensor partials, Tensor ids, Tensor b_tab, Tensor s_tab, int[] splits, int K) -> ()");
   m.def("attn_bwd(Tensor dout, Tensor q, Tensor k, Tensor v, Tensor o, Tensor lse, bool causal, float scale, int dq_mode=3, Tensor? dq_out=None, Tensor? dk_out=None, Tensor? dv_out=None) -> (Tensor, Tensor, Tensor)");
@@ -1704,6 +1757,7 @@
   m.impl("lora_xwt", &lora_xwt);
   m.impl("swiglu_lora", &swiglu_lora);
   m.impl("lora_grads", &lora_grads);
+  m.impl("swiglu_lora_bwd_grads", &swiglu_lora_bwd_grads);
   m.impl("lora_gather_shrink", &lora_gather_shrink);
   m.impl("lora_gather_expand_add_", &lora_gather_expand_add_);
 }
diff --git a/csrc/bindings.h b/csrc/bindings.h
--- a/csrc/bindings.h
+++ b/csrc/bindings.h
@@ -7,6 +7,7 @@
 #include "kernels/gemm8_args.h"
 #include "kernels/prefill_paged_args.h"
 #include "kernels/skinny_args.h"
+#include "kernels/swiglu_cols_args.h"
 #include "kernels/verify_args.h"
 #include "kernels/w4_args.h"
 
@@ -100,6 +101,8 @@
 int mx_lora_xwt(const uint16_t* X, int64_t ldx, const uint16_t* V, int64_t ldv, int Vrows, uint16_t* out, int64_t ldo,
                 float* ws, int M, int K, float alpha, int rows, hipStream_t stream);
 int mx_lora_xtg(const int64_t* desc, int np, int T, float alpha, int accumulate, float* ws, hipStream_t stream);
+int mx_swiglu_cols(const mx::SwigluColsLaunch& L, float alpha, hipStream_t stream);
+int64_t mx_swiglu_cols_splits_req();
 
 int mx_lora_serve_ksplits(int K);
 int mx_lora_gather_shrink(const uint16_t* x, int64_t ldx, const int32_t* ids, const uint16_t* a_tab, float* part,
diff --git a/csrc/kernels/lora.hip b/csrc/kernels/lora.hip
--- a/csrc/kernels/lora.hip
+++ b/csrc/kernels/lora.hip
@@ -779,6 +779,371 @@
       const int rr = k / NC, cc = k % NC;
       wp[k] = ((red[0][rr][cc] + red[1][rr][cc]) + red[2][rr][cc]) + red[3][rr][cc];
     }
+  }
+}
+
+struct ColsArgs {
+  const uint16_t *gu, *dm, *V, *st, *gd;
+  uint16_t* out;
+  float *wst, *wsg;
+  int64_t ldo, ldv, ldst, ldgd;
+  int T, F, RS;
+};
+
+constexpr int kColImg = 16384;
+
+template <class V>
+__device__ __forceinline__ V ld_uo(const void* base, uint32_t off) {
+  return *reinterpret_cast<const V*>(static_cast<const char*>(base) + off);
+}
+template <class V>
+__device__ __forceinline__ void st_uo(void* base, uint32_t off, const V& v) {
+  *reinterpret_cast<V*>(static_cast<char*>(base) + off) = v;
+}
+__device__ __forceinline__ uint32_t fresh(uint32_t v) {
+  asm volatile("" : "+v"(v));
+  return v;
+}
+
+#ifndef MX_COLS_PF
+#define MX_COLS_PF 1
+#endif
+template <int NRB, int ND>
+__global__ void __launch_bounds__(256, NRB == 2 ? 2 : 1) swiglu_cols_kernel(const ColsArgs a) {
+  constexpr bool PF = NRB == 2 && MX_COLS_PF;
+  constexpr int NT = NRB, NC = 16 * NRB, JB = NRB / 2, CW = 16 * (NRB + ND);
+  constexpr int GD0 = NRB == 2 ? 2 : 0;
+  constexpr int kSt = 3 * kColImg, kGd = NRB == 2 ? kSt : kSt + 8192, kV = kGd + 8192;
+  constexpr int kVRow = 2 * kSlRow;
+  __shared__ __attribute__((aligned(16))) char smem[kV + 2 * NC * kVRow];
+  const int tid = threadIdx.x, lane = tid & 63, c = lane & 15, g = lane >> 4;
+  const int w = __builtin_amdgcn_readfirstlane(tid >> 6);
+  const int strip = blockIdx.x, split = blockIdx.y;
+  const int F = a.F, tiles = F >> 7;
+  const int tl0 = strip * NT, nt = tiles - tl0 < NT ? tiles - tl0 : NT;
+  const int nblk = a.T >> 6;
+  const int b0 = (int)((int64_t)split * nblk / a.RS), b1 = (int)((int64_t)(split + 1) * nblk / a.RS);
+  const int row = tid >> 4, ch = tid & 15;
+  const int64_t F2 = 2 * (int64_t)F;
+  const int col0 = tl0 * 128;
+  const uint32_t lo_gu = 2u * ((uint32_t)row * (uint32_t)F2 + 8u * ch), lo_dm = 2u * ((uint32_t)row * (uint32_t)F + 8u * ch);
+  const uint32_t lo_out = 2u * ((uint32_t)row * (uint32_t)a.ldo + 8u * ch);
+  const uint32_t lo_v = 2u * ((uint32_t)row * (uint32_t)a.ldv + 8u * ch);
+
+  const uint32_t sbase = lds_addr(smem);
+  struct LaneMap {
+    int wofs, vwofs, vrofs, rofs[4];
+    uint32_t xb[2], sb[NRB], db[ND];
+  };
+  auto lane_map = [&](uint32_t t) {
+    LaneMap m;
+    const int c_ = t & 15, g_ = (t >> 4) & 3, row_ = t >> 4, ch_ = t & 15;
+    m.wofs = (ch_ >> 3) * 8192 + row_ * 128 + 16 * ((ch_ & 7) ^ xsw(row_));
+#pragma unroll
+    for (int kk = 0; kk < 4; ++kk)
+      m.rofs[kk] = (kk >> 1) * 8192 + (16 * w + c_) * 128 + 16 * ((4 * (kk & 1) + g_) ^ xsw(c_));
+    m.vwofs = kV + row_ * kVRow + 16 * ch_;
+    m.vrofs = kV + c_ * kVRow + 16 * g_;
+    const int qq = c_ >> 2, pp = c_ & 3, fl = xsw(4 * g_ + qq);
+    const uint32_t trow = sbase + (4 * g_ + qq) * 128 + 8 * (pp & 1);
+#pragma unroll
+    for (int ib = 0; ib < 2; ++ib)
+      m.xb[ib] = trow + (w >> 1) * 8192 + 16 * ((2 * (2 * (w & 1) + ib) + (pp >> 1)) ^ fl);
+#pragma unroll
+    for (int j = 0; j < NRB; ++j) m.sb[j] = trow + kSt + 16 * ((2 * j + (pp >> 1)) ^ fl);
+#pragma unroll
+    for (int j = 0; j < ND; ++j) m.db[j] = trow + kGd + 16 * ((2 * (GD0 + j) + (pp >> 1)) ^ fl);
+    return m;
+  };
+  const int srow = tid / (2 * NRB), sch = tid % (2 * NRB);
+  const int drow = tid / (2 * ND), dch = tid % (2 * ND);
+  const uint32_t lo_st = 2u * ((uint32_t)srow * (uint32_t)a.ldst + 8u * sch);
+  const uint32_t lo_gd = 2u * ((uint32_t)drow * (uint32_t)a.ldgd + 8u * dch);
+
+  f32x4 accT[NRB], accB[NT][2][2][JB], accA[NT][2][ND];
+#pragma unroll
+  for (int b = 0; b < NRB; ++b) accT[b] = f32x4{0.f, 0.f, 0.f, 0.f};
+#pragma unroll
+  for (int t = 0; t < NT; ++t)
+#pragma unroll
+    for (int ib = 0; ib < 2; ++ib) {
+#pragma unroll
+      for (int p = 0; p < 2; ++p)
+#pragma unroll
+        for (int j = 0; j < JB; ++j) accB[t][p][ib][j] = f32x4{0.f, 0.f, 0.f, 0.f};
+#pragma unroll
+      for (int j = 0; j < ND; ++j) accA[t][ib][j] = f32x4{0.f, 0.f, 0.f, 0.f};
+    }
+
+  u16x8 gg[4], uu[4], dd[4], vf[2][NRB], stn[JB], gdn;
+  auto load = [&](int b, int tt, u16x8(&g_)[4], u16x8(&u_)[4], u16x8(&d_)[4]) {
+    const uint16_t* gb_ = a.gu + (int64_t)b * 64 * F2 + col0;
+    const uint16_t* db_ = a.dm + (int64_t)b * 64 * F + col0;
+    const uint32_t lg = fresh(lo_gu), ld = fresh(lo_dm);
+#pragma unroll
+    for (int i = 0; i < 4; ++i) {
+      const uint32_t og = lg + 32u * i * (uint32_t)F2 + 256u * tt, od = ld + 32u * i * (uint32_t)F + 256u * tt;
+      g_[i] = ld_uo<u16x8>(gb_, og);
+      u_[i] = ld_uo<u16x8>(gb_, og + 2u * (uint32_t)F);
+      d_[i] = ld_uo<u16x8>(db_, od);
+    }
+  };
+  auto vload = [&](int tt) {
+    const uint32_t lv = fresh(lo_v);
+#pragma unroll
+    for (int p = 0; p < 2; ++p)
+#pragma unroll
+      for (int b = 0; b < NRB; ++b)
+        vf[p][b] = ld_uo<u16x8>(a.V + col0, lv + 32u * b * (uint32_t)a.ldv + 2u * p * (uint32_t)F + 256u * tt);
+  };
+  auto sload = [&](int b) {
+    const int64_t t0 = (int64_t)b * 64;
+#pragma unroll
+    for (int q = 0; q < JB; ++q)
+      stn[q] = ld_uo<u16x8>(a.st + t0 * a.ldst, lo_st + 2u * q * (128 / NRB) * (uint32_t)a.ldst);
+    if (tid < 128 * ND) gdn = ld_uo<u16x8>(a.gd + t0 * a.ldgd, lo_gd);
+  };
+  if (b0 < b1) {
+    if constexpr (PF) {
+      load(b0, 0, gg, uu, dd);
+      vload(0);
+    }
+    sload(b0);
+  }
+  for (int b = b0; b < b1; ++b) {
+    __syncthreads();
+#pragma unroll
+    for (int q = 0; q < JB; ++q) {
+      const int r_ = srow + q * (128 / NRB);
+      *reinterpret_cast<u16x8*>(smem + kSt + r_ * 128 + 16 * (sch ^ xsw(r_))) = stn[q];
+    }
+    if (tid < 128 * ND)
+      *reinterpret_cast<u16x8*>(smem + kGd + drow * 128 + 16 * ((2 * GD0 + dch) ^ xsw(drow))) = gdn;
+    if (b + 1 < b1) sload(b + 1);
+    uint16_t* ob_ = a.out + (int64_t)b * 64 * a.ldo + col0;
+#pragma unroll
+    for (int tt = 0; tt < NT; ++tt) {
+      if (tt >= nt) break;
+      if (tt > 0) __syncthreads();
+      u16x8 gn[4], un[4], dn[4];
+      if constexpr (PF) {
+        const bool more = tt + 1 < nt;
+        const int nb = more ? b : (b + 1 < b1 ? b + 1 : b), ntt = more ? tt + 1 : (b + 1 < b1 ? 0 : tt);
+        load(nb, ntt, gn, un, dn);
+      }
+      const uint32_t lo = fresh(lo_out);
+      const LaneMap lm = lane_map(fresh((uint32_t)tid));
+      auto row_math = [&](const u16x8& g_, const u16x8& u_, const u16x8& d_, int i) {
+        u16x8 o0, o1, om;
+#pragma unroll
+        for (int j = 0; j < 8; ++j) {
+          const float gf = bf2f(g_[j]), uf = bf2f(u_[j]), df = bf2f(d_[j]);
+          float dg, du;
+          swiglu_grad(df, gf, uf, dg, du);
+          o0[j] = f2bf(dg);
+          o1[j] = f2bf(du);
+          om[j] = f2bf(gf * sl_sigmoid(gf) * uf);
+        }
+        const uint32_t oo = lo + 32u * i * (uint32_t)a.ldo + 256u * tt;
+        st_uo(ob_, oo, o0);
+        st_uo(ob_, oo + 2u * (uint32_t)F, o1);
+        *reinterpret_cast<u16x8*>(smem + lm.wofs + 2048 * i) = o0;
+        *reinterpret_cast<u16x8*>(smem + kColImg + lm.wofs + 2048 * i) = o1;
+        *reinterpret_cast<u16x8*>(smem + 2 * kColImg + lm.wofs + 2048 * i) = om;
+      };
+      if constexpr (PF) {
+#pragma unroll
+        for (int i = 0; i < 4; ++i) row_math(gg[i], uu[i], dd[i], i);
+      } else {
+        const uint16_t* gb_ = a.gu + (int64_t)b * 64 * F2 + col0;
+        const uint16_t* db_ = a.dm + (int64_t)b * 64 * F + col0;
+#pragma unroll 1
+        for (int i = 0; i < 4; i += 2) {
+          const uint32_t og = fresh(lo_gu) + 32u * i * (uint32_t)F2 + 256u * tt;
+          const uint32_t od = fresh(lo_dm) + 32u * i * (uint32_t)F + 256u * tt;
+          const u16x8 g0 = ld_uo<u16x8>(gb_, og), u0 = ld_uo<u16x8>(gb_, og + 2u * (uint32_t)F);
+          const u16x8 d0 = ld_uo<u16x8>(db_, od);
+          const u16x8 g1 = ld_uo<u16x8>(gb_, og + 32u * (uint32_t)F2);
+          const u16x8 u1 = ld_uo<u16x8>(gb_, og + 32u * (uint32_t)F2 + 2u * (uint32_t)F);
+          const u16x8 d1 = ld_uo<u16x8>(db_, od + 32u * (uint32_t)F);
+          const int p = i >> 1;
+          const uint32_t lv = fresh(lo_v) + 2u * p * (uint32_t)F + 256u * tt;
+          u16x8 vh[NRB];
+#pragma unroll
+          for (int bb = 0; bb < NRB; ++bb) vh[bb] = ld_uo<u16x8>(a.V + col0, lv + 32u * bb * (uint32_t)a.ldv);
+          row_math(g0, u0, d0, i);
+          row_math(g1, u1, d1, i + 1);
+#pragma unroll
+          for (int bb = 0; bb < NRB; ++bb)
+            *reinterpret_cast<u16x8*>(smem + lm.vwofs + (p * NC + 16 * bb) * kVRow) = vh[bb];
+        }
+      }
+      if constexpr (PF) {
+#pragma unroll
+        for (int p = 0; p < 2; ++p)
+#pragma unroll
+          for (int bb = 0; bb < NRB; ++bb)
+            *reinterpret_cast<u16x8*>(smem + lm.vwofs + (p * NC + 16 * bb) * kVRow) = vf[p][bb];
+      }
+      __syncthreads();
+      __builtin_amdgcn_sched_barrier(0);
+#pragma unroll
+      for (int kk = 0; kk < 4; ++kk)
+#pragma unroll
+        for (int p = 0; p < 2; ++p) {
+          const u16x8 af = *reinterpret_cast<const u16x8*>(smem + p * kColImg + lm.rofs[kk]);
+#pragma unroll
+          for (int bb = 0; bb < NRB; ++bb) {
+            const u16x8 bf =
+                *reinterpret_cast<const u16x8*>(smem + lm.vrofs + (p * NC + 16 * bb) * kVRow + 64 * kk);
+            accT[bb] = lmfma(af, bf, accT[bb]);
+          }
+          __builtin_amdgcn_sched_barrier(0);
+        }
+      __builtin_amdgcn_sched_barrier(0);
+      auto frag = [](const u16x4& lo, const u16x4& hi) {
+        return u16x8{lo[0], lo[1], lo[2], lo[3], hi[0], hi[1], hi[2], hi[3]};
+      };
+#pragma unroll
+      for (int ks = 0; ks < 2; ++ks) {
+        u16x4 xr[3][2][2], sr[NRB][2], dr[ND][2];
+#pragma unroll
+        for (int h = 0; h < 2; ++h) {
+          const int ro = (32 * ks + 16 * h) * 128;
+#pragma unroll
+          for (int p = 0; p < 3; ++p)
+#pragma unroll
+            for (int ib = 0; ib < 2; ++ib) xr[p][ib][h] = trd_off(lm.xb[ib], p * kColImg + ro);
+#pragma unroll
+          for (int j = 0; j < NRB; ++j) sr[j][h] = trd_off(lm.sb[j], ro);
+#pragma unroll
+          for (int j = 0; j < ND; ++j) dr[j][h] = trd_off(lm.db[j], ro);
+        }
+        lds_wait();
+#pragma unroll
+        for (int h = 0; h < 2; ++h) {
+#pragma unroll
+          for (int p = 0; p < 3; ++p)
+#pragma unroll
+            for (int ib = 0; ib < 2; ++ib) pin(xr[p][ib][h]);
+#pragma unroll
+          for (int j = 0; j < NRB; ++j) pin(sr[j][h]);
+#pragma unroll
+          for (int j = 0; j < ND; ++j) pin(dr[j][h]);
+        }
+#pragma unroll
+        for (int ib = 0; ib < 2; ++ib) {
+#pragma unroll
+          for (int p = 0; p < 2; ++p) {
+            const u16x8 af = frag(xr[p][ib][0], xr[p][ib][1]);
+#pragma unroll
+            for (int j = 0; j < JB; ++j)
+              accB[tt][p][ib][j] = lmfma(af, frag(sr[p * JB + j][0], sr[p * JB + j][1]), accB[tt][p][ib][j]);
+          }
+          const u16x8 mf = frag(xr[2][ib][0], xr[2][ib][1]);
+#pragma unroll
+          for (int j = 0; j < ND; ++j) accA[tt][ib][j] = lmfma(mf, frag(dr[j][0], dr[j][1]), accA[tt][ib][j]);
+        }
+        __builtin_amdgcn_sched_barrier(0);
+      }
+      if constexpr (PF) {
+        vload(tt + 1 < nt ? tt + 1 : 0);
+#pragma unroll
+        for (int i = 0; i < 4; ++i) gg[i] = gn[i], uu[i] = un[i], dd[i] = dn[i];
+      }
+    }
+    float* wp = a.wst + ((int64_t)strip * a.T + (int64_t)b * 64 + 16 * w) * NC;
+    const uint32_t lt = fresh(4u * (4 * g * NC + c));
+#pragma unroll
+    for (int bb = 0; bb < NRB; ++bb) {
+#pragma unroll
+      for (int e = 0; e < 4; ++e) st_uo(wp, lt + 4u * (e * NC + 16 * bb), accT[bb][e]);
+      accT[bb] = f32x4{0.f, 0.f, 0.f, 0.f};
+    }
+  }
+  constexpr int r = 8 * NRB;
+  const uint32_t lq = fresh(4u * (4 * g * CW + c));
+#pragma unroll
+  for (int tt = 0; tt < NT; ++tt) {
+    if (tt >= nt) break;
+#pragma unroll
+    for (int ib = 0; ib < 2; ++ib) {
+      const int n0 = (tl0 + tt) * 128 + (w >> 1) * 64 + 16 * (2 * (w & 1) + ib);
+      float* wq = a.wsg + ((int64_t)split * F + n0) * CW;
+#pragma unroll
+      for (int e = 0; e < 4; ++e) {
+        const uint32_t lo = lq + 4u * e * CW;
+#pragma unroll
+        for (int p = 0; p < 2; ++p)
+#pragma unroll
+          for (int j = 0; j < JB; ++j) st_uo(wq, lo + 4u * (p * r + 16 * j), accB[tt][p][ib][j][e]);
+#pragma unroll
+        for (int j = 0; j < ND; ++j) st_uo(wq, lo + 4u * (2 * r + 16 * j), accA[tt][ib][j][e]);
+      }
+    }
+  }
+}
+
+__global__ void __launch_bounds__(256) swiglu_cols_reduce_kernel(const float* __restrict__ wsg, int RS, int F, int r,
+                                                                 int nd, uint16_t* __restrict__ gb, int64_t ldgb,
+                                                                 uint16_t* __restrict__ ga, int64_t ldga) {
+  __shared__ float sa[32][65];
+  const int CW = 2 * r + 16 * nd, n0 = blockIdx.x * 64, tid = threadIdx.x;
+  const float* w0 = wsg + (int64_t)n0 * CW;
+  const int64_t sstep = (int64_t)F * CW;
+  for (int e = tid; e < 64 * CW; e += 256) {
+    const int n = e / CW, q = e % CW;
+    float s = w0[e];
+#pragma unroll 4
+    for (int sp = 1; sp < RS; ++sp) s += w0[sp * sstep + e];
+    if (q < 2 * r) {
+      uint16_t* o = gb + ((int64_t)(q / r) * F + n0 + n) * ldgb + q;
+      *o = f2bf(bf2f(*o) + s);
+    } else {
+      sa[q - 2 * r][n] = s;
+    }
+  }
+  __syncthreads();
+  for (int e = tid; e < 16 * nd * 64; e += 256) {
+    const int j = e >> 6, n = e & 63;
+    uint16_t* o = ga + (int64_t)j * ldga + n0 + n;
+    *o = f2bf(bf2f(*o) + sa[j][n]);
+  }
+}
+
+__global__ void __launch_bounds__(256) swiglu_cols_tail_reduce_kernel(const float* __restrict__ wst, int strips,
+                                                                      int64_t plane, int NC, int pad,
+                                                                      uint16_t* __restrict__ tail, int64_t ldo,
+                                                                      float alpha) {
+  __shared__ float4 part[8][32];
+  const int it = threadIdx.x & 31, grp = threadIdx.x >> 5;
+  const int64_t e = ((int64_t)blockIdx.x * 32 + it) * 4;
+  const int s0 = grp * strips / 8, s1 = (grp + 1) * strips / 8;
+  float4 acc{0.f, 0.f, 0.f, 0.f};
+#pragma unroll 4
+  for (int s = s0; s < s1; ++s) {
+    const float4 v = *reinterpret_cast<const float4*>(wst + s * plane + e);
+    acc.x += v.x, acc.y += v.y, acc.z += v.z, acc.w += v.w;
+  }
+  part[grp][it] = acc;
+  __syncthreads();
+  if (grp == 0) {
+    float4 t = part[0][it];
+#pragma unroll
+    for (int k = 1; k < 8; ++k) {
+      const float4 v = part[k][it];
+      t.x += v.x, t.y += v.y, t.z += v.z, t.w += v.w;
+    }
+    const int64_t row = e / NC;
+    const int cc = (int)(e % NC);
+    uint2 o;
+    o.x = pack_bf16x2(alpha * t.x, alpha * t.y);
+    o.y = pack_bf16x2(alpha * t.z, alpha * t.w);
+    *reinterpret_cast<uint2*>(tail + row * ldo + cc) = o;
+  } else if (grp == 1 && pad > NC) {
+    const int64_t row0 = (int64_t)blockIdx.x * 128 / NC;
+    const int zc = pad - NC;
+    for (int k = it; k < (128 / NC) * zc; k += 32) tail[(row0 + k / zc) * ldo + NC + k % zc] = 0;
   }
 }
 
@@ -844,6 +1209,32 @@
   const char* v = getenv(name);
   return v && *v ? atoi(v) : dflt;
 }
+
+extern "C" int64_t mx_swiglu_cols_splits_req() { return lora_env("MXLLM_SWIGLU_COLS_RS", 0); }
+
+extern "C" int mx_swiglu_cols(const mx::SwigluColsLaunch& L, float alpha, hipStream_t stream) {
+  if (L.T == 0) return 0;
+  if (!mx::swiglu_cols_takes(L)) return -1;
+  const int T = (int)L.T, F = (int)L.F, nrb = (int)L.nrb, nd = (int)L.nd;
+  const int strips = (int)mx::swiglu_cols_strips(F, nrb), RS = (int)mx::swiglu_cols_splits(T, F, nrb, L.splits);
+  ColsArgs a{};
+  a.gu = static_cast<const uint16_t*>(L.gu), a.dm = static_cast<const uint16_t*>(L.dm);
+  a.V = static_cast<const uint16_t*>(L.v), a.st = static_cast<const uint16_t*>(L.st);
+  a.gd = static_cast<const uint16_t*>(L.gd), a.out = static_cast<uint16_t*>(L.out);
+  a.wst = L.ws, a.wsg = L.ws + mx::swiglu_cols_tail_ws(T, F, nrb);
+  a.ldo = L.ldo, a.ldv = L.ldv, a.ldst = L.ldst, a.ldgd = L.ldgd;
+  a.T = T, a.F = F, a.RS = RS;
+  const dim3 grid(strips, RS);
+  if (nrb == 2 && nd == 1) swiglu_cols_kernel<2, 1><<<grid, 256, 0, stream>>>(a);
+  else if (nrb == 2) swiglu_cols_kernel<2, 2><<<grid, 256, 0, stream>>>(a);
+  else if (nd == 1) swiglu_cols_kernel<4, 1><<<grid, 256, 0, stream>>>(a);
+  else swiglu_cols_kernel<4, 2><<<grid, 256, 0, stream>>>(a);
+  swiglu_cols_tail_reduce_kernel<<<(unsigned)((int64_t)T * 16 * nrb / 128), 256, 0, stream>>>(
+      a.wst, strips, (int64_t)T * 16 * nrb, 16 * nrb, (int)L.pad, a.out + 2 * (int64_t)F, L.ldo, alpha);
+  swiglu_cols_reduce_kernel<<<F / 64, 256, 0, stream>>>(a.wsg, RS, F, 8 * nrb, nd, static_cast<uint16_t*>(L.gb), L.ldgb,
+                                                       static_cast<uint16_t*>(L.ga), L.ldga);
+  return (int)hipGetLastError();
+}
 static int lora_splits(int tiles, int blocks, int smax) {
   if (tiles <= 0) return 1;
   const int target = lora_env("MXLLM_LORA_WGS", 256);
diff --git a/csrc/kernels/swiglu_cols_args.h b/csrc/kernels/swiglu_cols_args.h
--- /dev/null
+++ b/csrc/kernels/swiglu_cols_args.h
@@ -0,0 +1,72 @@
+#pragma once
+#include <stdint.h>
+
+namespace mx {
+
+constexpr int SC_TILE = 128;
+constexpr int SC_ROWS = 64;
+constexpr int SC_WGS = 1024;
+constexpr int SC_MAX_SPLITS = 1024;
+constexpr int64_t SC_MAX_LD = 1 << 24;
+
+struct SwigluColsLaunch {
+  const void* gu;
+  const void* dm;
+  void* out;
+  int64_t ldo;
+  const void* v;
+  int64_t ldv;
+  const void* st;
+  int64_t ldst;
+  const void* gd;
+  int64_t ldgd;
+  void* gb;
+  int64_t ldgb;
+  void* ga;
+  int64_t ldga;
+  float* ws;
+  int64_t T, F, nrb, nd, pad;
+  int64_t splits;
+};
+
+inline int64_t swiglu_cols_strip(int64_t nrb) { return SC_TILE * nrb; }
+inline int64_t swiglu_cols_strips(int64_t F, int64_t nrb) {
+  const int64_t w = swiglu_cols_strip(nrb);
+  return w > 0 ? (F + w - 1) / w : 0;
+}
+inline int64_t swiglu_cols_splits(int64_t T, int64_t F, int64_t nrb, int64_t req) {
+  const int64_t strips = swiglu_cols_strips(F, nrb), blocks = T / SC_ROWS;
+  int64_t s = req > 0 ? req : (strips > 0 ? (SC_WGS + strips / 2) / strips : 1);
+  if (s > blocks) s = blocks;
+  if (s > SC_MAX_SPLITS) s = SC_MAX_SPLITS;
+  return s < 1 ? 1 : s;
+}
+inline int64_t swiglu_cols_tail_ws(int64_t T, int64_t F, int64_t nrb) {
+  return swiglu_cols_strips(F, nrb) * T * 16 * nrb;
+}
+inline int64_t swiglu_cols_ws(int64_t T, int64_t F, int64_t nrb, int64_t nd, int64_t splits_req) {
+  return swiglu_cols_tail_ws(T, F, nrb) + swiglu_cols_splits(T, F, nrb, splits_req) * F * 16 * (nrb + nd);
+}
+
+inline bool swiglu_cols_takes(const SwigluColsLaunch& L) {
+  constexpr int64_t I32 = 0x7fffffff;
+  if (!L.gu || !L.dm || !L.out || !L.v || !L.st || !L.gd || !L.gb || !L.ga || !L.ws) return false;
+  if (L.T < SC_ROWS || L.T % SC_ROWS || L.T > I32) return false;
+  if (L.F < SC_TILE || L.F % SC_TILE || 2 * L.F > SC_MAX_LD) return false;
+  if (L.ldo > SC_MAX_LD || L.ldv > SC_MAX_LD || L.ldst > SC_MAX_LD || L.ldgd > SC_MAX_LD) return false;
+  if (L.nrb != 2 && L.nrb != 4) return false;
+  if (L.nd != 1 && L.nd != 2) return false;
+  if (L.pad < 16 * L.nrb || L.pad % 8 || L.pad > I32) return false;
+  if (L.ldo < 2 * L.F + L.pad || L.ldo % 8) return false;
+  if (L.ldv < 2 * L.F || L.ldv % 8) return false;
+  if (L.ldst < 16 * L.nrb || L.ldst % 8) return false;
+  if (L.ldgd < 16 * L.nd || L.ldgd % 8) return false;
+  if ((uintptr_t)L.gu % 16 || (uintptr_t)L.dm % 16 || (uintptr_t)L.out % 16 || (uintptr_t)L.v % 16 ||
+      (uintptr_t)L.st % 16 || (uintptr_t)L.gd % 16)
+    return false;
+  if (L.ldgb < 16 * L.nrb || L.ldga < L.F) return false;
+  if ((uintptr_t)L.gb % 2 || (uintptr_t)L.ga % 2 || (uintptr_t)L.ws % 16) return false;
+  return true;
+}
+
+}
diff --git a/mxllm/models/llama.py b/mxllm/models/llama.py
--- a/mxllm/models/llama.py
+++ b/mxllm/models/llama.py
@@ -96,13 +96,14 @@
         amat = self.wa if self.transposed else self.wbuf[sum(self.splits):, :self.in_features]
         return (amat, R, self.scaling), (self.wbt, R, self.scaling)
 
-    def forward(self, x: torch.Tensor, x_tail: bool = False, dy_tail: bool = False) -> torch.Tensor:
+    def forward(self, x: torch.Tensor, x_tail: bool = False, dy_tail: bool = False, mlp_link=None,
+                mlp_role: str | None = None) -> torch.Tensor:
         if self.lora_r > 0:
             if self.augmented():
                 return ops.lora_linear_aug(x, self.lora_a, self.lora_b, self.wbuf, self.splits, self.scaling,
                                            self.pad, self.wbt, getattr(self, "wxt", None),
                                            getattr(self, "wa", None) if self.transposed else None,
-                                           x_tail=x_tail, dy_tail=dy_tail)
+                                           x_tail=x_tail, dy_tail=dy_tail, mlp_link=mlp_link, mlp_role=mlp_role)
             return ops.lora_linear(x, self.weight, self.lora_a, self.lora_b, self.splits, self.scaling)
         return ops.linear(x, self.weight)
 
@@ -231,15 +232,19 @@
             m = fused.gate_up_swiglu(x, layer.wgu.weight, out_pad=self._pad(layer.wd))
             d = layer.wd(m)
         else:
-            tf, tb = self._swiglu_tails(layer, x)
-            m = ops.swiglu(layer.wgu(x, dy_tail=tb is not None), out_pad=self._pad(layer.wd),
-                           grad_pad=self._pad(layer.wgu), tail_fwd=tf, tail_bwd=tb)
-            d = layer.wd(m, x_tail=tf is not None)
+            d = self._mlp_block(layer, x)
         last = i + 1 == len(self.layers)
         nxt = self.final_norm if last else self.layers[i + 1].attn_norm
         x, h = ops.add_rms_norm(d, h, nxt, cfg.norm_eps, out_pad=0 if last else self._pad(self.layers[i + 1].wqkv),
                                 grad_pad=self._pad(layer.wd))
         return x, h
+
+    def _mlp_block(self, layer, x: torch.Tensor) -> torch.Tensor:
+        tf, tb = self._swiglu_tails(layer, x)
+        link = ops.lora_mlp_link(layer.wgu, layer.wd, x, (tf, tb))
+        m = ops.swiglu(layer.wgu(x, dy_tail=tb is not None, mlp_link=link, mlp_role="gu"),
+                       out_pad=self._pad(layer.wd), grad_pad=self._pad(layer.wgu), tail_fwd=tf, tail_bwd=tb, link=link)
+        return layer.wd(m, x_tail=tf is not None, mlp_link=link, mlp_role="d")
 
     def _recompute_m(self, layer, i: int) -> bool:
         if (RECOMPUTE_SWIGLU == "0" or any(lin.lora_r > 0 for lin in (layer.wqkv, layer.wgu, layer.wd))
diff --git a/mxllm/ops/__init__.py b/mxllm/ops/__init__.py
--- a/mxllm/ops/__init__.py
+++ b/mxllm/ops/__init__.py
@@ -1,7 +1,7 @@
 from ._ext import available as native_available, native, use_native
 from .norm import rms_norm, add_rms_norm
 from .attention import attention_block
-from .activation import lora_tail_ok, swiglu
+from .activation import LoRAMLPLink, lora_mlp_link, lora_tail_ok, swiglu
 from .loss import linear_cross_entropy, cross_entropy
 from .optim import SplitMaster, adamw_step_, sq_norm
 from .embedding import embedding
diff --git a/mxllm/ops/activation.py b/mxllm/ops/activation.py
--- a/mxllm/ops/activation.py
+++ b/mxllm/ops/activation.py
@@ -4,16 +4,49 @@
 
 import torch
 
+from ..parallel.grad_ready import direct_grad, mark_ready
 from . import reference as ref
 from ._ext import native, use_native
 
 
+class LoRAMLPLink:
+    __slots__ = ("b_gu", "a_d", "nd", "st", "gd", "armed", "done")
+
+    def __init__(self, b_gu: torch.Tensor, a_d: torch.Tensor):
+        self.b_gu, self.a_d, self.nd = b_gu, a_d, a_d.shape[0] // 16
+        self.st = self.gd = None
+        self.armed = self.done = False
+
+    def targets(self):
+        gb, ga = direct_grad(self.b_gu), direct_grad(self.a_d)
+        return None if gb is None or ga is None else (gb, ga)
+
+
+def lora_mlp_link(wgu, wd, x: torch.Tensor, tails) -> LoRAMLPLink | None:
+    if not _MLP_BWD or tails[0] is None or tails[1] is None or not torch.is_grad_enabled():
+        return None
+    if wgu.transposed or wd.transposed or x.shape[0] % 64 or wgu.lora_r not in (16, 32) or wd.lora_r != wgu.lora_r:
+        return None
+    if len(wgu.splits) != 2 or wgu.splits[0] != wgu.splits[1] or len(wd.splits) != 1:
+        return None
+    if not all(p.requires_grad for p in (wgu.lora_a, wgu.lora_b, wd.lora_a, wd.lora_b)):
+        return None
+    link = LoRAMLPLink(wgu.lora_b, wd.lora_a)
+    return link if link.targets() is not None else None
+
+
 class _SwiGLUFn(torch.autograd.Function):
     @staticmethod
-    def forward(ctx, gu, out_pad, grad_pad, tail_fwd, tail_bwd):
-        ctx.save_for_backward(gu)
+    def forward(ctx, gu, out_pad, grad_pad, tail_fwd, tail_bwd, link=None, st=None):
+        if st is not None:
+            ctx.save_for_backward(gu, st)
+        else:
+            ctx.save_for_backward(gu)
         ctx.grad_pad = grad_pad
         ctx.tail_bwd = tail_bwd
+        ctx.link = link if st is not None else None
+        if ctx.link is not None:
+            link.armed = True
         if tail_fwd is not None:
             v, nrb, s = tail_fwd
             return native().swiglu_lora(None, gu, out_pad, v, nrb, s)
@@ -21,13 +54,25 @@
 
     @staticmethod
     def backward(ctx, dm):
-        (gu,) = ctx.saved_tensors
-        if ctx.tail_bwd is not None:
+        saved = ctx.saved_tensors
+        gu, link = saved[0], ctx.link
+        gd = None
+        if link is not None:
+            gd, link.gd = link.gd, None
+        tg = link.targets() if gd is not None else None
+        if tg is not None:
+            v, nrb, s = ctx.tail_bwd
+            dgu = native().swiglu_lora_bwd_grads(dm.contiguous(), gu, ctx.grad_pad, v, nrb, s, saved[1], gd, link.nd,
+                                                 tg[0], tg[1])
+            mark_ready(link.b_gu)
+            mark_ready(link.a_d)
+            link.done = True
+        elif ctx.tail_bwd is not None:
             v, nrb, s = ctx.tail_bwd
             dgu = native().swiglu_lora(dm.contiguous(), gu, ctx.grad_pad, v, nrb, s)
         else:
             dgu = native().swiglu_bwd(dm.contiguous(), gu, ctx.grad_pad)
-        return dgu, None, None, None, None
+        return dgu, None, None, None, None, None, None
 
 
 def lora_tail_ok(x: torch.Tensor, T: int, F2: int, pad: int, R: int) -> bool:
@@ -36,14 +81,21 @@
 
 
 _FUSE_TAIL = os.environ.get("MXLLM_SWIGLU_LORA", "1") != "0"
+_MLP_BWD = os.environ.get("MXLLM_LORA_MLP_BWD", "1") != "0"
 
 
-def swiglu(gate_up: torch.Tensor, out_pad: int = 0, grad_pad: int = 0, tail_fwd=None, tail_bwd=None) -> torch.Tensor:
+def swiglu(gate_up: torch.Tensor, out_pad: int = 0, grad_pad: int = 0, tail_fwd=None, tail_bwd=None,
+           link: LoRAMLPLink | None = None) -> torch.Tensor:
+    st = None
+    if link is not None:
+        st, link.st = link.st, None
     if use_native(gate_up):
         if gate_up.dim() != 2:
             out_pad = grad_pad = 0
             tail_fwd = tail_bwd = None
         tf = (tail_fwd[0], tail_fwd[1] // 16, float(tail_fwd[2])) if tail_fwd is not None else None
         tb = (tail_bwd[0], tail_bwd[1] // 16, float(tail_bwd[2])) if tail_bwd is not None else None
-        return _SwiGLUFn.apply(gate_up.contiguous(), out_pad, grad_pad, tf, tb)
+        if tb is None or tf is None or st is None:
+            link = st = None
+        return _SwiGLUFn.apply(gate_up.contiguous(), out_pad, grad_pad, tf, tb, link, st)
     return ref.swiglu(gate_up)
diff --git a/mxllm/ops/linear.py b/mxllm/ops/linear.py
--- a/mxllm/ops/linear.py
+++ b/mxllm/ops/linear.py
@@ -100,7 +100,26 @@
     da = db = None
     ga = direct_grad(ctx.lora_a) if need_a else None
     gb = direct_grad(ctx.lora_b) if need_b else None
-    if nat and need_a and need_b:
+    link = getattr(ctx, "mlp_link", None)
+    role = getattr(ctx, "mlp_role", None) if link is not None else None
+    if (nat and need_a and need_b and role == "d" and link.armed and link.a_d is ctx.lora_a
+            and link.targets() is not None):
+        tgb = gb if gb is not None else torch.zeros(N, R, dtype=dy2.dtype, device=dy2.device)
+        native().lora_grads(x2, dy2, dya[:, N:], xa[:, K:], ga, tgb, list(splits), r, gb is not None, False, True)
+        if gb is not None:
+            mark_ready(ctx.lora_b)
+        else:
+            db = tgb
+        link.gd = dya[:, N:]
+    elif nat and need_a and need_b and role == "gu" and link.done and link.b_gu is ctx.lora_b and gb is not None:
+        link.done = False
+        tga = ga if ga is not None else torch.empty(R, K, dtype=dy2.dtype, device=dy2.device)
+        native().lora_grads(x2, dy2, dya[:, N:], xa[:, K:], tga, gb, list(splits), r, ga is not None, True, False)
+        if ga is not None:
+            mark_ready(ctx.lora_a)
+        else:
+            da = tga
+    elif nat and need_a and need_b:
         acc = ga is not None and gb is not None
         tga = ga if acc else torch.empty(R, K, dtype=dy2.dtype, device=dy2.device)
         tgb = gb if acc else torch.zeros(N, R, dtype=dy2.dtype, device=dy2.device)
@@ -140,7 +159,8 @@
 class _LoRAAugFn(torch.autograd.Function):
 
     @staticmethod
-    def forward(ctx, x, a, b, wbuf, scaling, splits, r, pad, wbt, wxt=None, wa=None, x_tail=False, dy_tail=False):
+    def forward(ctx, x, a, b, wbuf, scaling, splits, r, pad, wbt, wxt=None, wa=None, x_tail=False, dy_tail=False,
+                mlp_link=None, mlp_role=None):
         tr = wa is not None
         if tr:
             K, N = wbuf.shape[0] - pad, wbuf.shape[1] - pad
@@ -161,6 +181,9 @@
         ctx.lora_a, ctx.lora_b, ctx.wbt, ctx.wxt = a, b, wbt, wxt
         ctx.dims = (N, K, scaling, tuple(splits), r, pad, x.shape, nat, tr)
         ctx.dy_tail = dy_tail
+        ctx.mlp_link, ctx.mlp_role = (mlp_link, mlp_role) if nat and not tr else (None, None)
+        if ctx.mlp_link is not None and mlp_role == "gu":
+            mlp_link.st = xa[:, K:]
         return y.view(*x.shape[:-1], N)
 
     @staticmethod
@@ -168,15 +191,17 @@
         xa, wbuf = ctx.saved_tensors
         dx, da, db = _lora_aug_backward(ctx, xa, wbuf, dy, ctx.dy_tail, ctx.needs_input_grad[1],
                                         ctx.needs_input_grad[2])
-        return dx, da, db, None, None, None, None, None, None, None, None, None, None
+        return dx, da, db, None, None, None, None, None, None, None, None, None, None, None, None
 
 
 def lora_linear_aug(x: torch.Tensor, a: torch.Tensor, b: torch.Tensor, wbuf: torch.Tensor, splits: Sequence[int],
                     scaling: float, pad: int, wbt: torch.Tensor | None = None,
                     wxt: torch.Tensor | None = None, wa: torch.Tensor | None = None,
-                    x_tail: bool = False, dy_tail: bool = False) -> torch.Tensor:
+                    x_tail: bool = False, dy_tail: bool = False, mlp_link=None,
+                    mlp_role: str | None = None) -> torch.Tensor:
     r = a.shape[0] // len(splits)
-    return _LoRAAugFn.apply(x, a, b, wbuf, scaling, tuple(splits), r, pad, wbt, wxt, wa, bool(x_tail), bool(dy_tail))
+    return _LoRAAugFn.apply(x, a, b, wbuf, scaling, tuple(splits), r, pad, wbt, wxt, wa, bool(x_tail), bool(dy_tail),
+                            mlp_link, mlp_role)
 
 
 _LORA_QKV_ROPE = os.environ.get("MXLLM_LORA_QKV_ROPE", "1") != "0"
diff --git a/mxllm/ops/reference.py b/mxllm/ops/reference.py
--- a/mxllm/ops/reference.py
+++ b/mxllm/ops/reference.py
@@ -70,6 +70,33 @@
     return (F.silu(g) * u).to(gate_up.dtype)
 
 
+def swiglu_lora_bwd_grads(dm: torch.Tensor, gu: torch.Tensor, pad: int, v: torch.Tensor, nrb: int, alpha: float,
+                          st: torch.Tensor, gd: torch.Tensor, nd: int, gb: torch.Tensor, ga: torch.Tensor) -> torch.Tensor:
+    ts = (dm, gu, v, st, gd, gb, ga)
+    if any(t.dtype != torch.bfloat16 or t.dim() != 2 or t.stride(1) != 1 or t.device != gu.device for t in ts):
+        raise RuntimeError("swiglu_lora_bwd_grads: 2-D bf16 operands with unit column stride on one device")
+    T, F2 = gu.shape
+    F_, R, r = F2 // 2, 16 * nrb, 8 * nrb
+    if (not gu.is_contiguous() or not dm.is_contiguous() or F2 == 0 or F2 % 256 or T % 64 or nrb not in (2, 4)
+            or nd not in (1, 2) or pad < R or pad % 8 or tuple(dm.shape) != (T, F_) or v.shape[0] < R
+            or v.shape[1] != F2 or st.shape[0] != T or st.shape[1] < R or gd.shape[0] != T or gd.shape[1] < 16 * nd
+            or gb.shape[0] != F2 or gb.shape[1] < R or ga.shape[0] < 16 * nd or ga.shape[1] != F_
+            or any(t.stride(0) % 8 or t.stride(0) < t.shape[1] for t in (v, st, gd))):
+        raise RuntimeError("swiglu_lora_bwd_grads: operands refused")
+    g, u, d = gu[:, :F_].float(), gu[:, F_:].float(), dm.float()
+    s = torch.sigmoid(g)
+    dgu = torch.cat([d * u * s * (1 + g * (1 - s)), d * g * s], dim=1).to(gu.dtype)
+    m = (g * s * u).to(gu.dtype)
+    out = torch.zeros(T, F2 + pad, dtype=gu.dtype, device=gu.device)
+    out[:, :F2] = dgu
+    out[:, F2:F2 + R] = (alpha * (dgu.float() @ v[:R].float().t())).to(gu.dtype)
+    for i in range(2):
+        blk = gb[i * F_:(i + 1) * F_, i * r:(i + 1) * r]
+        blk.copy_((blk.float() + dgu[:, i * F_:(i + 1) * F_].float().t() @ st[:, i * r:(i + 1) * r].float()).to(gb.dtype))
+    ga[:16 * nd].copy_((ga[:16 * nd].float() + gd[:, :16 * nd].float().t() @ m.float()).to(ga.dtype))
+    return out[:, :F2]
+
+
 def cross_entropy(logits: torch.Tensor, labels: torch.Tensor, ignore_index: int = -100) -> torch.Tensor:
     return F.cross_entropy(logits.float(), labels, ignore_index=ignore_index, reduction="mean")
 
```

Measured after the change: 4763 tokens/s (median of 6 runs). About the same (+0.9%).
